# lmb-freiburg/understanding_flow_robustness

Hardware: AMD Instinct MI355X
Metric: attack-iters/s (higher is better)
Workload: dtype f32

## Files before the change

include/ufr_hip.h:

```cpp
#ifndef UFR_HIP_H_
#define UFR_HIP_H_

#include <stdint.h>

#ifdef __cplusplus
extern "C" {
#endif

#define UFR_ABI_VERSION 9

enum { UFR_F32 = 0, UFR_F64 = 1, UFR_F16 = 2 };
enum {
  UFR_OK = 0,
  UFR_EINVAL = -1,
  UFR_EUNSUPPORTED = -2,
  UFR_ELAUNCH = -3
};

typedef void* ufr_stream_t;

int ufr_abi_version(void);
const char* ufr_last_error(void);
int ufr_device_count(void);
const char* ufr_build_manifest(void);
// ... 376 lines not shown
int ufr_normalize_frames(const float* frames_a, const float* frames_b, float* out, int Ba, int Bb, int C, int H, int W,
                         const double* mean, ufr_stream_t stream);

int ufr_corr_forward_planes_window(const void* f1_planes, const void* f2_planes, long in_plane_stride, void* out_planes,
                                   long out_plane_stride, int out_chunk0, int B, int C, int H, int W, int patch,
                                   int dilation_patch, float scale, float slope, const int* win, int level_stride,
                                   int win_cells, ufr_stream_t stream);

int ufr_corr_forward_planes_changed(const void* f1_planes, const void* f2_planes, long in_plane_stride, void* out_planes,
                                    long out_plane_stride, int out_chunk0, int B, int C, int H, int W, int patch,
                                    int dilation_patch, float scale, float slope, const int* win, int level_stride,
                                    int win_cells_h, int win_cells_w, int margin, ufr_stream_t stream);

int ufr_corr_backward_window_fused(const float* f1, const float* f2, const float* G, int g_chunk0, float g_scale,
                                   const float* G_redir, float* grad_window, int B, int C, int H, int W, int patch,
                                   int dilation_patch, const int* win, int level_stride, int wh, int ww, int margin,
                                   ufr_stream_t stream);

int ufr_corr_forward_planes(const void* f1_planes, const void* f2_planes, long in_plane_stride, void* out_planes,
                            long out_plane_stride, int out_chunk0, int B, int C, int H, int W, int patch,
                            int dilation_patch, float scale, float slope, ufr_stream_t stream);
int ufr_flow_head_planes_forward(const void* planes, long plane_stride, int chunk0, int chunks, const float* wpk, int w_chunks,
                                 const float* bias, float* out, int B, int H, int W, ufr_stream_t stream);
int ufr_flow_head_planes_forward_mfma(const void* planes, long plane_stride, int chunk0, int chunks, const void* wmf, int w_chunks,
                                      const float* bias, float* out, int B, int H, int W, ufr_stream_t stream);
int ufr_flow_head_split_plan(int B, int H, int W, int chunks, int* slices, int* starved, long* partial_floats);
int ufr_flow_head_planes_forward_split(const void* planes, long plane_stride, int chunk0, int chunks, const void* wmf, int w_chunks,
                                       float* partials, long partial_floats, int slices, int B, int H, int W, ufr_stream_t stream);
int ufr_flow_head_split_finish(const float* partials, long partial_floats, int slices, const float* bias, float* flow,
                               const float* up_w, const float* up_bias, void* up_planes, long up_plane_stride, int up_chunk, int B,
                               int H, int W, ufr_stream_t stream);
int ufr_deconv_flow_tail_backward_mfma(const void* grad_planes, long plane_stride, int chunk0, int chunks, const void* wmf,
                                       int w_chunks, float* G, int g_chunks, int out_chunk, int B, int H, int W, ufr_stream_t stream);
int ufr_flow_head_planes_backward(const float* grad_y, const float* wpk, int w_chunks, float* G, int g_chunks, int chunk0, int chunks,
                                  int B, int H, int W, int accumulate, ufr_stream_t stream);
int ufr_flow_head_planes_backward_finalize(const float* grad_y, const float* wpk, int w_chunks, float* G, int g_chunks, int chunk0,
                                           int chunks, int B, int H, int W, int accumulate, const void* mask_planes, void* out_planes,
                                           long out_plane_stride, int fin_chunk0, int fin_chunks, float slope, ufr_stream_t stream);
#define UFR_PF_REGION_BAND 1
#define UFR_PF_REGION_WINDOW 2
int ufr_flow_head_planes_backward_regions(const float* grad_y, const float* wpk, int w_chunks, float* G, int g_chunks, int chunk0,
                                          int chunks, int B, int H, int W, int accumulate, int head_chunks, int region,
                                          const int* origin, int origin_stride, int origin_div, int reg_h, int reg_w, int margin,
                                          float* head_out, int head_out_images, const void* mask_planes, void* out_planes,
                                          long out_plane_stride, int fin_chunk0, int fin_chunks, float slope, ufr_stream_t stream);
int ufr_upfeat_planes_forward_mfma(const void* planes, long plane_stride, int chunk0, int chunks, const void* wmf, int w_chunks,
                                   const float* bias, float* out, int B, int H, int W, ufr_stream_t stream);
int ufr_upfeat_planes_backward(const float* grad_y, const float* wpk, int w_chunks, float* G, int g_chunks, int chunk0, int chunks,
                               int B, int H, int W, int accumulate, ufr_stream_t stream);
int ufr_flow_up_planes_forward(const float* x, const float* w, const float* bias, void* planes, long plane_stride,
                               int chunk, int B, int H, int W, ufr_stream_t stream);
int ufr_flow_up_planes_backward(const float* G, int chunk, const float* w, float* grad_x, int B, int H, int W,
                                int accumulate , ufr_stream_t stream);

#define UFR_TRAIN_LOSS_MAX_SCALES 8
typedef struct {
  const float* gt; int B, H, W;
  int nscale;
  const float* pred[UFR_TRAIN_LOSS_MAX_SCALES];
  float* grad[UFR_TRAIN_LOSS_MAX_SCALES];
  int h[UFR_TRAIN_LOSS_MAX_SCALES], w[UFR_TRAIN_LOSS_MAX_SCALES];
  double weight[UFR_TRAIN_LOSS_MAX_SCALES];
  int kind;
  double div_flow;
  double* ws; long ws_elems;
  double* out;
} ufr_train_loss_desc;
long ufr_train_loss_workspace_doubles(int B, int nscale, const int* h, const int* w);
int ufr_train_loss(const ufr_train_loss_desc* d, ufr_stream_t stream);

typedef struct { float* p; const float* g; float* m; float* v; long n; } ufr_adamw_seg;
typedef struct { double lr, beta1, beta2, eps, weight_decay, bias1, bias2; } ufr_adamw_hyper;
long ufr_grad_norm_partials(const ufr_adamw_seg* segs, int nseg);
int ufr_grad_norm(const ufr_adamw_seg* segs, int nseg, float max_norm, double* partials, long partial_elems, float* norm_out,
                  ufr_stream_t stream);
int ufr_adamw_step(const ufr_adamw_seg* segs, int nseg, const ufr_adamw_hyper* h, const float* norm, ufr_stream_t stream);

int ufr_sweep_paste(const float* tgt, const float* ref, const float* patch_p, const float* mask_p, const int* origins,
                    const int* origins_host, float* adv_tgt, float* adv_ref, int K, int H, int W, int ph, int pw, float lo, float hi,
                    const ufr_cone_chain* chain, int win_h, int win_w, int* win, float* xw, ufr_stream_t stream);
long ufr_sweep_metrics_workspace_doubles(int K);
int ufr_sweep_metrics(const float* pred, const float* gt, const float* mask_p, const int* origins, const int* origins_host, int K,
                      int H, int W, int Hg, int Wg, int ph, int pw, int valid_in_patch, double* ws, long ws_elems, float* out,
                      int row0, int rows, ufr_stream_t stream);

#define UFR_FEATURE_STATS_MAX_SEGS 32
typedef struct {
  const void* src; long plane_stride; long pixels; int kind, images, image0, B, chunk0, channels; double unleaky; long out_col;
} ufr_feature_stats_seg;
long ufr_feature_stats_workspace_doubles(const ufr_feature_stats_seg* segs, int nseg);
int ufr_feature_stats(const ufr_feature_stats_seg* segs, int nseg, double* ws, long ws_elems, double* out, int out_rows, long out_cols,
                      long out_stride, ufr_stream_t stream);

#define UFR_DIVERSE_COLS 8
long ufr_abs_sums_workspace_doubles(long n);
int ufr_abs_sums(const float* g0, const float* g1, long n, double* ws, long ws_elems, float* out, ufr_stream_t stream);
int ufr_momentum_update(const float* img0, const float* img1, const float* g0, const float* g1, const float* sums, float* m0,
                        float* m1, float* adv0, float* adv1, float* delta, int B, int CHW, float mu, float one_minus_mu, float lr,
                        float eps, float lo, float hi, int frames, int ascent, ufr_stream_t stream);
int ufr_diverse_table_check(const int* table_host, int rows, int H, int W);
long ufr_diverse_workspace_doubles(int B, int H, int W, int Cg);
int ufr_diverse_forward(const float* adv0, const float* adv1, const float* gt, float* x0, float* x1, float* gt_out, int B, int H,
                        int W, int Cg, const int* table, int rows, const int* step, float* scale_t, double* ws, long ws_elems,
                        ufr_stream_t stream);
int ufr_diverse_backward(const float* gx0, const float* gx1, float* g0, float* g1, int B, int H, int W, const int* table, int rows,
                         const int* step, ufr_stream_t stream);
// ... 7 lines not shown
```

understanding_flow_robustness_amd/_lib.py:

```python
from __future__ import annotations

import ctypes as C
import os

import torch

_HERE = os.path.dirname(os.path.abspath(__file__))
LIB_PATH = os.environ.get("UFR_HIP_LIB") or os.path.join(_HERE, "lib", "libufr_hip.so")
UFR_F32, UFR_F64, UFR_F16 = 0, 1, 2
ABI_VERSION = 9
_lib = None


class CorrParams(C.Structure):
    _fields_ = [(n, C.c_int) for n in (
        "kH", "kW", "patchH", "patchW", "padH", "padW", "dilationH", "dilationW",
        "dilation_patchH", "dilation_patchW", "dH", "dW")]


UFR_MAX_LEVELS = 8


class Pyramid(C.Structure):
    _fields_ = [("num_levels", C.c_int),
# ... 204 lines not shown
    "ufr_cm_norm_stats_apply": [_vp, _vp, _vp, _f, _vp, _l, _i, _vp, _l, _i, _l, _i, _i, _i, _i, _vp],
    "ufr_cm_norm_backward": [_vp, _vp, _vp, _i, _vp, _vp, _vp, _vp, _l, _i, _l, _i, _i, _i, _vp],
    "ufr_cm_masked_copy": [_vp, _vp, _l, _vp, _l, _vp],
    "ufr_raft_flow_patches": [_vp, _vp, _l, _i, _i, _i, _i, _vp],
    "ufr_raft_motion_finish_slabs": [_vp, _i, _i, _i, _vp, _f, _vp, _l, _vp, _l, _i, _vp, _i, _i, _i, _vp],
    "ufr_raft_motion_finish": [_vp, _l, _vp, _l, _i, _vp, _i, _i, _i, _vp],
    "ufr_raft_coords_step": [_vp, _vp, _vp, _vp, _vp, _l, _vp],
    "ufr_grad_finalize_consume": [_vp, _vp, _vp, _l, _l, _i, _f, _vp],
    "ufr_gru_gates_cm_forward": [_vp, _vp, _l, _i, _vp, _l, _i, _l, _i, _vp],
    "ufr_gru_gates_cm_forward_slabs": [_vp, _i, _i, _vp, _vp, _vp, _vp, _l, _i, _vp, _l, _i, _l, _i, _vp],
    "ufr_gru_blend_cm_forward_slabs": [_vp, _i, _i, _vp, _vp, _vp, _vp, _vp, _l, _i, _vp, _l, _i, _l, _i, _vp],
    "ufr_gru_blend_cm_forward": [_vp, _vp, _vp, _l, _i, _vp, _l, _i, _l, _i, _vp],
    "ufr_gru_blend_cm_backward": [_vp, _vp, _vp, _l, _i, _vp, _vp, _l, _i, _vp, _vp, _l, _i, _vp, _vp],
    "ufr_gru_gates_cm_backward": [_vp, _vp, _l, _i, _vp, _vp, _vp, _l, _i, _vp, _l, _i, _i, _vp, _vp],
    "ufr_altcorr_pyramid_forward": [_vp, _vp, _vp, _vp, _i, _i, _i, _i, _i, _f, _vp],
    "ufr_altcorr_pyramid_backward": [_vp, _vp, _vp, _vp, _vp, _vp, _i, _i, _i, _i, _i, _f, _i, _vp],
    "ufr_altcorr_pyramid_backward_cm": [_vp, _vp, _vp, _vp, _vp, _vp, _i, _i, _i, _i, _i, _f, _i, _vp],
    "ufr_upfeat_planes_forward_mfma": [_vp, _l, _i, _i, _vp, _i, _vp, _vp, _i, _i, _i, _vp],
    "ufr_upfeat_planes_backward": [_vp, _vp, _i, _vp, _i, _i, _i, _i, _i, _i, _i, _vp],
    "ufr_flow_up_planes_forward": [_vp, _vp, _vp, _vp, _l, _i, _i, _i, _i, _vp],
    "ufr_flow_head_split_plan": [_i, _i, _i, _i, C.POINTER(C.c_int), C.POINTER(C.c_int), C.POINTER(C.c_long)],
    "ufr_flow_head_planes_forward_split": [_vp, _l, _i, _i, _vp, _i, _vp, _l, _i, _i, _i, _i, _vp],
    "ufr_flow_head_split_finish": [_vp, _l, _i, _vp, _vp, _vp, _vp, _vp, _l, _i, _i, _i, _i, _vp],
    "ufr_flow_up_planes_backward": [_vp, _i, _vp, _vp, _i, _i, _i, _i, _vp],
    "ufr_corr_forward_planes_changed": [_vp, _vp, _l, _vp, _l, _i, _i, _i, _i, _i, _i, _i, _f, _f, _vp, _i, _i, _i, _i, _vp],
    "ufr_corr_forward_planes_window": [_vp, _vp, _l, _vp, _l, _i, _i, _i, _i, _i, _i, _i, _f, _f, _vp, _i, _i, _vp],
    "ufr_corr_forward_planes": [_vp, _vp, _l, _vp, _l, _i, _i, _i, _i, _i, _i, _i, _f, _f, _vp],
    "ufr_convex_upsample_forward": [_vp, _vp, _vp, _i, _i, _i, _vp],
    "ufr_convex_upsample_backward": [_vp, _vp, _vp, _vp, _vp, _vp, _i, _i, _i, _vp],
    "ufr_affine_resample_f64": [_vp, _vp, _i, _i, _i, _i, _i, _d, _d, _d, _d, _d, _d, _i, _vp],
    "ufr_patch_place": [_vp, _vp, _vp, _i, _i, _i, _vp, _vp, _vp, _i, _i, _i, _i, _vp],
    "ufr_patch_crop_f64": [_vp, _vp, _vp, _i, _i, _i, _i, _i, _i, _i, _vp],
    "ufr_resample_u8_horizontal": [_vp, _vp, _i, _i, _i, _i, _i, _vp, _vp, _i, _vp],
    "ufr_resample_u8_vertical": [_vp, _vp, _i, _i, _i, _i, _vp, _vp, _i, _vp],
    "ufr_u8_to_tensor": [_vp, _vp, _i, _i, _i, _i, _i, _i, _i, _f, _vp],
    "ufr_kitti_flow_decode": [_vp, _vp, _i, _i, _vp],
    "ufr_host_png_unfilter": [_vp, _vp, _i, _i, _i],
    "ufr_igemm_clock_probe": [_vp, _i],
    "ufr_altcorr_planes_prepare": [_vp, _vp, _l, _l, _i, _vp],
    "ufr_altcorr_planes_forward": [_vp, _l, C.POINTER(AltCorrPlaneLevels), _vp, _vp, _i, _i, _i, _i, _i, _f, _vp],
    "ufr_conv1_direct": [_vp, _vp, _i, _i, _i, _i, _vp, _vp, _vp, _f, _vp, _l, _i, _vp],
    "ufr_train_loss": [C.POINTER(TrainLossDesc), _vp],
    "ufr_grad_norm": [C.POINTER(AdamwSeg), _i, _f, _vp, _l, _vp, _vp],
    "ufr_adamw_step": [C.POINTER(AdamwSeg), _i, C.POINTER(AdamwHyper), _vp, _vp],
    "ufr_sweep_paste": [_vp, _vp, _vp, _vp, _vp, _vp, _vp, _vp, _i, _i, _i, _i, _i, _f, _f, C.POINTER(ConeChain), _i, _i, _vp, _vp, _vp],
    "ufr_sweep_metrics": [_vp, _vp, _vp, _vp, _vp, _i, _i, _i, _i, _i, _i, _i, _i, _vp, _l, _vp, _i, _i, _vp],
    "ufr_feature_stats": [C.POINTER(FeatureStatsSeg), _i, _vp, _l, _vp, _i, _l, _l, _vp],
    "ufr_abs_sums": [_vp, _vp, _l, _vp, _l, _vp, _vp],
    "ufr_momentum_update": [_vp, _vp, _vp, _vp, _vp, _vp, _vp, _vp, _vp, _vp, _i, _i, _f, _f, _f, _f, _f, _f, _i, _i, _vp],
    "ufr_diverse_table_check": [_vp, _i, _i, _i],
    "ufr_diverse_forward": [_vp, _vp, _vp, _vp, _vp, _vp, _i, _i, _i, _i, _vp, _i, _vp, _vp, _vp, _l, _vp],
    "ufr_diverse_backward": [_vp, _vp, _vp, _vp, _i, _i, _i, _vp, _i, _vp, _vp],
    "ufr_step_advance": [_vp, _vp],
}
DIVERSE_COLS = 8
PLAIN = {"ufr_abi_version": (C.c_int, []), "ufr_last_error": (C.c_char_p, []),
         "ufr_device_count": (C.c_int, []), "ufr_build_manifest": (C.c_char_p, []),
         "ufr_igemm_variant_fallbacks": (C.c_int, []),
         "ufr_conv3x3_c2_workspace_floats": (C.c_long, [_i, _i, _i, _i]),
         "ufr_cm_norm_workspace_doubles": (C.c_long, [_l, _i, _i]),
         "ufr_resample2d_backward_workspace_bytes": (C.c_long, [_i, _i, _i]),
         "ufr_pwc_warp_backward_workspace_bytes": (C.c_long, [_i, _i, _i]),
         "ufr_altcorr_pyramid_workspace_bytes": (C.c_long, [_i, _i, _i, _i, _i, _i]),
         "ufr_train_loss_workspace_doubles": (C.c_long, [_i, _i, C.POINTER(C.c_int), C.POINTER(C.c_int)]),
         "ufr_grad_norm_partials": (C.c_long, [C.POINTER(AdamwSeg), _i]),
         "ufr_sweep_metrics_workspace_doubles": (C.c_long, [_i]),
         "ufr_feature_stats_workspace_doubles": (C.c_long, [C.POINTER(FeatureStatsSeg), _i]),
         "ufr_abs_sums_workspace_doubles": (C.c_long, [_l]),
         "ufr_diverse_workspace_doubles": (C.c_long, [_i, _i, _i, _i])}


def lib():
    global _lib
    if _lib is None:
        if not os.path.exists(LIB_PATH):
            raise RuntimeError(
                f"{LIB_PATH} not found: build it with `python -c 'import __graft_entry__ as g; "
                "g.build()'` or `make -C understanding_flow_robustness_amd/csrc` (hipcc, gfx950). "
                "There is no CPU fallback.")
        handle = C.CDLL(LIB_PATH)
        for name, args in SIGNATURES.items():
            fn = getattr(handle, name)
            fn.argtypes, fn.restype = args, C.c_int
        for name, (res, args) in PLAIN.items():
            fn = getattr(handle, name)
            fn.argtypes, fn.restype = args, res
        if handle.ufr_abi_version() != ABI_VERSION:
            raise RuntimeError(f"{LIB_PATH} has ABI version {handle.ufr_abi_version()}, these bindings are written for "
                               f"{ABI_VERSION}: rebuild it (`make -C understanding_flow_robustness_amd/csrc`)")
        verify_build(handle.ufr_build_manifest().decode("ascii", "replace"))
        _lib = handle
    return _lib


_CSRC = os.path.join(_HERE, "csrc")
_HEADER = os.path.join(os.path.dirname(_HERE), "include", "ufr_hip.h")


def source_checksums(csrc: str = _CSRC, header: str = _HEADER) -> dict:
    import hashlib
    with open(os.path.join(csrc, "ufr_common.h"), "rb") as f:
        shared = f.read()
    with open(header, "rb") as f:
        shared += f.read()
    sums = {}
    for name in sorted(os.listdir(csrc)):
# ... 226 lines not shown
```

understanding_flow_robustness_amd/csrc/attack.hip:

```cpp
#include "ufr_common.h"

namespace {

using ufr::dev::clampf;

__global__ void paste_kernel(const float* __restrict__ tgt, const float* __restrict__ ref,
                             const float* __restrict__ patch, const float* __restrict__ mask,
                             float* __restrict__ adv_tgt, float* __restrict__ adv_ref, long total,
                             long CHW, long pstride, long mstride, int do_clamp, float lo, float hi) {
  for (long i = (long)blockIdx.x * blockDim.x + threadIdx.x; i < total;
       i += (long)gridDim.x * blockDim.x) {
    const long b = i / CHW, e = i - b * CHW;
    const float m = mask[b * mstride + e], pv = patch[b * pstride + e];
    const float mp = m * pv, om = 1.0f - m;
    float a = om * tgt[i] + mp;
    float r = om * ref[i] + mp;
    if (do_clamp) { a = clampf(a, lo, hi); r = clampf(r, lo, hi); }
    adv_tgt[i] = a;
    adv_ref[i] = r;
  }
}

__global__ void update_private_kernel(const float* __restrict__ tgt, const float* __restrict__ ref,
                                      const float* __restrict__ g_tgt, const float* __restrict__ g_ref,
// ... 280 lines not shown
        }
      rows[(long)g * (n + 1) + e] = s;
    }
  }
}

__global__ void patch_apply_paste_rect_kernel(const float* __restrict__ rows, int n_rows, float* __restrict__ patch_p,
                                              float* __restrict__ loss, const float* __restrict__ tgt, const float* __restrict__ ref,
                                              const float* __restrict__ mask_p, const int* __restrict__ origins,
                                              float* __restrict__ adv_tgt, float* __restrict__ adv_ref, int B, int H, int W, int ph,
                                              int pw, float step, float bound, int do_clamp, float lo, float hi,
                                              const float* __restrict__ gate) {
  const bool stopped = gate != nullptr && gate[0] != 0.f;
  const int n = 3 * ph * pw;
  for (int e = blockIdx.x * blockDim.x + threadIdx.x; e <= n; e += gridDim.x * blockDim.x) {
    float s = 0.f;
    for (int r = 0; r < n_rows; ++r) s += rows[(long)r * (n + 1) + e];
    if (e == n) { *loss = s; continue; }
    if (stopped) continue;
    const float pv = patch_p[e] - clampf(step * s, -bound, bound);
    patch_p[e] = pv;
    const int c = e / (ph * pw), q = e - c * ph * pw, i = q / pw, j = q - i * pw;
    const float m = mask_p[e], mp = m * pv, om = 1.0f - m;
    for (int b = 0; b < B; ++b) {
      const int y = origins[2 * b] + i, x = origins[2 * b + 1] + j;
      if ((unsigned)y >= (unsigned)H || (unsigned)x >= (unsigned)W) continue;
      const long o = ((long)b * 3 + c) * H * W + (long)y * W + x;
      float a = om * tgt[o] + mp, d = om * ref[o] + mp;
      if (do_clamp) { a = clampf(a, lo, hi); d = clampf(d, lo, hi); }
      adv_tgt[o] = a;
      adv_ref[o] = d;
    }
  }
}

__global__ void normalize_frames_kernel(const float* __restrict__ a, const float* __restrict__ b, float* __restrict__ out,
                                        long na, long total, int C, long HW, const double* __restrict__ mean) {
  for (long i = (long)blockIdx.x * blockDim.x + threadIdx.x; i < total; i += (long)gridDim.x * blockDim.x) {
    const int c = (int)((i / HW) % C);
    const float v = i < na ? a[i] : b[i - na];
    out[i] = (float)((double)v - mean[c]);
  }
}

__global__ void gate_kernel(const float* __restrict__ loss_cur, float* __restrict__ state, float thr) {
  if (threadIdx.x == 0 && blockIdx.x == 0 && state[0] == 0.f) {
    const float l = *loss_cur;
    state[1] += 1.f;
    state[2] = l;
    if (!(l > thr)) state[0] = 1.f;
  }
}

}

extern "C" int ufr_attack_gate(const float* loss_cur, float* state, float threshold, ufr_stream_t stream) {
  UFR_REQUIRE(loss_cur && state, "attack gate: null pointer argument");
  hipLaunchKernelGGL(gate_kernel, dim3(1), dim3(64), 0, ufr::as_stream(stream), loss_cur, state, threshold);
  return ufr::launched("gate_kernel");
}

extern "C" int ufr_patch_paste(const float* tgt, const float* ref, const float* patch,
                               const float* mask, float* adv_tgt, float* adv_ref, int B, int CHW,
                               long patch_bstride, long mask_bstride, int do_clamp, float lo,
                               float hi, ufr_stream_t stream) {
  UFR_REQUIRE(tgt && ref && patch && mask && adv_tgt && adv_ref, "patch paste: null pointer argument");
  UFR_REQUIRE(B > 0 && CHW > 0, "patch paste: bad shape");
  const long total = (long)B * CHW;
  hipLaunchKernelGGL(paste_kernel, dim3(ufr::stream_grid(total, 256)), dim3(256), 0,
                     ufr::as_stream(stream), tgt, ref, patch, mask, adv_tgt, adv_ref, total,
                     (long)CHW, patch_bstride, mask_bstride, do_clamp, lo, hi);
  return ufr::launched("paste_kernel");
}

extern "C" int ufr_patch_update(const float* tgt, const float* ref, const float* g_tgt,
                                const float* g_ref, float* patch, const float* mask, float* adv_tgt,
                                float* adv_ref, int B, int CHW, long patch_bstride, long mask_bstride,
                                float step, float bound, float lo, float hi, const float* gate_state,
                                ufr_stream_t stream) {
  UFR_REQUIRE(B > 0 && CHW > 0, "patch update: bad shape");
  UFR_REQUIRE(patch_bstride != 0 || B == 1,
              "patch update: one canvas patch behind %d pairs is not defined -- a shared patch lives in patch "
              "coordinates (ufr_patch_grad_crop / ufr_patch_apply / ufr_patch_paste_placed)", B);
  UFR_REQUIRE(tgt && ref && g_tgt && g_ref && patch && mask && adv_tgt && adv_ref,
              "patch update: null pointer argument");
  const long total = (long)B * CHW;
  hipLaunchKernelGGL(update_private_kernel, dim3(ufr::stream_grid(total, 256)), dim3(256), 0, ufr::as_stream(stream),
                     tgt, ref, g_tgt, g_ref, patch, mask, adv_tgt, adv_ref, total, (long)CHW,
                     patch_bstride, mask_bstride, step, bound, lo, hi, gate_state);
  return ufr::launched("update_private_kernel");
}

extern "C" int ufr_flow_loss(const float* flow, const float* target, float* grad_flow, float* loss,
                             int B, int HW, int kind, float weight, float* partials, ufr_stream_t stream) {
  UFR_REQUIRE(flow && target && grad_flow && loss && partials, "flow loss: null pointer argument");
  UFR_REQUIRE(B > 0 && HW > 0 && (kind == 0 || kind == 1), "flow loss: bad argument");
  const long npix = (long)B * HW;
  int grid = ufr::stream_grid(npix, 256);
  if (grid > UFR_LOSS_PARTIALS) grid = UFR_LOSS_PARTIALS;
  hipLaunchKernelGGL(flow_loss_kernel, dim3(grid), dim3(256), 0, ufr::as_stream(stream), flow,
                     target, grad_flow, partials, B, (long)HW, kind, weight);
  hipLaunchKernelGGL(loss_finalize_kernel, dim3(1), dim3(64), 0, ufr::as_stream(stream), partials, grid, loss);
  return ufr::launched("flow_loss_kernel");
}

constexpr int F2_T = 16, F2_R = 4 * F2_T + 8;
// ... 220 lines not shown
    if (cy < h && cx < w) {
      float wxs[8];
      bool vx[8];
#pragma unroll
      for (int t = 0; t < 8; ++t) {
        const int c = 4 * cxl + t, x0 = ti[1][0][c], x1 = ti[1][1][c];
        const float lx = tl[1][c];
        vx[t] = x0 != 255;
        wxs[t] = (x0 == cxl + 1 ? 1.f - lx : 0.f) + (x1 == cxl + 1 ? lx : 0.f);
      }
      float su = 0.f, sv = 0.f;
#pragma unroll
      for (int s = 0; s < 8; ++s) {
        const int r = 4 * cyl + s, y0 = ti[0][0][r], y1 = ti[0][1][r];
        if (y0 == 255) continue;
        const float ly = tl[0][r];
        const float wy = (y0 == cyl + 1 ? 1.f - ly : 0.f) + (y1 == cyl + 1 ? ly : 0.f);
        if (wy == 0.f) continue;
        float ru = 0.f, rv = 0.f;
#pragma unroll
        for (int t = 0; t < 8; ++t)
          if (vx[t]) {
            ru += wxs[t] * g[0][r][4 * cxl + t];
            rv += wxs[t] * g[1][r][4 * cxl + t];
          }
        su += wy * ru;
        sv += wy * rv;
      }
      gflow2[((long)b * 2) * hw + (long)cy * w + cx] = su * flow_scale;
      gflow2[((long)b * 2 + 1) * hw + (long)cy * w + cx] = sv * flow_scale;
    }
  }
  for (int off = 32; off > 0; off >>= 1) part += __shfl_down(part, off, 64);
  if ((tid & 63) == 0) red[tid >> 6] = part;
  __syncthreads();
  if (tid == 0) partials[(blockIdx.z * gridDim.y + blockIdx.y) * gridDim.x + blockIdx.x] = (red[0] + red[1] + red[2] + red[3]) * invn;
}

extern "C" int ufr_flow2_upsampled_loss_fast(const float* flow2, float flow_scale, const float* target, float* grad_flow2, float* loss,
                                             int B, int h, int w, int kind, float weight, float* partials, ufr_stream_t stream) {
  UFR_REQUIRE(flow2 && target && grad_flow2 && loss && partials, "upsampled flow loss (fast): null pointer argument");
  UFR_REQUIRE(B > 0 && h > 0 && w > 0 && (kind == 0 || kind == 1), "upsampled flow loss (fast): bad argument");
  const dim3 grid(ufr::ceil_div(w, F2_T), ufr::ceil_div(h, F2_T), B);
  const long n = (long)grid.x * grid.y * grid.z;
  if (n > UFR_LOSS_PARTIALS || B > 65535)
    return ufr::fail(UFR_EUNSUPPORTED, "upsampled flow loss (fast): %ld tiles exceed the %d partial sums of the fixed-order reduction", n,
                     UFR_LOSS_PARTIALS);
  hipLaunchKernelGGL(flow2_upsampled_loss_fast_kernel, grid, dim3(256), 0, ufr::as_stream(stream), flow2, flow_scale, target,
                     grad_flow2, partials, B, h, w, kind, weight);
  hipLaunchKernelGGL(loss_finalize_kernel, dim3(1), dim3(64), 0, ufr::as_stream(stream), partials, (int)n, loss);
  return ufr::launched("flow2_upsampled_loss_fast_kernel");
}

namespace ufr {
void loss_finalize_launch(const float* partials, int n, float* loss, hipStream_t st) {
  hipLaunchKernelGGL(loss_finalize_kernel, dim3(1), dim3(64), 0, st, partials, n, loss);
}
}

static int check_placed(const int* origins_host, int B, int H, int W, int ph, int pw) {
  if (!origins_host) return 1;
  for (int b = 0; b < B; ++b)
    if (origins_host[2 * b] < 0 || origins_host[2 * b] + ph > H || origins_host[2 * b + 1] < 0 ||
        origins_host[2 * b + 1] + pw > W)
      return 0;
  return 1;
}

extern "C" int ufr_patch_grad_crop(const float* g_tgt, const float* g_ref, const float* mask_p, const int* origins,
                                   const int* origins_host, const float* loss_local, float* rows, int B, int H, int W,
                                   int ph, int pw, int groups, ufr_stream_t stream) {
  UFR_REQUIRE(g_tgt && g_ref && mask_p && origins && loss_local && rows, "patch grad crop: null pointer argument");
  UFR_REQUIRE(B > 0 && H > 0 && W > 0 && ph > 0 && pw > 0 && ph <= H && pw <= W, "patch grad crop: bad shape");
  UFR_REQUIRE(groups > 0 && B % groups == 0, "patch grad crop: the pairs must split evenly into %d groups", groups);
  UFR_REQUIRE(check_placed(origins_host, B, H, W, ph, pw), "patch grad crop: a placement leaves the frame");
  const int n = 3 * ph * pw + 1;
  hipLaunchKernelGGL(patch_grad_crop_kernel, dim3(ufr::ceil_div(n, 256)), dim3(256), 0, ufr::as_stream(stream), g_tgt,
                     g_ref, mask_p, origins, loss_local, rows, B, H, W, ph, pw, groups);
  return ufr::launched("patch_grad_crop_kernel");
}

extern "C" int ufr_patch_grad_crop_window(const float* gxw, const int* win, const float* mask_p, const int* origins,
                                          const float* loss_local, float* rows, int B, int H, int W, int wh, int ww, int ph, int pw,
                                          int groups, ufr_stream_t stream) {
  UFR_REQUIRE(gxw && win && mask_p && origins && loss_local && rows, "patch grad crop (window): null pointer argument");
  UFR_REQUIRE(B > 0 && H > 0 && W > 0 && ph > 0 && pw > 0 && ph <= H && pw <= W && wh > 0 && ww > 0 && wh <= H && ww <= W,
              "patch grad crop (window): bad shape");
  UFR_REQUIRE(groups > 0 && B % groups == 0, "patch grad crop (window): the pairs must split evenly into %d groups", groups);
  const int n = 3 * ph * pw + 1;
  hipLaunchKernelGGL(patch_grad_crop_window_kernel, dim3(ufr::ceil_div(n, 256)), dim3(256), 0, ufr::as_stream(stream), gxw, win,
                     mask_p, origins, loss_local, rows, B, H, W, wh, ww, ph, pw, groups);
  return ufr::launched("patch_grad_crop_window_kernel");
}

extern "C" int ufr_patch_apply(const float* rows, int n_rows, float* patch_p, float* loss, int ph, int pw, float step,
                               float bound, const float* gate_state, ufr_stream_t stream) {
  UFR_REQUIRE(rows && patch_p && loss, "patch apply: null pointer argument");
  UFR_REQUIRE(n_rows > 0 && ph > 0 && pw > 0, "patch apply: bad shape");
  const int n = 3 * ph * pw;
  hipLaunchKernelGGL(patch_apply_kernel, dim3(ufr::ceil_div(n + 1, 256)), dim3(256), 0, ufr::as_stream(stream), rows,
                     n_rows, patch_p, loss, n, step, bound, gate_state);
  return ufr::launched("patch_apply_kernel");
}

extern "C" int ufr_patch_paste_placed(const float* tgt, const float* ref, const float* patch_p, const float* mask_p,
                                      const int* origins, const int* origins_host, float* adv_tgt, float* adv_ref,
// ... 90 lines not shown
```

understanding_flow_robustness_amd/csrc/conv1_direct.hip:

```cpp
#include <atomic>

#include "ufr_common.h"

namespace {

using ufr::dev::bf16x8;
using ufr::dev::f32x4;
using ufr::dev::split3;
typedef __attribute__((ext_vector_type(4))) __bf16 bf16x4;

constexpr int TY = 8, TX = 32;
constexpr int RY = 2 * TY + 5, RX = 2 * TX + 5;
constexpr int LX = 72;
constexpr int PLANE_B = RY * LX * 8;
constexpr int BUF_B = 3 * PLANE_B;
constexpr int PX_PER_THREAD = (RY * RX + 511) / 512;
__device__ constexpr int PROD_W[6] = {2, 0, 1, 1, 0, 0};
__device__ constexpr int PROD_X[6] = {0, 2, 1, 0, 1, 0};

struct Conv1Args {
  const float* fa; const float* fb; int Ba, N, H, W;
  const double* mean;
  const __bf16* wimg;
  const float* bias; float slope;
  __bf16* out; long plane_stride; int out_chunk0;
  int tiles_x, tiles_y, tiles;
};

template <bool BUF_>
__global__ __launch_bounds__(512) __attribute__((amdgpu_waves_per_eu(2, 2))) void conv1_direct_kernel(const Conv1Args a) {
  extern __shared__ __attribute__((aligned(16))) unsigned char lds[];
  const int tid = threadIdx.x, lane = tid & 63, wave = __builtin_amdgcn_readfirstlane(tid >> 6);
  const int q = wave & 3, half = wave >> 2;
  const int li = lane & 15, g = lane >> 4;
  const int Hh = a.H >> 1, Wh = a.W >> 1;
  const long M = (long)a.N * Hh * Wh;

  for (int i = tid; i < 2 * BUF_B / 16; i += 512) reinterpret_cast<uint4*>(lds)[i] = make_uint4(0, 0, 0, 0);
  bf16x8 wf[7][3];
#pragma unroll
  for (int ky = 0; ky < 7; ++ky)
#pragma unroll
    for (int p = 0; p < 3; ++p)
      wf[ky][p] = *reinterpret_cast<const bf16x8*>(a.wimg + (((long)p * 7 + ky) * 64 + q * 16 + li) * 32 + g * 8);
  float bias4[4];
#pragma unroll
  for (int r = 0; r < 4; ++r) bias4[r] = a.bias[q * 16 + g * 4 + r];
  const double m0 = a.mean[0], m1 = a.mean[1], m2 = a.mean[2];
  __amdgpu_buffer_rsrc_t rsrc = __builtin_amdgcn_make_buffer_rsrc(a.out, 0, BUF_ ? (int)(6L * a.plane_stride) : 0, 0x00020000);

  float pre[PX_PER_THREAD][3];
  unsigned pre_ok = 0;
  auto tile_coords = [&](int t, int& n, int& Y0, int& X0) {
    const int tx = t % a.tiles_x, r = t / a.tiles_x;
    n = r / a.tiles_y;
    Y0 = (r - n * a.tiles_y) * TY;
    X0 = tx * TX;
  };
  auto fetch = [&](int t) {
    int n, Y0, X0;
    tile_coords(t, n, Y0, X0);
    const float* img = n < a.Ba ? a.fa + (long)n * 3 * a.H * a.W : a.fb + (long)(n - a.Ba) * 3 * a.H * a.W;
    const long HW = (long)a.H * a.W;
    pre_ok = 0;
#pragma unroll
    for (int i = 0; i < PX_PER_THREAD; ++i) {
      const int idx = tid + 512 * i, ry = idx / RX, rx = idx - ry * RX;
      const int iy = 2 * Y0 - 3 + ry, ix = 2 * X0 - 3 + rx;
      const bool ok = idx < RY * RX && (unsigned)iy < (unsigned)a.H && (unsigned)ix < (unsigned)a.W;
      const long o = (long)iy * a.W + ix;
      pre[i][0] = ok ? img[o] : 0.f;
      pre[i][1] = ok ? img[o + HW] : 0.f;
      pre[i][2] = ok ? img[o + 2 * HW] : 0.f;
      pre_ok |= ok ? 1u << i : 0u;
    }
  };
  auto stage = [&](int buf) {
    unsigned char* base = lds + buf * BUF_B;
#pragma unroll
    for (int i = 0; i < PX_PER_THREAD; ++i) {
      const int idx = tid + 512 * i;
      if (idx >= RY * RX) continue;
      const int ry = idx / RX, rx = idx - ry * RX;
      const bool ok = (pre_ok >> i) & 1u;
      const float v0 = ok ? (float)((double)pre[i][0] - m0) : 0.f;
      const float v1 = ok ? (float)((double)pre[i][1] - m1) : 0.f;
      const float v2 = ok ? (float)((double)pre[i][2] - m2) : 0.f;
      bf16x4 p0, p1, p2;
      __bf16 x, y, z;
      split3(v0, x, y, z); p0[0] = x; p1[0] = y; p2[0] = z;
      split3(v1, x, y, z); p0[1] = x; p1[1] = y; p2[1] = z;
      split3(v2, x, y, z); p0[2] = x; p1[2] = y; p2[2] = z;
      p0[3] = (__bf16)0.f; p1[3] = (__bf16)0.f; p2[3] = (__bf16)0.f;
      unsigned char* d = base + (ry * LX + rx) * 8;
      *reinterpret_cast<bf16x4*>(d) = p0;
      *reinterpret_cast<bf16x4*>(d + PLANE_B) = p1;
      *reinterpret_cast<bf16x4*>(d + 2 * PLANE_B) = p2;
    }
  };

  int t = blockIdx.x;
  if (t >= a.tiles) return;
  fetch(t);
  __syncthreads();
  stage(0);
  int tn = t + gridDim.x;
  if (tn < a.tiles) fetch(tn);
  __syncthreads();

  for (int it = 0; t < a.tiles; ++it, t = tn, tn += gridDim.x) {
    const int buf = it & 1;
    int n, Y0, X0;
    tile_coords(t, n, Y0, X0);
    const unsigned char* src = lds + buf * BUF_B;
    const unsigned char* base = src + ((2 * half * 4) * LX + 2 * (li + g)) * 8;
    bf16x8 xf[3][3];
    auto read_step = [&](int s, bf16x8 (&dst)[3]) {
      const int pt = s / 7, ky = s - 7 * pt;
      const unsigned char* px = base + ((2 * (pt >> 1) + ky) * LX + 2 * ((pt & 1) * 16)) * 8;
#pragma unroll
      for (int p = 0; p < 3; ++p) dst[p] = *reinterpret_cast<const bf16x8*>(px + p * PLANE_B);
    };
    read_step(0, xf[0]);
// ... 32 lines not shown
      const long e = ((long)(a.out_chunk0 + (q >> 1)) * M + m) * 32 + (q & 1) * 16 + (g & 2) * 4;
      const bool live = y < Hh && x < Wh;
      if constexpr (BUF_) {
        const unsigned off = live ? (unsigned)(e * 2) : 0x80000000u;
        typedef __attribute__((ext_vector_type(4))) unsigned u32x4;
        __builtin_amdgcn_raw_buffer_store_b128(__builtin_bit_cast(u32x4, o0), rsrc, off, 0, 0);
        __builtin_amdgcn_raw_buffer_store_b128(__builtin_bit_cast(u32x4, o1), rsrc, off, (unsigned)(a.plane_stride * 2), 0);
        __builtin_amdgcn_raw_buffer_store_b128(__builtin_bit_cast(u32x4, o2), rsrc, off, (unsigned)(a.plane_stride * 4), 0);
      } else if (live) {
        __bf16* o = a.out + e;
        *reinterpret_cast<bf16x8*>(o) = o0;
        *reinterpret_cast<bf16x8*>(o + a.plane_stride) = o1;
        *reinterpret_cast<bf16x8*>(o + 2 * a.plane_stride) = o2;
      }
    };
    f32x4 acc_prev[4];
#pragma unroll
    for (int pt = 0; pt < 8; ++pt) {
      f32x4 acc[4];
#pragma unroll
      for (int c = 0; c < 4; ++c) acc[c] = f32x4{0.f, 0.f, 0.f, 0.f};
      if (pt > 0) epilogue(pt - 1, acc_prev);
#pragma unroll
      for (int ky = 0; ky < 7; ++ky) {
        const int s = pt * 7 + ky;
        if (s + 2 < 56) read_step(s + 2, xf[(s + 2) % 3]);
#pragma unroll
        for (int tp = 0; tp < 6; ++tp) {
          const int c = (ky * 6 + tp) & 3;
          acc[c] = __builtin_amdgcn_mfma_f32_16x16x32_bf16(wf[ky][PROD_W[tp]], xf[s % 3][PROD_X[tp]], acc[c], 0, 0, 0);
        }
      }
#pragma unroll
      for (int i = 0; i < 42; ++i) {
        __builtin_amdgcn_sched_group_barrier(0x008, 1, 0);
        __builtin_amdgcn_sched_group_barrier(0x002, 2, 0);
        if (i & 1) __builtin_amdgcn_sched_group_barrier(0x100, 1, 0);
      }
      __builtin_amdgcn_sched_barrier(0);
#pragma unroll
      for (int c = 0; c < 4; ++c) acc_prev[c] = acc[c];
    }
    epilogue(7, acc_prev);
    if (tn < a.tiles) {
      stage(buf ^ 1);
      if (tn + (int)gridDim.x < a.tiles) fetch(tn + gridDim.x);
    }
    __syncthreads();
  }
}

}

extern "C" int ufr_conv1_direct(const float* frames_a, const float* frames_b, int Ba, int Bb, int H, int W, const double* mean,
                                const void* wimg, const float* bias, float slope, void* out_planes, long plane_stride,
                                int out_chunk0, ufr_stream_t stream) {
  UFR_REQUIRE(frames_a && mean && wimg && bias && out_planes && (frames_b || Bb == 0), "conv1 direct: null pointer");
  UFR_REQUIRE(Ba > 0 && Bb >= 0 && H > 0 && W > 0 && !(H & 1) && !(W & 1) && plane_stride > 0 && out_chunk0 >= 0, "conv1 direct: bad shape");
  Conv1Args a;
  a.fa = frames_a; a.fb = frames_b; a.Ba = Ba; a.N = Ba + Bb; a.H = H; a.W = W; a.mean = mean;
  a.wimg = static_cast<const __bf16*>(wimg); a.bias = bias; a.slope = slope;
  a.out = static_cast<__bf16*>(out_planes); a.plane_stride = plane_stride; a.out_chunk0 = out_chunk0;
  a.tiles_x = ((W >> 1) + TX - 1) / TX; a.tiles_y = ((H >> 1) + TY - 1) / TY;
  const long tiles = (long)a.N * a.tiles_x * a.tiles_y;
  UFR_REQUIRE(tiles < (1L << 30) && (long)a.N * (H >> 1) * (W >> 1) < (1L << 30), "conv1 direct: too many pixels");
  a.tiles = (int)tiles;
  int dev = 0;
  if (hipGetDevice(&dev) != hipSuccess || dev < 0 || dev >= 64) return ufr::fail(UFR_ELAUNCH, "conv1 direct: no current device");
  static std::atomic<bool> raised[64] = {};
  if (!raised[dev].load(std::memory_order_acquire)) {
    hipError_t e = ufr::ensure_dynamic_lds(reinterpret_cast<const void*>(conv1_direct_kernel<true>), 2 * BUF_B);
    if (e == hipSuccess) e = ufr::ensure_dynamic_lds(reinterpret_cast<const void*>(conv1_direct_kernel<false>), 2 * BUF_B);
    if (e != hipSuccess) return ufr::fail(UFR_ELAUNCH, "conv1 direct: %s", hipGetErrorString(e));
    raised[dev].store(true, std::memory_order_release);
  }
  const int grid = (int)(tiles < ufr::kNumCU ? tiles : ufr::kNumCU);
  if (6L * plane_stride < 0x7fffffffL) conv1_direct_kernel<true><<<grid, 512, 2 * BUF_B, ufr::as_stream(stream)>>>(a);
  else conv1_direct_kernel<false><<<grid, 512, 2 * BUF_B, ufr::as_stream(stream)>>>(a);
  return ufr::launched("conv1_direct_kernel");
}
```

understanding_flow_robustness_amd/csrc/correlation_window_mfma.hip:

```cpp
#include "ufr_common.h"

namespace {

using ufr::dev::bf16x8;
using ufr::dev::f32x4;
using ufr::dev::split3;

__device__ constexpr int WPA[6] = {2, 0, 1, 1, 0, 0};
__device__ constexpr int WPB[6] = {0, 2, 1, 0, 1, 0};

constexpr int WP = 21, WR = 10, WC = 256;
constexpr int AST = 72;

template <int NR, int TPW>
__global__ __launch_bounds__(256) void corr_bwd_window_mfma_kernel(
    const float* __restrict__ f1, const float* __restrict__ f2, const float* __restrict__ G, int g_chunk0, float g_scale,
    const float* __restrict__ Gredir, float* __restrict__ gwin, int B, int H, int W, const int* __restrict__ win,
    int level_stride, int wh, int ww, int margin) {
  constexpr int CS = 16 / (4 * TPW);
  __shared__ __attribute__((aligned(16))) __bf16 As[2][NR][3][16 * AST];
  const int tid = threadIdx.x, lane = tid & 63, wave = tid >> 6;
  const int lin = blockIdx.x + gridDim.x * (blockIdx.y + gridDim.y * blockIdx.z);
  const int n = lin % B, rest = lin / B, bx = rest % (int)gridDim.x, by = rest / (int)gridDim.x;
  const int adj = by / CS, cs = by - adj * CS;
  const int pr = bx & 1, ly0 = pr + 2 * (bx >> 1) * NR;
  const int* w = win + n * 8;
  const int y0 = min(max(w[0] / level_stride, 0), H - wh), x0 = min(max(w[1] / level_stride, 0), W - ww);
  const int xb = ((x0 - 2 * WR) >> 2) << 2;
  const long M = (long)B * H * W, plane = (long)H * W;
  const float* src = (adj == 0 ? f2 : f1) + (long)n * WC * plane;
  for (int i = tid; i < 2 * NR * 3 * 16 * AST / 8; i += 256) reinterpret_cast<bf16x8*>(&As[0][0][0][0])[i] = bf16x8{};
  f32x4 acc[NR][TPW];
#pragma unroll
  for (int r = 0; r < NR; ++r)
#pragma unroll
    for (int t = 0; t < TPW; ++t) acc[r][t] = f32x4{0.f, 0.f, 0.f, 0.f};
  __syncthreads();
  const int ybase = y0 + ly0;
  const int ct0 = cs * 4 * TPW + wave * TPW;
  for (int s = 0; s < WP + NR - 1; ++s) {
    const int sy = ybase - 2 * WR + 2 * s;
    if (sy < 0 || sy >= H) continue;
    const int buf = s & 1;
    bf16x8 fb[TPW][2][3];
#pragma unroll
    for (int t = 0; t < TPW; ++t)
#pragma unroll
      for (int ks = 0; ks < 2; ++ks) {
        const int c = (ct0 + t) * 16 + (lane & 15), col = xb + 32 * ks + 8 * (lane >> 4);
        const float* p = src + ((long)c * H + sy) * W + col;
        float4 v0 = make_float4(0.f, 0.f, 0.f, 0.f), v1 = v0;
        if (col >= 0 && col < W) v0 = *reinterpret_cast<const float4*>(p);
        if (col + 4 >= 0 && col + 4 < W) v1 = *reinterpret_cast<const float4*>(p + 4);
        const float v[8] = {v0.x, v0.y, v0.z, v0.w, v1.x, v1.y, v1.z, v1.w};
#pragma unroll
        for (int e = 0; e < 8; ++e) {
          __bf16 a, b2, c2;
          split3(v[e], a, b2, c2);
          fb[t][ks][0][e] = a; fb[t][ks][1][e] = b2; fb[t][ks][2][e] = c2;
        }
      }
    for (int item = tid; item < NR * 16 * WP; item += 256) {
      const int r = item / (16 * WP), rem = item - r * 16 * WP, j = rem >> 4, xl = rem & 15;
      const int i = adj == 0 ? s - r : 2 * WR - s + r;
      const int ly = ly0 + 2 * r;
      if (i < 0 || i >= WP || ly >= wh) continue;
      const int x = x0 + xl, y = y0 + ly;
      const int xs = adj == 0 ? x + 2 * (j - WR) : x - 2 * (j - WR);
      float v = 0.f;
      if (xl < ww && xs >= 0 && xs < W) {
        const int d = i * WP + j;
        const long pix = adj == 0 ? ((long)n * H + y) * W + x : ((long)n * H + sy) * W + xs;
        v = G[((long)(g_chunk0 + (d >> 5)) * M + pix) * 32 + (d & 31)] * g_scale;
      }
      __bf16 a, b2, c2;
      split3(v, a, b2, c2);
      const int o = xl * AST + (xs - xb);
      As[buf][r][0][o] = a; As[buf][r][1][o] = b2; As[buf][r][2][o] = c2;
    }
    __syncthreads();
#pragma unroll
    for (int r = 0; r < NR; ++r) {
      const int i = adj == 0 ? s - r : 2 * WR - s + r;
      if (i < 0 || i >= WP || ly0 + 2 * r >= wh) continue;
#pragma unroll
      for (int ks = 0; ks < 2; ++ks) {
        bf16x8 fa[3];
#pragma unroll
        for (int p = 0; p < 3; ++p)
          fa[p] = *reinterpret_cast<const bf16x8*>(&As[buf][r][p][(lane & 15) * AST + 32 * ks + 8 * (lane >> 4)]);
#pragma unroll
        for (int t = 0; t < TPW; ++t)
#pragma unroll
          for (int q = 0; q < 6; ++q)
            acc[r][t] = __builtin_amdgcn_mfma_f32_16x16x32_bf16(fa[WPA[q]], fb[t][ks][WPB[q]], acc[r][t], 0, 0, 0);
      }
    }
  }
#pragma unroll
  for (int r = 0; r < NR; ++r) {
    const int ly = ly0 + 2 * r;
    if (ly >= wh) continue;
    const int y = y0 + ly;
    const bool rim_y = (ly < margin && y0 > 0) || (ly >= wh - margin && y0 + wh < H);
#pragma unroll
    for (int t = 0; t < TPW; ++t) {
      const int c = (ct0 + t) * 16 + (lane & 15);
#pragma unroll
      for (int e = 0; e < 4; ++e) {
        const int xl = 4 * (lane >> 4) + e;
        if (xl >= ww) continue;
        const bool rim = rim_y || (xl < margin && x0 > 0) || (xl >= ww - margin && x0 + ww < W);
        float v = acc[r][t][e];
        if (adj == 0 && Gredir) v += Gredir[((long)(c >> 5) * M + ((long)n * H + y) * W + x0 + xl) * 32 + (c & 31)];
        gwin[(((long)(adj * B + n) * WC + c) * wh + ly) * ww + xl] = rim ? 0.f : v;
      }
    }
  }
}

}

extern "C" int ufr_corr_backward_window_fused(const float* f1, const float* f2, const float* G, int g_chunk0, float g_scale,
                                              const float* G_redir, float* grad_window, int B, int C, int H, int W, int patch,
                                              int dilation_patch, const int* win, int level_stride, int wh, int ww, int margin,
                                              ufr_stream_t stream) {
  UFR_REQUIRE(f1 && f2 && G && grad_window && win, "corr backward window (fused): null pointer");
  UFR_REQUIRE(B > 0 && H > 0 && W > 0 && g_chunk0 >= 0 && level_stride > 0, "corr backward window (fused): bad shape");
  UFR_REQUIRE(wh > 0 && ww > 0 && wh <= H && ww <= W && margin >= 0 && 2 * margin <= wh && 2 * margin <= ww,
              "corr backward window (fused): window %dx%d (margin %d) in %dx%d", wh, ww, margin, H, W);
  if (C != WC || patch != WP || dilation_patch != 2 || ww > 16 || (W & 3))
    return ufr::fail(UFR_EUNSUPPORTED, "corr backward window (fused): built for 256 channels, patch 21, dilation_patch 2, windows "
                                       "of at most 16 cells across, W a multiple of 4; got C=%d patch=%d dilation=%d ww=%d W=%d",
                     C, patch, dilation_patch, ww, W);
  const int cfg = B <= 2 ? 11 : 21;
#define UFR_CBW_LAUNCH(NR, TPW)                                                                                             \
  corr_bwd_window_mfma_kernel<NR, TPW><<<dim3(2 * ufr::ceil_div(ufr::ceil_div(wh, 2), NR), 2 * (16 / (4 * TPW)), B), 256, 0, \
                                         ufr::as_stream(stream)>>>(f1, f2, G, g_chunk0, g_scale, G_redir, grad_window, B, H, W, \
                                                                   win, level_stride, wh, ww, margin)
  if (cfg == 11) UFR_CBW_LAUNCH(1, 1);
  else UFR_CBW_LAUNCH(2, 1);
#undef UFR_CBW_LAUNCH
  return ufr::launched("corr_bwd_window_mfma_kernel");
}
```

understanding_flow_robustness_amd/csrc/engine_small.hip:

```cpp
#include "ufr_common.h"

namespace {

using ufr::dev::bf16x8;
using ufr::dev::f32x4;
using ufr::dev::split3;

constexpr int PF_TH = 8, PF_TW = 32, PF_HH = PF_TH + 2, PF_HW = PF_TW + 2, PF_CS = 36;
__global__ __launch_bounds__(1024) void flow_head_planes_fwd(const __bf16* __restrict__ x, long plane_stride, int chunk0,
                                                             int chunks, const float* __restrict__ wpk,
                                                             const float* __restrict__ bias, float* __restrict__ out, int B,
                                                             int H, int W, int S) {
  extern __shared__ __attribute__((aligned(16))) float lds_pf[];
  const long M = (long)B * H * W;
  const int tid = threadIdx.x, slice = tid >> 8, t = tid & 255;
  float* tile = lds_pf + (long)slice * (PF_HH * PF_HW * PF_CS);
  float* part = lds_pf + (long)S * (PF_HH * PF_HW * PF_CS + 576);
  const int tiles_x = (W + PF_TW - 1) / PF_TW, tiles_y = (H + PF_TH - 1) / PF_TH;
  const int b = blockIdx.x / (tiles_x * tiles_y), tr = blockIdx.x - b * tiles_x * tiles_y;
  const int y0 = (tr / tiles_x) * PF_TH, x0 = (tr % tiles_x) * PF_TW;
  const int ly = t / PF_TW, lx = t - ly * PF_TW;
  const int per = (chunks + S - 1) / S, c_lo = slice * per, c_hi = min(chunks, c_lo + per);
  float a0 = 0.f, a1 = 0.f;
  for (int ch = c_lo; ch < c_lo + per; ++ch) {
// ... 75 lines not shown
    msk[k] = ok ? 1.f : 0.f;
  }
  float a0 = 0.f, a1 = 0.f;
  const int per = (chunks + S - 1) / S, c_lo = slice * per, c_hi = min(chunks, c_lo + per);
  for (int ch = c_lo; ch < c_hi; ++ch) {
    const __bf16* xc = x + ((long)(chunk0 + ch) * M + pp) * 32 + q * 8;
    const float* wc = lds_w + ch * 576 + q * 8;
#pragma unroll 3
    for (int k = 0; k < 9; ++k) {
      const __bf16* src = xc + off[k];
      const bf16x8 p0 = *reinterpret_cast<const bf16x8*>(src);
      const bf16x8 p1 = *reinterpret_cast<const bf16x8*>(src + plane_stride);
      const bf16x8 p2 = *reinterpret_cast<const bf16x8*>(src + 2 * plane_stride);
      const float4 w0a = *reinterpret_cast<const float4*>(wc + (k * 2 + 0) * 32), w0b = *reinterpret_cast<const float4*>(wc + (k * 2 + 0) * 32 + 4);
      const float4 w1a = *reinterpret_cast<const float4*>(wc + (k * 2 + 1) * 32), w1b = *reinterpret_cast<const float4*>(wc + (k * 2 + 1) * 32 + 4);
      const float w0[8] = {w0a.x, w0a.y, w0a.z, w0a.w, w0b.x, w0b.y, w0b.z, w0b.w};
      const float w1[8] = {w1a.x, w1a.y, w1a.z, w1a.w, w1b.x, w1b.y, w1b.z, w1b.w};
      float s0 = 0.f, s1 = 0.f;
#pragma unroll
      for (int j = 0; j < 8; ++j) {
        const float v = ((float)p0[j] + (float)p1[j]) + (float)p2[j];
        s0 = fmaf(v, w0[j], s0);
        s1 = fmaf(v, w1[j], s1);
      }
      a0 = fmaf(s0, msk[k], a0);
      a1 = fmaf(s1, msk[k], a1);
    }
  }
  a0 += __shfl_xor(a0, 1, 64); a1 += __shfl_xor(a1, 1, 64);
  a0 += __shfl_xor(a0, 2, 64); a1 += __shfl_xor(a1, 2, 64);
  float* part = lds_w + chunks * 576;
  if (q == 0) {
    part[(slice * 64 + (t >> 2)) * 2 + 0] = a0;
    part[(slice * 64 + (t >> 2)) * 2 + 1] = a1;
  }
  __syncthreads();
  if (slice == 0 && q == 0 && live) {
    float r0 = 0.f, r1 = 0.f;
    for (int sl = 0; sl < S; ++sl) {
      r0 += part[(sl * 64 + (t >> 2)) * 2 + 0];
      r1 += part[(sl * 64 + (t >> 2)) * 2 + 1];
    }
    const long HW = (long)H * W, b = pix / HW, p = pix - b * HW;
    out[(b * 2 + 0) * HW + p] = r0 + bias[0];
    out[(b * 2 + 1) * HW + p] = r1 + bias[1];
  }
}

__device__ constexpr int PFM_A[6] = {2, 0, 1, 1, 0, 0};
__device__ constexpr int PFM_B[6] = {0, 2, 1, 0, 1, 0};
__device__ __attribute__((aligned(64))) unsigned pf_zero_page[16];
constexpr int PFM_MAXT = 6;

template <int MODE, int WPS_ = 4, int MAXT_ = PFM_MAXT>
__global__ __launch_bounds__(512) void flow_head_planes_fwd_mfma(const __bf16* __restrict__ x, long plane_stride, int chunk0,
                                                                 int chunks, const __bf16* __restrict__ wmf,
                                                                 const float* __restrict__ bias, float* __restrict__ out,
                                                                 int out_chunk, int B, int H, int W, int TH, int S) {
  constexpr int TW = MODE == 0 ? 32 : 16, TS = MODE == 0 ? 20 : 36;
  constexpr int PFM_HW = MODE == 2 ? 18 : 34;
  extern __shared__ __attribute__((aligned(16))) float pfm_T[];
  const int Hs = MODE == 1 ? 2 * H : H, Ws = MODE == 1 ? 2 * W : W;
  const long M = (long)B * Hs * Ws;
  const int tid = threadIdx.x, lane = tid & 63, wave = tid >> 6, slice = wave / WPS_, tw = wave % WPS_;
  const int tiles_x = (W + TW - 1) / TW, tiles_y = (H + TH - 1) / TH;
  const int b = blockIdx.x / (tiles_x * tiles_y), tr = blockIdx.x - b * tiles_x * tiles_y;
  const int y0 = (tr / tiles_x) * TH, x0 = (tr % tiles_x) * TW;
  const int sy0 = MODE == 1 ? 2 * y0 - 1 : y0 - 1, sx0 = MODE == 1 ? 2 * x0 - 1 : x0 - 1;
  const int nh = (MODE == 1 ? 2 * TH + 2 : TH + 2) * PFM_HW, mt = (nh + 15) >> 4;
  const __bf16* zero = reinterpret_cast<const __bf16*>(pf_zero_page);
  const __bf16* abase[MAXT_];
  unsigned okmask = 0;
#pragma unroll
  for (int s = 0; s < MAXT_; ++s) {
    const int hp = (tw + WPS_ * s) * 16 + (lane & 15);
    const int hy = hp / PFM_HW, hx = hp - hy * PFM_HW;
    const int yy = sy0 + hy, xx = sx0 + hx;
    const bool ok = tw + WPS_ * s < mt && hp < nh && yy >= 0 && yy < Hs && xx >= 0 && xx < Ws;
    abase[s] = ok ? x + ((long)chunk0 * M + ((long)b * Hs + yy) * Ws + xx) * 32 + (lane >> 4) * 8 : zero;
    okmask |= ok ? 1u << s : 0u;
  }
  f32x4 acc[MAXT_][2];
#pragma unroll
  for (int s = 0; s < MAXT_; ++s) acc[s][0] = acc[s][1] = f32x4{0.f, 0.f, 0.f, 0.f};
  const int per = (chunks + S - 1) / S, c_lo = slice * per, c_hi = min(chunks, c_lo + per);
  const __bf16* wl = wmf + (lane & 15) * 32 + (lane >> 4) * 8;
  for (int ch = c_lo; ch < c_hi; ++ch) {
    bf16x8 fb[2][3];
#pragma unroll
    for (int p = 0; p < 3; ++p)
#pragma unroll
      for (int nt = 0; nt < 2; ++nt) fb[nt][p] = *reinterpret_cast<const bf16x8*>(wl + (((long)ch * 3 + p) * 2 + nt) * 512);
#pragma unroll
    for (int h = 0; h < MAXT_; h += 6) {
      bf16x8 fa[6][3];
#pragma unroll
      for (int s = 0; s < 6; ++s)
        if (tw + WPS_ * (h + s) < mt) {
#pragma unroll
          for (int p = 0; p < 3; ++p) {
            const long off = (okmask >> (h + s) & 1u) ? (long)ch * M * 32 + p * plane_stride : 0;
            fa[s][p] = *reinterpret_cast<const bf16x8*>(abase[h + s] + off);
          }
        }
#pragma unroll
      for (int s = 0; s < 6; ++s)
        if (tw + WPS_ * (h + s) < mt) {
#pragma unroll
          for (int nt = 0; nt < 2; ++nt)
#pragma unroll
            for (int q = 0; q < 6; ++q)
              acc[h + s][nt] = __builtin_amdgcn_mfma_f32_16x16x32_bf16(fa[s][PFM_A[q]], fb[nt][PFM_B[q]], acc[h + s][nt], 0, 0, 0);
        }
    }
  }
  float* T = pfm_T + (long)slice * mt * 16 * TS;
#pragma unroll
  for (int s = 0; s < MAXT_; ++s)
    if (tw + WPS_ * s < mt) {
#pragma unroll
      for (int r = 0; r < 4; ++r) {
        float* row = T + ((tw + WPS_ * s) * 16 + (lane >> 4) * 4 + r) * TS;
        row[lane & 15] = acc[s][0][r];
        if (MODE != 0 || (lane & 15) < 2) row[16 + (lane & 15)] = acc[s][1][r];
      }
    }
  __syncthreads();
  if constexpr (MODE == 2) {
    const int Ho = 2 * H, Wo = 2 * W;
    for (int idx = tid; idx < 2 * TH * 32; idx += blockDim.x) {
      const int ly = idx >> 5, lx = idx & 31;
      const int Y = 2 * y0 + ly, X = 2 * x0 + lx;
      if (Y >= Ho || X >= Wo) continue;
      float r0 = 0.f, r1 = 0.f;
      for (int sl = 0; sl < S; ++sl) {
        const float* Ts = pfm_T + (long)sl * mt * 16 * TS;
#pragma unroll
        for (int t = 0; t < 2; ++t) {
          const int ky = ((Y + 1) & 1) + 2 * t, hy = (Y + 1 - ky) / 2 - sy0;
#pragma unroll
          for (int u = 0; u < 2; ++u) {
            const int kx = ((X + 1) & 1) + 2 * u, hx = (X + 1 - kx) / 2 - sx0;
            const float* e = Ts + (hy * PFM_HW + hx) * TS + 2 * (ky * 4 + kx);
            r0 += e[0];
            r1 += e[1];
          }
        }
      }
      const long HWo = (long)Ho * Wo, p = (long)Y * Wo + X;
      out[((long)b * 2 + 0) * HWo + p] = r0 + bias[0];
      out[((long)b * 2 + 1) * HWo + p] = r1 + bias[1];
    }
    return;
  }
  if (tid < TH * TW) {
    const int ly = tid / TW, lx = tid - ly * TW;
    const int yy = y0 + ly, xx = x0 + lx;
    if (yy < H && xx < W) {
      float r0 = 0.f, r1 = 0.f;
      for (int sl = 0; sl < S; ++sl) {
        const float* Ts = pfm_T + (long)sl * mt * 16 * TS;
        if (MODE == 0) {
#pragma unroll
          for (int k = 0; k < 9; ++k) {
            const float* e = Ts + ((ly + k / 3) * PFM_HW + lx + k % 3) * TS + 2 * k;
            r0 += e[0];
            r1 += e[1];
          }
        } else {
#pragma unroll
          for (int k = 0; k < 16; ++k) {
            const float* e = Ts + ((2 * ly + k / 4) * PFM_HW + 2 * lx + k % 4) * TS + 2 * k;
            r0 += e[0];
            r1 += e[1];
          }
        }
      }
      if (MODE == 0) {
        const long HW = (long)H * W, p = (long)yy * W + xx;
        out[((long)b * 2 + 0) * HW + p] = r0 + bias[0];
        out[((long)b * 2 + 1) * HW + p] = r1 + bias[1];
      } else {
        float* o = out + ((long)out_chunk * B * H * W + ((long)b * H + yy) * W + xx) * 32;
        o[0] = r0;
        o[1] = r1;
      }
    }
  }
}

constexpr int PFS_TS = 18;
__global__ __launch_bounds__(256) void flow_head_split_gemm(const __bf16* __restrict__ x, long plane_stride, int chunk0, int chunks,
                                                            const __bf16* __restrict__ wmf, float* __restrict__ Tp, long M, int per) {
  const int lane = threadIdx.x & 63, wave = threadIdx.x >> 6, slice = blockIdx.y;
  const long m0 = ((long)blockIdx.x * 4 + wave) * 16;
  if (m0 >= M) return;
  const long p = m0 + (lane & 15);
  const bool ok = p < M;
  const __bf16* a = ok ? x + ((long)chunk0 * M + p) * 32 + (lane >> 4) * 8 : reinterpret_cast<const __bf16*>(pf_zero_page);
  const long astep = ok ? M * 32 : 0;
  const long pstep = ok ? plane_stride : 0;
  const __bf16* wl = wmf + (lane & 15) * 32 + (lane >> 4) * 8;
  const int c_lo = slice * per, c_hi = min(chunks, c_lo + per);
  f32x4 acc[2] = {f32x4{0.f, 0.f, 0.f, 0.f}, f32x4{0.f, 0.f, 0.f, 0.f}};
// ... 319 lines not shown
      const float w1[8] = {w1a.x, w1a.y, w1a.z, w1a.w, w1b.x, w1b.y, w1b.z, w1b.w};
#pragma unroll
      for (int j = 0; j < 8; ++j) a[j] = fmaf(g1[k], w1[j], fmaf(g0[k], w0[j], a[j]));
    }
    float4* dst = reinterpret_cast<float4*>(G + ((long)(chunk0 + ch) * M + pix) * 32 + q * 8);
    float4 lo = make_float4(a[0], a[1], a[2], a[3]), hi = make_float4(a[4], a[5], a[6], a[7]);
    if (accumulate) {
      const float4 o0 = dst[0], o1 = dst[1];
      lo.x += o0.x; lo.y += o0.y; lo.z += o0.z; lo.w += o0.w;
      hi.x += o1.x; hi.y += o1.y; hi.z += o1.z; hi.w += o1.w;
    }
    dst[0] = lo;
    dst[1] = hi;
  }
}

__global__ void flow_up_planes_fwd(const float* __restrict__ x, const float* __restrict__ w, const float* __restrict__ bias,
                                   __bf16* __restrict__ planes, long plane_stride, int chunk, int B, int H, int W, int has_bias) {
  const int Ho = 2 * H, Wo = 2 * W;
  const long total = (long)B * Ho * Wo;
  for (long i = (long)blockIdx.x * blockDim.x + threadIdx.x; i < total; i += (long)gridDim.x * blockDim.x) {
    const int X = (int)(i % Wo), Y = (int)((i / Wo) % Ho), b = (int)(i / ((long)Wo * Ho));
    float a0 = has_bias ? bias[0] : 0.f, a1 = has_bias ? bias[1] : 0.f;
#pragma unroll
    for (int t = 0; t < 2; ++t) {
      const int ky = ((Y + 1) & 1) + 2 * t, yy = (Y + 1 - ky) / 2;
      if (Y + 1 - ky < 0 || yy >= H) continue;
#pragma unroll
      for (int u = 0; u < 2; ++u) {
        const int kx = ((X + 1) & 1) + 2 * u, xx = (X + 1 - kx) / 2;
        if (X + 1 - kx < 0 || xx >= W) continue;
#pragma unroll
        for (int ic = 0; ic < 2; ++ic) {
          const float v = x[((size_t)b * 2 + ic) * H * W + (size_t)yy * W + xx];
          a0 = fmaf(v, w[((ic * 2 + 0) * 4 + ky) * 4 + kx], a0);
          a1 = fmaf(v, w[((ic * 2 + 1) * 4 + ky) * 4 + kx], a1);
        }
      }
    }
    __bf16 s0[3], s1[3];
    split3(a0, s0[0], s0[1], s0[2]);
    split3(a1, s1[0], s1[1], s1[2]);
    __bf16* dst = planes + ((long)chunk * total + i) * 32;
#pragma unroll
    for (int p = 0; p < 3; ++p) {
      bf16x8 v = {s0[p], s1[p], (__bf16)0.f, (__bf16)0.f, (__bf16)0.f, (__bf16)0.f, (__bf16)0.f, (__bf16)0.f};
      const bf16x8 zero = {(__bf16)0.f, (__bf16)0.f, (__bf16)0.f, (__bf16)0.f, (__bf16)0.f, (__bf16)0.f, (__bf16)0.f, (__bf16)0.f};
      bf16x8* o = reinterpret_cast<bf16x8*>(dst + p * plane_stride);
      o[0] = v; o[1] = zero; o[2] = zero; o[3] = zero;
    }
  }
}

__global__ void flow_up_planes_bwd(const float* __restrict__ G, int chunk, const float* __restrict__ w, float* __restrict__ gx,
                                   int B, int H, int W, int accumulate) {
  const int Ho = 2 * H, Wo = 2 * W;
  const long total = (long)B * H * W, Mf = (long)B * Ho * Wo;
  for (long i = (long)blockIdx.x * blockDim.x + threadIdx.x; i < total; i += (long)gridDim.x * blockDim.x) {
    const int xx = (int)(i % W), yy = (int)((i / W) % H), b = (int)(i / ((long)W * H));
    float a0 = 0.f, a1 = 0.f;
#pragma unroll
    for (int ky = 0; ky < 4; ++ky) {
      const int Y = 2 * yy - 1 + ky;
      if (Y < 0 || Y >= Ho) continue;
#pragma unroll
      for (int kx = 0; kx < 4; ++kx) {
        const int X = 2 * xx - 1 + kx;
        if (X < 0 || X >= Wo) continue;
        const float2 g = *reinterpret_cast<const float2*>(G + ((long)chunk * Mf + ((long)b * Ho + Y) * Wo + X) * 32);
        a0 = fmaf(g.x, w[((0 * 2 + 0) * 4 + ky) * 4 + kx], a0);
        a1 = fmaf(g.x, w[((1 * 2 + 0) * 4 + ky) * 4 + kx], a1);
        a0 = fmaf(g.y, w[((0 * 2 + 1) * 4 + ky) * 4 + kx], a0);
        a1 = fmaf(g.y, w[((1 * 2 + 1) * 4 + ky) * 4 + kx], a1);
      }
    }
    float* o0 = gx + ((size_t)b * 2 + 0) * H * W + (size_t)yy * W + xx;
    float* o1 = gx + ((size_t)b * 2 + 1) * H * W + (size_t)yy * W + xx;
    *o0 = accumulate ? *o0 + a0 : a0;
    *o1 = accumulate ? *o1 + a1 : a1;
  }
}

bool planes_hold(long plane_stride, long pixels, int chunk0, int chunks) {
  return plane_stride > 0 && (long)(chunk0 + chunks) * pixels * 32 <= plane_stride;
}
#define UFR_REQUIRE_RANGE(what, plane_stride, pixels, chunk0, chunks, w_chunks)                                                       \
  do {                                                                                                                                \
    if (!planes_hold(plane_stride, pixels, chunk0, chunks))                                                                           \
      return ufr::fail(UFR_EINVAL, "%s: chunks [%d, %d) leave the planes operand (%ld chunks per plane)", what, chunk0,               \
                       chunk0 + chunks, (long)(plane_stride) / ((long)(pixels) * 32));                                               \
    if ((chunks) > (w_chunks))                                                                                                        \
      return ufr::fail(UFR_EINVAL, "%s: %d chunks asked of packed weights that hold %d", what, chunks, w_chunks);                     \
  } while (0)
#define UFR_REQUIRE_GRANGE(what, chunk0, chunks, w_chunks, g_chunks)                                                                  \
  do {                                                                                                                                \
    if ((chunk0) + (chunks) > (g_chunks))                                                                                             \
      return ufr::fail(UFR_EINVAL, "%s: chunks [%d, %d) leave the gradient sum (%d chunks)", what, chunk0, chunk0 + chunks, g_chunks); \
    if ((chunks) > (w_chunks))                                                                                                        \
      return ufr::fail(UFR_EINVAL, "%s: %d chunks asked of packed weights that hold %d", what, chunks, w_chunks);                     \
  } while (0)

}

extern "C" int ufr_flow_head_planes_forward(const void* planes, long plane_stride, int chunk0, int chunks, const float* wpk, int w_chunks,
                                            const float* bias, float* out, int B, int H, int W, ufr_stream_t stream) {
  UFR_REQUIRE(planes && wpk && bias && out, "flow head (planes) forward: null pointer");
  UFR_REQUIRE(B > 0 && H > 0 && W > 0 && chunks > 0 && chunks <= 48 && chunk0 >= 0 && (long)B * H * W < (1L << 29),
              "flow head (planes) forward: bad shape");
  UFR_REQUIRE_RANGE("flow head (planes) forward", plane_stride, (long)B * H * W, chunk0, chunks, w_chunks);
  const int blocks = B * ufr::ceil_div(H, PF_TH) * ufr::ceil_div(W, PF_TW);
  hipStream_t st = ufr::as_stream(stream);
  (void)ufr::ensure_dynamic_lds(reinterpret_cast<const void*>(flow_head_planes_fwd), (2 * (PF_HH * PF_HW * PF_CS + 576) + 2 * 256 * 2) * 4);
  (void)ufr::ensure_dynamic_lds(reinterpret_cast<const void*>(flow_head_planes_fwd_small), 48 * 576 * 4 + 4 * 64 * 2 * 4);
  if (blocks >= 192) {
    const int S = (blocks < 512 && chunks >= 8) ? 2 : 1;
    const size_t lds = ((size_t)S * (PF_HH * PF_HW * PF_CS + 576) + (size_t)S * 256 * 2) * 4;
    flow_head_planes_fwd<<<blocks, 256 * S, lds, st>>>(static_cast<const __bf16*>(planes), plane_stride, chunk0, chunks, wpk, bias,
                                                       out, B, H, W, S);
    return ufr::launched("flow_head_planes_fwd");
  }
  const long M = (long)B * H * W;
  const int sblocks = ufr::ceil_div(M, 64);
  int S = 1;
  while (S < 4 && (long)sblocks * S * 2 <= 2048 && chunks >= 4 * S) S *= 2;
  const size_t lds = (size_t)chunks * 576 * 4 + (size_t)S * 64 * 2 * 4;
  flow_head_planes_fwd_small<<<sblocks, 256 * S, lds, st>>>(static_cast<const __bf16*>(planes), plane_stride, chunk0, chunks, wpk,
                                                           bias, out, B, H, W, S);
  return ufr::launched("flow_head_planes_fwd_small");
}

namespace {
struct PfMode0Plan { int TH, blocks, S; bool eight, starved; };
PfMode0Plan pf_mode0_plan(int B, int H, int W, int chunks) {
  auto blocks_of = [&](int th) { return (long)B * ufr::ceil_div(H, th) * ufr::ceil_div(W, 32); };
  PfMode0Plan p;
  p.TH = blocks_of(8) >= 512 ? 8 : (blocks_of(4) >= 256 ? 4 : 2);
  p.blocks = (int)blocks_of(p.TH);
  const int S = (p.blocks >= 512 || chunks < 4) ? 1 : 2;
  const int mt = ((p.TH + 2) * 34 + 15) / 16;
  p.eight = mt <= 12 && S == 2 && chunks >= 16 && p.blocks <= 256;
  p.S = p.eight ? 8 : S;
  p.starved = blocks_of(4) < 256;
  return p;
}

template <int MODE>
int launch_pf_mfma(const void* planes, long plane_stride, int chunk0, int chunks, const void* wmf, const float* bias, float* out,
                   int out_chunk, int B, int H, int W, hipStream_t st, const char* what) {
  constexpr int TW = MODE == 0 ? 32 : 16, TS = MODE == 0 ? 20 : 36, HWs = MODE == 2 ? 18 : 34;
  auto blocks_of = [&](int th) { return B * ufr::ceil_div(H, th) * ufr::ceil_div(W, TW); };
  int TH;
  if (MODE == 0) TH = blocks_of(8) >= 512 ? 8 : (blocks_of(4) >= 256 ? 4 : 2);
  else if (MODE == 1) TH = blocks_of(4) >= 256 ? 4 : 2;
  else TH = blocks_of(16) >= 512 ? 16 : (blocks_of(8) >= 256 ? 8 : 4);
  const int blocks = blocks_of(TH);
  const int S = (blocks >= 512 || chunks < 4) ? 1 : 2;
  const int mt = ((MODE == 1 ? 2 * TH + 2 : TH + 2) * HWs + 15) / 16;
  const size_t lds = (size_t)S * mt * 16 * TS * sizeof(float);
  if (lds > 64 * 1024) {
    hipError_t e = ufr::ensure_dynamic_lds(reinterpret_cast<const void*>(flow_head_planes_fwd_mfma<MODE>), lds);
    if (e != hipSuccess) return ufr::fail(UFR_ELAUNCH, "%s: %s", what, hipGetErrorString(e));
  }
  if constexpr (MODE == 0) if (mt <= 12 && S == 2 && chunks >= 16 && blocks <= 256) {
    const size_t lds8 = (size_t)8 * mt * 16 * TS * sizeof(float);
    hipError_t e = ufr::ensure_dynamic_lds(reinterpret_cast<const void*>(flow_head_planes_fwd_mfma<MODE, 1, 12>),
                                           8 * 12 * 16 * TS * sizeof(float));
    if (e != hipSuccess) return ufr::fail(UFR_ELAUNCH, "%s: %s", what, hipGetErrorString(e));
    flow_head_planes_fwd_mfma<MODE, 1, 12><<<blocks, 512, lds8, st>>>(static_cast<const __bf16*>(planes), plane_stride, chunk0, chunks,
                                                                      static_cast<const __bf16*>(wmf), bias, out, out_chunk, B, H, W, TH, 8);
    return ufr::launched(what);
  }
  flow_head_planes_fwd_mfma<MODE><<<blocks, 256 * S, lds, st>>>(static_cast<const __bf16*>(planes), plane_stride, chunk0, chunks,
                                                                static_cast<const __bf16*>(wmf), bias, out, out_chunk, B, H, W, TH, S);
  return ufr::launched(what);
}
}

extern "C" int ufr_flow_head_planes_forward_mfma(const void* planes, long plane_stride, int chunk0, int chunks, const void* wmf,
                                                 int w_chunks, const float* bias, float* out, int B, int H, int W, ufr_stream_t stream) {
  UFR_REQUIRE(planes && wmf && bias && out, "flow head (planes, mfma) forward: null pointer");
  UFR_REQUIRE(B > 0 && H > 0 && W > 0 && chunks > 0 && chunks <= 48 && chunk0 >= 0 && (long)B * H * W < (1L << 29),
              "flow head (planes, mfma) forward: bad shape");
  UFR_REQUIRE_RANGE("flow head (planes, mfma) forward", plane_stride, (long)B * H * W, chunk0, chunks, w_chunks);
  return launch_pf_mfma<0>(planes, plane_stride, chunk0, chunks, wmf, bias, out, 0, B, H, W, ufr::as_stream(stream),
                           "flow_head_planes_fwd_mfma");
}

extern "C" int ufr_flow_head_split_plan(int B, int H, int W, int chunks, int* slices, int* starved, long* partial_floats) {
  UFR_REQUIRE(slices && starved && partial_floats, "flow head split plan: null pointer");
  UFR_REQUIRE(B > 0 && H > 0 && W > 0 && chunks > 0 && chunks <= 48 && (long)B * H * W < (1L << 29), "flow head split plan: bad shape");
  const PfMode0Plan p = pf_mode0_plan(B, H, W, chunks);
  *slices = p.S;
  *starved = p.starved ? 1 : 0;
  *partial_floats = (long)p.S * B * H * W * PFS_TS;
  return UFR_OK;
}

extern "C" int ufr_flow_head_planes_forward_split(const void* planes, long plane_stride, int chunk0, int chunks, const void* wmf,
                                                  int w_chunks, float* partials, long partial_floats, int slices, int B, int H, int W,
                                                  ufr_stream_t stream) {
  UFR_REQUIRE(planes && wmf && partials, "flow head (planes, split) forward: null pointer");
  UFR_REQUIRE(B > 0 && H > 0 && W > 0 && chunks > 0 && chunks <= 48 && chunk0 >= 0 && (long)B * H * W < (1L << 29),
              "flow head (planes, split) forward: bad shape");
  UFR_REQUIRE_RANGE("flow head (planes, split) forward", plane_stride, (long)B * H * W, chunk0, chunks, w_chunks);
  const PfMode0Plan p = pf_mode0_plan(B, H, W, chunks);
  UFR_REQUIRE(slices == p.S, "flow head (planes, split) forward: %d chunk slices asked, the unsplit form of this grid adds %d (the sums "
              "would differ in the last bits)", slices, p.S);
  const long M = (long)B * H * W;
  UFR_REQUIRE(partial_floats >= (long)slices * M * PFS_TS, "flow head (planes, split) forward: the partials buffer holds %ld floats, "
              "%d slices of %ld pixels need %ld", partial_floats, slices, M, (long)slices * M * PFS_TS);
  const int per = ufr::ceil_div(chunks, slices);
  flow_head_split_gemm<<<dim3(ufr::ceil_div(M, 64), slices), 256, 0, ufr::as_stream(stream)>>>(
      static_cast<const __bf16*>(planes), plane_stride, chunk0, chunks, static_cast<const __bf16*>(wmf), partials, M, per);
  return ufr::launched("flow_head_split_gemm");
}

extern "C" int ufr_flow_head_split_finish(const float* partials, long partial_floats, int slices, const float* bias, float* flow,
                                          const float* up_w, const float* up_bias, void* up_planes, long up_plane_stride, int up_chunk,
                                          int B, int H, int W, ufr_stream_t stream) {
  UFR_REQUIRE(partials && bias && flow, "flow head split finish: null pointer");
  UFR_REQUIRE(B > 0 && B <= 65535 && H > 0 && W > 0 && slices > 0 && (long)B * H * W < (1L << 27), "flow head split finish: bad shape");
  UFR_REQUIRE(partial_floats >= (long)slices * B * H * W * PFS_TS, "flow head split finish: the partials buffer holds %ld floats, %d "
              "slices need %ld", partial_floats, slices, (long)slices * B * H * W * PFS_TS);
  if (up_planes) {
    UFR_REQUIRE(up_w && up_chunk >= 0, "flow head split finish: the upsampling needs its weights and a chunk");
    UFR_REQUIRE(planes_hold(up_plane_stride, (long)B * H * W * 4, up_chunk, 1), "flow head split finish: chunk %d leaves the planes "
                "operand", up_chunk);
  }
  flow_head_split_finish<<<dim3(ufr::ceil_div(W, PFF_T), ufr::ceil_div(H, PFF_T), B), 256, 0, ufr::as_stream(stream)>>>(
      partials, slices, bias, flow, up_w, up_bias, static_cast<__bf16*>(up_planes), up_plane_stride, up_chunk, B, H, W);
  return ufr::launched("flow_head_split_finish");
}

extern "C" int ufr_deconv_flow_tail_backward_mfma(const void* grad_planes, long plane_stride, int chunk0, int chunks, const void* wmf,
                                                  int w_chunks, float* G, int g_chunks, int out_chunk, int B, int H, int W,
                                                  ufr_stream_t stream) {
  UFR_REQUIRE(grad_planes && wmf && G, "deconv flow tail backward: null pointer");
  UFR_REQUIRE(B > 0 && H > 0 && W > 0 && chunks > 0 && chunks <= 48 && chunk0 >= 0 && out_chunk >= 0 &&
// ... 74 lines not shown
                       PfFinalize{static_cast<const __bf16*>(mask_planes), static_cast<__bf16*>(out_planes), out_plane_stride, fin_chunk0,
                                  fin_chunks, slope},
                       ufr::as_stream(stream));
}

extern "C" int ufr_flow_head_planes_backward_regions(const float* grad_y, const float* wpk, int w_chunks, float* G, int g_chunks, int chunk0,
                                                     int chunks, int B, int H, int W, int accumulate, int head_chunks, int region,
                                                     const int* origin, int origin_stride, int origin_div, int reg_h, int reg_w,
                                                     int margin, float* head_out, int head_out_images, const void* mask_planes,
                                                     void* out_planes, long out_plane_stride, int fin_chunk0, int fin_chunks, float slope,
                                                     ufr_stream_t stream) {
  const char* what = "flow head (planes) backward, regions";
  UFR_REQUIRE(grad_y && wpk && G && origin, "%s: null pointer", what);
  UFR_REQUIRE(B > 0 && H > 0 && W > 0 && chunks > 0 && chunks <= 48 && chunk0 >= 0 && (long)B * H * W < (1L << 29), "%s: bad shape", what);
  UFR_REQUIRE_GRANGE("flow head (planes) backward, regions", chunk0, chunks, w_chunks, g_chunks);
  UFR_REQUIRE(head_chunks > 0 && head_chunks <= chunks, "%s: the head group is %d of %d chunks", what, head_chunks, chunks);
  UFR_REQUIRE(region == UFR_PF_REGION_BAND || region == UFR_PF_REGION_WINDOW, "%s: region kind %d", what, region);
  UFR_REQUIRE(origin_div > 0 && reg_w > 0 && reg_w <= W && reg_h > 0 && reg_h <= H, "%s: region %d x %d does not fit %d x %d", what,
              reg_h, reg_w, H, W);
  if (region == UFR_PF_REGION_BAND) {
    UFR_REQUIRE(origin_stride >= 1 && reg_h == H && margin == 0 && !head_out, "%s: a band spans every row, has no rim and stays in G", what);
  } else {
    UFR_REQUIRE(origin_stride >= 2 && margin >= 0 && 2 * margin <= reg_h && 2 * margin <= reg_w, "%s: bad window stride / margin", what);
    UFR_REQUIRE(!head_out || head_out_images >= B, "%s: the window tensor holds %d images, the range %d", what, head_out_images, B);
  }
  PfFinalize fin{nullptr, nullptr, 0, 0, 0, 1.f};
  if (out_planes) {
    UFR_REQUIRE(planes_hold(out_plane_stride, (long)B * H * W, chunk0 + fin_chunk0, fin_chunks),
                "%s: the finalised segment leaves the gradient planes", what);
    UFR_REQUIRE(fin_chunk0 >= head_chunks && fin_chunks > 0 && fin_chunk0 + fin_chunks <= chunks && out_plane_stride > 0,
                "%s: the finalised segment leaves the trailing group", what);
    fin = PfFinalize{static_cast<const __bf16*>(mask_planes), static_cast<__bf16*>(out_planes), out_plane_stride, fin_chunk0, fin_chunks, slope};
  }
  auto slice = [](long pixels, int n, int& bx, int& per, int& slices) {
    bx = ufr::ceil_div(pixels * 4, 256);
    slices = 1;
    while ((long)bx * slices < 1024 && slices < n) slices *= 2;
    if (slices > n) slices = n;
    per = ufr::ceil_div(n, slices);
    slices = ufr::ceil_div(n, per);
  };
  PfRegion reg{region, origin, origin_stride, origin_div, reg_h, reg_w, margin, head_out, head_out_images, head_chunks, 0, 0, 0, 1, 1};
  const int tail_chunks = chunks - head_chunks;
  int tail_slices = 0;
  slice((long)B * reg_h * reg_w, head_chunks, reg.head_bx, reg.head_per, reg.head_slices);
  if (tail_chunks > 0) slice((long)B * H * W, tail_chunks, reg.tail_bx, reg.tail_per, tail_slices);
  const int per = reg.head_per > reg.tail_per || tail_chunks == 0 ? reg.head_per : reg.tail_per;
  (void)ufr::ensure_dynamic_lds(reinterpret_cast<const void*>(flow_head_planes_bwd_regions), 48 * 576 * 4);
  flow_head_planes_bwd_regions<<<dim3(reg.head_bx * reg.head_slices + reg.tail_bx * tail_slices), 256, (size_t)per * 576 * 4,
                                 ufr::as_stream(stream)>>>(grad_y, wpk, G, chunk0, chunks, B, H, W, accumulate, reg, fin);
  return ufr::launched("flow_head_planes_bwd_regions");
}

extern "C" int ufr_flow_up_planes_forward(const float* x, const float* w, const float* bias, void* planes, long plane_stride,
                                          int chunk, int B, int H, int W, ufr_stream_t stream) {
  UFR_REQUIRE(x && w && planes, "flow upsample (planes) forward: null pointer");
  UFR_REQUIRE(B > 0 && H > 0 && W > 0 && chunk >= 0, "flow upsample (planes) forward: bad shape");
  flow_up_planes_fwd<<<ufr::stream_grid((long)B * 4 * H * W, 256), 256, 0, ufr::as_stream(stream)>>>(
      x, w, bias, static_cast<__bf16*>(planes), plane_stride, chunk, B, H, W, bias != nullptr);
  return ufr::launched("flow_up_planes_fwd");
}

extern "C" int ufr_flow_up_planes_backward(const float* G, int chunk, const float* w, float* grad_x, int B, int H, int W,
                                           int accumulate, ufr_stream_t stream) {
  UFR_REQUIRE(G && w && grad_x, "flow upsample (planes) backward: null pointer");
  UFR_REQUIRE(B > 0 && H > 0 && W > 0 && chunk >= 0, "flow upsample (planes) backward: bad shape");
  flow_up_planes_bwd<<<ufr::stream_grid((long)B * H * W, 256), 256, 0, ufr::as_stream(stream)>>>(G, chunk, w, grad_x, B, H, W, accumulate);
  return ufr::launched("flow_up_planes_bwd");
}
```

understanding_flow_robustness_amd/flownetc_engine.py:

```python
from __future__ import annotations

import os

import torch
from ._lib import engine_cache as _engine_cache

from . import _lib as L
from . import igemm as ig

_HEADS = ((6, 1024), (5, 1026), (4, 770), (3, 386), (2, 194))


def pf_split_plan(B: int, H: int, W: int, chunks: int):
    import ctypes
    slices, starved, floats = ctypes.c_int(0), ctypes.c_int(0), ctypes.c_long(0)
    L.check(L.lib().ufr_flow_head_split_plan(int(B), int(H), int(W), int(chunks), ctypes.byref(slices), ctypes.byref(starved),
                                             ctypes.byref(floats)), "predict_flow split plan")
    return slices.value, bool(starved.value), floats.value


def _pack_flow_head(weight: torch.Tensor) -> torch.Tensor:
    cin = weight.shape[1]
    chunks = ig.pad32(cin) // 32
    w = torch.zeros(2, chunks * 32, 9, dtype=torch.float32, device=weight.device)
# ... 7 lines not shown
    w = torch.zeros(chunks * 32, 32, dtype=torch.float32, device=weight.device)
    w[:cin, :18] = weight.detach().float().reshape(2, cin, 9).permute(1, 2, 0).reshape(cin, 18)
    wn = w.view(chunks, 32, 32).permute(0, 2, 1).contiguous()
    planes = ig._split3(wn).view(3, chunks, 32, 32).permute(1, 0, 2, 3).contiguous()
    return planes


def _pack_flow_tail_mfma(weight2: torch.Tensor) -> torch.Tensor:
    cout = weight2.shape[1]
    chunks = ig.pad32(cout) // 32
    w = torch.zeros(chunks * 32, 32, dtype=torch.float32, device=weight2.device)
    w[:cout] = weight2.detach().float().reshape(2, cout, 16).permute(1, 2, 0).reshape(cout, 32)
    wn = w.view(chunks, 32, 32).permute(0, 2, 1).contiguous()
    return ig._split3(wn).view(3, chunks, 32, 32).permute(1, 0, 2, 3).contiguous()


_TILE = {7: (128, 768)}
_WINDOW_TILE = {**_TILE, 4: (128, 768)}
_PLAN = dict(min_ktiles=16, tile=_TILE)


class FlowNetCHeadEngine:
    def __init__(self, net, B: int, H: int, W: int, device):
        if H % 64 or W % 64:
            raise ValueError("FlowNetC head engine: frame sides must be multiples of 64")
        L.lib()
        self.net, self.B, self.H, self.W, self.dev = net, int(B), int(H), int(W), torch.device(device)
        g = {s: (H // s, W // s) for s in (4, 8, 16, 32, 64)}
        self.grid = g
        P = lambda s, chunks: ig.Planes(B, g[s][0], g[s][1], chunks, self.dev)
        G = lambda s, chunks: ig.GradSum(B, g[s][0], g[s][1], chunks, self.dev)
        self.siamese = hasattr(net, "conv_redir")
        self.c3a_p, self.c3b_p = (P(8, 8), P(8, 8)) if self.siamese else (None, None)
        self.in31, self.cat3, self.cat2 = P(8, 15 if self.siamese else 8), P(8, 13), P(4, 7)
        self.c4a, self.cat4 = P(16, 16), P(16, 25)
        self.c5a, self.cat5 = P(32, 16), P(32, 33)
        self.c6a, self.c6 = P(64, 32), P(64, 32)
        f32 = dict(dtype=torch.float32, device=self.dev)
        self.flow = {k: torch.zeros(B, 2, *g[2 ** k], **f32) for k in (6, 5, 4, 3, 2)}
        self.G_cat2, self.G_cat3, self.G_cat4, self.G_cat5 = G(4, 7), G(8, 13), G(16, 25), G(32, 33)
        self.G_c6, self.G_in31, self.G_c3a = G(64, 32), G(8, 15 if self.siamese else 8), G(8, 8)
        self.gz_cat2, self.gz_cat3, self.gz_cat4, self.gz_cat5 = P(4, 7), P(8, 13), P(16, 25), P(32, 33)
        self.gz_c6, self.gz_c6a, self.gz_c5a, self.gz_c4a = P(64, 32), P(64, 32), P(32, 16), P(16, 16)
        self.gz_in31 = P(8, 15) if self.siamese else None
        self.g_flow = {k: torch.zeros(B, 2, *g[2 ** k], **f32) for k in (6, 5, 4, 3)}
        self.g_corr = torch.zeros(B, 21, 21, *g[8], **f32)
        self.g_c2a = torch.zeros(B, 128, *g[4], **f32)
        self.g_c3a, self.g_c3a_redir, self.g_c3b = (torch.zeros(B, 256, *g[8], **f32) for _ in range(3))
        self.c3_nchw = torch.zeros(2 * B, 256, *g[8], **f32)
        self._prefix = None
        self.flow_out, self.flow_scale = self.flow[2], float(getattr(net, "div_flow", 20.0))
        self._wprefixes, self._wprefix = {}, None
        self._win_m3 = 0
        self._build_launches()

    def _conv(self, name):
        return getattr(self.net, name)[0]

    def _bias(self, conv):
        if conv.bias is None:
            return torch.zeros(conv.out_channels, dtype=torch.float32, device=self.dev)
        return conv.bias.detach().float().contiguous()

    def _stem_layers(self):
        from .plane_graph import stem_stages
        return [(name, block[0], lvl) for lvl, stage in enumerate(stem_stages(self.net), 1) for name, block in stage]

    def _build_launches(self):
        net, g = self.net, self.grid
        queue = ig.LaunchQueue(self.dev, **_PLAN)

        def plan(wi, x, in_chunk0, rows, out_hw, **kw):
            kw.setdefault("variant", self._variant_for(wi))
            return queue.add(wi, x, in_chunk0, rows, out_hw, **kw)

        self._pipe_variant = {"0": 2, "5": 5}.get(os.environ.get("UFR_IGEMM_PIPE", "6"), 6)

        fwd, bwd = {}, {}
        cw = lambda n, s, p: ig.conv_forward_weights(self._conv(n).weight, s, p)
        cb = lambda n, s, p: ig.conv_backward_weights(self._conv(n).weight, s, p)
        bias = lambda n: self._bias(self._conv(n))
        if self.siamese:
            fwd["conv_redir"] = plan(cw("conv_redir", 1, 0), self.c3a_p, 0, g[8], g[8], out_planes=self.in31, out_chunk0=0,
                                     bias=bias("conv_redir"))
        fwd["conv3_1"] = plan(cw("conv3_1", 1, 1), self.in31, 0, g[8], g[8], out_planes=self.cat3, out_chunk0=0, bias=bias("conv3_1"))
        fwd["conv4"] = plan(cw("conv4", 2, 1), self.cat3, 0, g[16], g[16], out_planes=self.c4a, bias=bias("conv4"))
        fwd["conv4_1"] = plan(cw("conv4_1", 1, 1), self.c4a, 0, g[16], g[16], out_planes=self.cat4, out_chunk0=0, bias=bias("conv4_1"))
        fwd["conv5"] = plan(cw("conv5", 2, 1), self.cat4, 0, g[32], g[32], out_planes=self.c5a, bias=bias("conv5"))
        fwd["conv5_1"] = plan(cw("conv5_1", 1, 1), self.c5a, 0, g[32], g[32], out_planes=self.cat5, out_chunk0=0, bias=bias("conv5_1"))
        fwd["conv6"] = plan(cw("conv6", 2, 1), self.cat5, 0, g[64], g[64], out_planes=self.c6a, bias=bias("conv6"))
        fwd["conv6_1"] = plan(cw("conv6_1", 1, 1), self.c6a, 0, g[64], g[64], out_planes=self.c6, bias=bias("conv6_1"))
        dec = {5: (self.c6, 64, self.cat5, 16), 4: (self.cat5, 32, self.cat4, 16), 3: (self.cat4, 16, self.cat3, 8),
               2: (self.cat3, 8, self.cat2, 4)}
        for k, (src, s_in, dst, chunk0) in dec.items():
            n = f"deconv{k}"
            fwd[n] = plan(ig.deconv_forward_weights(self._conv(n).weight, 1), src, 0, g[s_in], g[s_in // 2], out_planes=dst,
                          out_chunk0=chunk0, bias=bias(n))
        gz = {5: (self.gz_cat5, 16, 16), 4: (self.gz_cat4, 16, 8), 3: (self.gz_cat3, 8, 4), 2: (self.gz_cat2, 4, 2)}
        Gabove = {2: self.G_cat3, 3: self.G_cat4, 4: self.G_cat5}
        self.tail_w, self.tail_args = {}, {}
        for k in (2, 3, 4):
            src, chunk0, _ = gz[k]
            s_in = {2: 8, 3: 16, 4: 32}[k]
            w = self._conv(f"deconv{k}").weight
            main = w.shape[0] - 2
            bwd[f"deconv{k}"] = plan(ig.deconv_backward_weights(w[:main], 1), src, chunk0, g[s_in], g[s_in], out_f32=Gabove[k])
            self.tail_w[k] = _pack_flow_tail_mfma(w[main:])
            self.tail_args[k] = (src, chunk0, ig.pad32(w.shape[1]) // 32, Gabove[k], main // 32, g[s_in])
        bwd["deconv5"] = plan(ig.deconv_backward_weights(self._conv("deconv5").weight, 1), self.gz_cat5, 16, g[64], g[64],
                              add=self.G_c6, mask=self.c6, out_planes=self.gz_c6)
        bwd["conv6_1"] = plan(cb("conv6_1", 1, 1), self.gz_c6, 0, g[64], g[64], mask=self.c6a, out_planes=self.gz_c6a)
        bwd["conv6"] = plan(cb("conv6", 2, 1), self.gz_c6a, 0, g[64], g[32], add=self.G_cat5, mask=self.cat5, out_planes=self.gz_cat5)
        bwd["conv5_1"] = plan(cb("conv5_1", 1, 1), self.gz_cat5, 0, g[32], g[32], mask=self.c5a, out_planes=self.gz_c5a)
        bwd["conv5"] = plan(cb("conv5", 2, 1), self.gz_c5a, 0, g[32], g[16], add=self.G_cat4, mask=self.cat4, out_planes=self.gz_cat4)
        bwd["conv4_1"] = plan(cb("conv4_1", 1, 1), self.gz_cat4, 0, g[16], g[16], mask=self.c4a, out_planes=self.gz_c4a)
        bwd["conv4"] = plan(cb("conv4", 2, 1), self.gz_c4a, 0, g[16], g[8], add=self.G_cat3, mask=self.cat3, out_planes=self.gz_cat3)
        if self.siamese:
            bwd["conv3_1"] = plan(cb("conv3_1", 1, 1), self.gz_cat3, 0, g[8], g[8], mask=self.in31, out_planes=self.gz_in31,
                                  out_f32=self.G_in31, planes_chunks=1, f32_first_chunk=1)
            bwd["conv_redir"] = plan(cb("conv_redir", 1, 0), self.gz_in31, 0, g[8], g[8], out_f32=self.G_c3a)
        else:
            bwd["conv3_1"] = plan(cb("conv3_1", 1, 1), self.gz_cat3, 0, g[8], g[8], out_f32=self.G_in31)
        self.ws = queue.build()
        self.fwd = {k: h.launch for k, h in fwd.items()}
        self.plain = {}
        self.bwd = {k: self._with_tail(("full", k), h.launch, h.args, h.kw, h.S) for k, h in bwd.items()}
        self._plans = {("fwd", k): (*h.args, h.S, h.kw) for k, h in fwd.items()}
        self._plans.update({("bwd", k): (*h.args, h.S, h.kw) for k, h in bwd.items()})
        self._band, self.fwd_band, self.bwd_band = None, {}, {}
        self.bwd_band_wide, self.bwd_rest, self._band_plans, self._pf_band, self._split_w = {}, {}, {}, {}, {}
        self.pf_w = {k: _pack_flow_head(getattr(net, f"predict_flow{k}").weight) for k, _ in _HEADS}
        self.pf_wm = {k: _pack_flow_head_mfma(getattr(net, f"predict_flow{k}").weight) for k, _ in _HEADS}
        self.pf_b = {k: getattr(net, f"predict_flow{k}").bias.detach().float().contiguous() for k, _ in _HEADS}
        self.up = {k: getattr(net, f"upsampled_flow{k}_to_{k - 1}") for k in (6, 5, 4, 3)}
        self.up_w = {k: m.weight.detach().float().contiguous() for k, m in self.up.items()}
        self.up_b = {k: (m.bias.detach().float().contiguous() if m.bias is not None else None) for k, m in self.up.items()}
        self.pf_src = {6: (self.c6, 32), 5: (self.cat5, 33), 4: (self.cat4, 25), 3: (self.cat3, 13), 2: (self.cat2, 7)}
        self.pf_G = {6: self.G_c6, 5: self.G_cat5, 4: self.G_cat4, 3: self.G_cat3, 2: self.G_cat2}
        self.up_dst = {6: (self.cat5, 32), 5: (self.cat4, 24), 4: (self.cat3, 12), 3: (self.cat2, 6)}
        self.up_G = {6: (self.G_cat5, 32), 5: (self.G_cat4, 24), 4: (self.G_cat3, 12), 3: (self.G_cat2, 6)}
        self.pf_split, floats = {}, 0
        for k in (6, 5, 4, 3):
            src, chunks = self.pf_src[k]
            slices, starved, n = pf_split_plan(self.B, src.H, src.W, chunks)
            if starved:
                self.pf_split[k] = (slices, n)
                floats = max(floats, n)
        self.pf_partials = torch.empty(max(floats, 1), dtype=torch.float32, device=self.dev)
        self._pf_pending = None
        self.pf_ran = {}

    def _with_tail(self, key, plain, args, kw, S, resident=None):
        self.plain.pop(key, None)
        if S != 1 and resident is None:
            return plain
        wi, x, c0, rows, out_hw = args
        launch = ig.make_launch(wi, x, c0, rows, out_hw, ws=self.ws, balance=True, resident=resident, **kw)
        if launch.tail_plan is None:
            return plain
        self.plain[key] = plain
        return launch

    def tail_launches(self):
        tables = {"full": self.bwd, "band": self.bwd_band, "rest": self.bwd_rest}
        return [(tag, name, tables[tag][name].tail_plan) for tag, name in sorted(self.plain)]

    def _variant_for(self, wi):
        return self._pipe_variant if wi.Npad % 128 == 0 else 2

    def _build_prefix(self):
        B, dev = self.B, self.dev
        H, W = self.H, self.W
        layers = self._stem_layers()
        wis = [None] + [ig.conv_forward_weights(conv.weight, conv.stride[0], conv.padding[0]) for _, conv, _ in layers[1:]]
        scratch = {}

        def level_buffer(lvl, slot, chunks):
            if (lvl, slot) not in scratch:
                scratch[(lvl, slot)] = ig.Planes(B, H >> lvl, W >> lvl, chunks, dev)
            return scratch[(lvl, slot)]
        halves = {}
        for h, taps in (("a", {2: self.cat2, 3: self.c3a_p}), ("b", {3: self.c3b_p})):
            outs = []
            for i, (_, conv, lvl) in enumerate(layers):
                later = sum(1 for _, _, l in layers[i + 1:] if l == lvl)
                outs.append(taps[lvl] if later == 0 and lvl in taps else level_buffer(lvl, later % 2, ig.pad32(conv.out_channels) // 32))
            chain = []
            for i in range(1, len(layers)):
                name, conv, lvl = layers[i]
                launch = ig.make_launch(wis[i], outs[i - 1], 0, (H >> lvl, W >> lvl), (H >> lvl, W >> lvl), out_planes=outs[i],
                                        out_chunk0=0, bias=self._bias(conv), variant=self._variant_for(wis[i]))
                chain.append((name, launch, wis[i]))
            conv1 = layers[0][1]
            P = dict(c1=outs[0], layers=chain, b1=self._bias(conv1), w1=conv1.weight.detach())
            P.update({name: launch for name, launch, _ in chain})
            P.update({name + "_wi": wi for name, _, wi in chain})
            P.update(self._conv1_launch(B, H, W, outs[0]))
            halves[h] = P
        self._prefix = halves

    def _conv1_launch(self, n: int, H: int, W: int, c1: ig.Planes) -> dict:
        conv1 = self._stem_layers()[0][1]
# ... 64 lines not shown
        B2, dev = 2 * self.B, self.dev
        f32 = dict(dtype=torch.float32, device=dev)
        h2, w2, h4, w4, h8, w8 = wh // 2, ww // 2, wh // 4, ww // 4, wh // 8, ww // 8
        layers = self._stem_layers()
        n = len(layers)
        tap2 = max(i for i, (_, _, lvl) in enumerate(layers) if lvl == 2)
        acts = [ig.Planes(B2, wh >> lvl, ww >> lvl, ig.pad32(conv.out_channels) // 32, dev) for _, conv, lvl in layers]
        gz = [ig.Planes(B2, wh >> lvl, ww >> lvl, ig.pad32(conv.out_channels) // 32, dev) for _, conv, lvl in layers]
        G_p = ig.GradSum(B2, h2 + 3, w2 + 2, 1, dev)
        G_gw2 = ig.GradSum(B2, h4, w4, 4, dev)
        grid = lambda i: (wh >> layers[i][2], ww >> layers[i][2])
        queue, names = ig.LaunchQueue(dev, tune=False, **dict(_PLAN, tile=_WINDOW_TILE)), []
        plan = lambda wi, x, rows, out_hw, **kw: queue.add(wi, x, 0, rows, out_hw, **{"variant": self._variant_for(wi), **kw})
        for i in range(1, n):
            name, conv, _ = layers[i]
            plan(ig.conv_forward_weights(conv.weight, conv.stride[0], conv.padding[0]), acts[i - 1], grid(i), grid(i),
                 out_planes=acts[i], bias=self._bias(conv), variant=4)
            names.append(name)
        for i in range(n - 1, 0, -1):
            name, conv, _ = layers[i]
            kw = dict(add=G_gw2, mask=acts[i - 1], out_planes=gz[i - 1]) if i - 1 == tap2 else dict(out_planes=gz[i - 1], mask=acts[i - 1])
            plan(ig.conv_backward_weights(conv.weight, conv.stride[0], conv.padding[0]), gz[i], grid(i), grid(i - 1), **kw)
            names.append(name + "_bwd")
        plan(ig.conv1_packed_backward_weights(layers[0][1].weight), gz[0], (h2 + 3, w2 + 2), (h2 + 3, w2 + 2), out_f32=G_p)
        names.append(layers[0][0] + "_bwd")
        ws = queue.build()
        chain = [(name, h.launch, h.wi) for name, h in zip(names, queue.handles)]
        P = dict(hw=(wh, ww), c1=acts[0], c2=acts[tap2], c3=acts[-1], gz_c3=gz[-1], gz_c2=gz[tap2], G_gw2=G_gw2, ws=ws,
                 acts=acts, gz=gz, fwd=chain[:n - 1], bwd=chain[n - 1:],
                 G_p=G_p, gxw=torch.zeros(B2, 3, wh, ww, **f32),
                 c2_nchw=torch.zeros(B2, 128, h4, w4, **f32), c3_nchw=torch.zeros(B2, 256, h8, w8, **f32))
        P.update({name: launch for name, launch, _ in chain})
        P.update({name + "_wi": wi for name, _, wi in chain})
        P.update(self._conv1_launch(B2, wh, ww, acts[0]))
        self._wprefixes[(wh, ww)] = P
        self._bound_wprefixes()
        return P

    MAX_WINDOW_PREFIXES = 4

    def _bound_wprefixes(self):
        while len(self._wprefixes) > self.MAX_WINDOW_PREFIXES:
            del self._wprefixes[next(iter(self._wprefixes))]

    def window_prefix(self, wh: int, ww: int) -> dict:
        P = self._wprefixes.pop((int(wh), int(ww)), None)
        if P is None:
            P = self._build_window_prefix(int(wh), int(ww))
        else:
            self._wprefixes[(int(wh), int(ww))] = P
        self._wprefix = P
        return P

    def window_prefix_forward(self, xw: torch.Tensor, win: torch.Tensor, m2: int, m3: int, c2_nchw: bool = True):
        wh, ww = int(xw.shape[2]), int(xw.shape[3])
        P = self.window_prefix(wh, ww)
        self._win_m3 = int(m3)
        self._conv1(P, xw.detach(), None)
        for _, launch, _ in P["fwd"]:
            launch()
        c2, c3, H, W = P["c2"], P["c3"], self.H, self.W
        L.check(L.lib().ufr_window_features_planes(
            L.ptr(c2.t), c2.plane_stride, L.ptr(c3.t), c3.plane_stride, L.ptr(self.cat2.t), self.cat2.plane_stride,
            L.ptr(self.c3a_p.t), self.c3a_p.plane_stride, L.ptr(self.c3b_p.t), self.c3b_p.plane_stride, L.ptr(self.c3_nchw),
            L.ptr(P["c3_nchw"]), L.ptr(win), self.B, H, W, wh, ww, int(m2), int(m3), L.stream()), "window features -> planes")
        if c2_nchw:
            c2.to_nchw(128, 0, out=P["c2_nchw"])

    def window_gather_conv2_gradient(self, win: torch.Tensor, m2: int):
        P = self._wprefix
        wh, ww = P["hw"]
        h4, w4 = self.grid[4]
        L.check(L.lib().ufr_window_gather_chunks(L.ptr(self.G_cat2.t), L.ptr(P["G_gw2"].t), L.ptr(win), self.B, self.B, 2 * self.B, 4,
                                                 h4, w4, wh // 4, ww // 4, 4, int(m2), L.stream()), "window gather (chunks)")

    def window_prefix_backward(self, gw3: torch.Tensor, gw2: torch.Tensor | None = None, unpack: bool = True) -> torch.Tensor:
        P, B = self._wprefix, self.B
        wh, ww = P["hw"]
        if gw2 is not None:
            full = torch.zeros(2 * B, 128, wh // 4, ww // 4, dtype=torch.float32, device=self.dev)
            full[:B] = gw2
            P["G_gw2"].t.copy_(full.view(2 * B, 4, 32, wh // 4, ww // 4).permute(1, 0, 3, 4, 2).reshape(4, -1, 32))
        gz = P["gz_c3"]
        L.check(L.lib().ufr_nchw_grad_to_planes(L.ptr(gw3), L.ptr(P["c3_nchw"]), L.ptr(gz.t), gz.plane_stride, 0, 2 * B, 256, wh // 8,
                                                ww // 8, ig.LEAKY, L.stream()), "window gradient -> planes")
        for _, launch, _ in P["bwd"]:
            launch()
        if not unpack:
            return P["G_p"].t
        L.check(L.lib().ufr_conv1_unpack_grad(L.ptr(P["G_p"].t), L.ptr(P["gxw"]), 2 * B, wh, ww, L.stream()), "conv1 unpack")
        return P["gxw"]

    _FWD_BAND = {"conv_redir": (8, 8), "conv3_1": (8, 8), "conv4": (16, 8), "conv4_1": (16, 16)}
    _BWD_BAND = {"conv5": (32, None), "conv4_1": (16, 16), "conv4": (16, 16), "conv3_1": (8, 8), "conv_redir": (8, 8)}

    def attach_band(self, band):
        if self._band is band:
            return
        self._band, self.fwd_band, self.bwd_band = band, {}, {}
        self.bwd_band_wide, self.bwd_rest, self._band_plans, self._pf_band = {}, {}, {}, {}
        self.plain = {k: v for k, v in self.plain.items() if k[0] == "full"}
        if not band.width:
            return
        W = self.W
        if band.width % 32 or band.width > W:
            raise ValueError("band width must be a multiple of 32 pixels inside the frame")
        origin = band.win[:, 1]
        resident = getattr(band, "tail_resident", None)

        def derive(kind, name, ls_rows, ls_in):
            wi, x, c0, rows, out_hw, S, kw = self._plans[(kind, name)]
            rows_b = (rows[0], band.width // ls_rows)
            extra = dict(row_band=(origin, 8, ls_rows))
            if ls_in is not None:
                extra["in_band"] = (origin, 8, ls_in, band.width // ls_in)
            h = ig.planned_launch(wi, x, c0, rows_b, out_hw, ws=self.ws, options=dict(_PLAN, tune=False), **kw, **extra)
            if kind == "bwd":
                return self._with_tail(("band", name), h.launch, h.args, h.kw, h.S, resident)
            return h.launch

        for name, (ls_rows, _) in self._FWD_BAND.items():
            if ("fwd", name) in self._plans:
                self.fwd_band[name] = derive("fwd", name, ls_rows, None)
        for name, (ls_rows, ls_in) in self._BWD_BAND.items():
            if ("bwd", name) in self._plans:
                self.bwd_band[name] = derive("bwd", name, ls_rows, ls_in)
        if self.siamese:
            self._attach_unread(band, origin)

    _SPLIT_DECONV = {2: ("conv3_1", 8), 3: ("conv4_1", 16)}

    def _attach_unread(self, band, origin):
        def planned(name, wi, x, c0, rows, out_hw, kw):
            kw.setdefault("variant", self._variant_for(wi))
            h = ig.planned_launch(wi, x, c0, rows, out_hw, ws=self.ws, options=_PLAN, **kw)
            self._band_plans[name] = (*h.args, h.kw)
            return self._with_tail(("rest" if name.endswith(" rest") else "band", name), h.launch, h.args, h.kw, h.S,
                                   getattr(band, "tail_resident", None))
# ... 43 lines not shown
        rows = []
        for kind, table, tag in (("fwd", self.fwd, "full"), ("bwd", self.bwd, "full"), ("fwd", self.fwd_band, "band"),
                                 ("bwd", self.bwd_band, "band"), ("bwd", self.bwd_rest, "full")):
            for name, launch in table.items():
                wi = self._band_plans[name][0] if kind == "bwd" and table is not self.bwd and name in self._band_plans else \
                    self._plans[(kind, name)][0]
                d = launch.desc
                rows.append((name, kind, tag, launch, wi.flops(d.B * d.Hr * d.Wr) / 1e9))
        if self._prefix is not None:
            for h, suffix in (("a", ""), ("b", " 2nd frames")):
                F = self._prefix[h]
                packed = [("conv1", F["conv1"], F["conv1_wi"])] if "conv1" in F else []
                for key, launch, wi in packed + F["layers"]:
                    d = launch.desc
                    rows.append((key + suffix, "fwd", "prefix", launch, wi.flops(d.B * d.Hr * d.Wr) / 1e9))
        P = getattr(self, "_wprefix", None)
        if P is not None:
            packed = [("conv1", P["conv1"], P["conv1_wi"])] if "conv1" in P else []
            for kind, chain in (("fwd", packed + P["fwd"]), ("bwd", P["bwd"])):
                for key, launch, wi in chain:
                    d = launch.desc
                    rows.append((key[:-4] if kind == "bwd" else key, kind, "window", launch, wi.flops(d.B * d.Hr * d.Wr) / 1e9))
        return rows

    def conv1_direct_table(self):
        rows = []
        sets = []
        if self._prefix is not None:
            sets += [("conv1 direct" + sfx, "prefix", self._prefix[h]) for h, sfx in (("a", ""), ("b", " 2nd frames"))]
        if getattr(self, "_wprefix", None) is not None:
            sets.append(("conv1 direct", "window", self._wprefix))
        for label, tag, P in sets:
            D = P.get("direct")
            if D is None:
                continue
            n, (H, W) = D["n"], D["hw"]
            frames = torch.rand(n, 3, H, W, device=self.dev)
            nbytes = n * 3 * H * W * 4 + n * (H // 2) * (W // 2) * 64 * 6
            rows.append((label, tag, (lambda P=P, frames=frames: self._conv1(P, frames, None)), float(nbytes), D["gflop"]))
        return rows

    def _pf_forward(self, k, defer=False):
        src, chunks = self.pf_src[k]
        if k in self.pf_split:
            slices, n = self.pf_split[k]
            L.check(L.lib().ufr_flow_head_planes_forward_split(L.ptr(src.t), src.plane_stride, 0, chunks, L.ptr(self.pf_wm[k]),
                                                               self.pf_wm[k].shape[0], L.ptr(self.pf_partials), n, slices, self.B, src.H,
                                                               src.W, L.stream()), "predict_flow forward (split)")
            self.pf_ran[k] = "split"
            self._pf_pending = k
            if not defer:
                self._pf_finish(k, upsample=False)
            return
        self.pf_ran[k] = "mfma"
        L.check(L.lib().ufr_flow_head_planes_forward_mfma(L.ptr(src.t), src.plane_stride, 0, chunks, L.ptr(self.pf_wm[k]),
                                                          self.pf_wm[k].shape[0], L.ptr(self.pf_b[k]), L.ptr(self.flow[k]), self.B, src.H, src.W,
                                                          L.stream()), "predict_flow forward (mfma)")

    def _pf_backward(self, k, gy, accumulate, finalize=None, region=None):
        src, chunks = self.pf_src[k]
        if region is not None:
            head, kind, origin, stride, div, rh, rw, margin, wout = region
            act, out, c0, n = finalize if finalize is not None else (None, None, 0, 0)
            L.check(L.lib().ufr_flow_head_planes_backward_regions(
                L.ptr(gy), L.ptr(self.pf_w[k]), self.pf_w[k].shape[0], L.ptr(self.pf_G[k].t), self.pf_G[k].chunks, 0, chunks, self.B,
                src.H, src.W, int(accumulate), int(head), int(kind), L.ptr(origin), int(stride), int(div), int(rh), int(rw), int(margin),
                L.ptr(wout.t) if wout is not None else None, wout.B if wout is not None else 0,
                L.ptr(act.t) if act is not None else None, L.ptr(out.t) if out is not None else None,
                out.plane_stride if out is not None else 0, int(c0), int(n), float(ig.LEAKY), L.stream()),
                "predict_flow backward (regions)")
            return
        if finalize is not None:
            act, out, c0, n = finalize
            L.check(L.lib().ufr_flow_head_planes_backward_finalize(L.ptr(gy), L.ptr(self.pf_w[k]), self.pf_w[k].shape[0], L.ptr(self.pf_G[k].t),
                                                                   self.pf_G[k].chunks, 0, chunks, self.B,
                                                                   src.H, src.W, int(accumulate), L.ptr(act.t), L.ptr(out.t), out.plane_stride,
                                                                   int(c0), int(n), float(ig.LEAKY), L.stream()),
                    "predict_flow backward + finalize")
            return
        L.check(L.lib().ufr_flow_head_planes_backward(L.ptr(gy), L.ptr(self.pf_w[k]), self.pf_w[k].shape[0], L.ptr(self.pf_G[k].t),
                                                      self.pf_G[k].chunks, 0, chunks, self.B,
                                                      src.H, src.W, int(accumulate), L.stream()), "predict_flow backward")

    def _pf_finish(self, k, upsample):
        slices, n = self.pf_split[k]
        f = self.flow[k]
        dst, chunk = self.up_dst[k] if upsample else (None, 0)
        L.check(L.lib().ufr_flow_head_split_finish(L.ptr(self.pf_partials), n, slices, L.ptr(self.pf_b[k]), L.ptr(f), L.ptr(self.up_w[k]),
                                                   L.ptr(self.up_b[k]) if self.up_b[k] is not None else None,
                                                   L.ptr(dst.t) if upsample else None, dst.plane_stride if upsample else 0, chunk, self.B,
                                                   f.shape[2], f.shape[3], L.stream()), "predict_flow finish (split)")
        self._pf_pending = None

    def _up_forward(self, k):
        if self._pf_pending == k:
            self._pf_finish(k, upsample=True)
            return
        dst, chunk = self.up_dst[k]
        f = self.flow[k]
        L.check(L.lib().ufr_flow_up_planes_forward(L.ptr(f), L.ptr(self.up_w[k]), L.ptr(self.up_b[k]) if self.up_b[k] is not None else None,
                                                   L.ptr(dst.t), dst.plane_stride, chunk, self.B, f.shape[2], f.shape[3],
                                                   L.stream()), "upsampled_flow forward")

    def _deconv_tail(self, k):
        src, chunk0, chunks, Gd, out_chunk, (h, w) = self.tail_args[k]
        L.check(L.lib().ufr_deconv_flow_tail_backward_mfma(L.ptr(src.t), src.plane_stride, chunk0, chunks, L.ptr(self.tail_w[k]),
                                                           self.tail_w[k].shape[0], L.ptr(Gd.t), Gd.chunks, out_chunk, self.B, h, w, L.stream()),
                "deconv data gradient, flow channels")

    def _up_backward(self, k):
        G, chunk = self.up_G[k]
        f = self.g_flow[k]
        L.check(L.lib().ufr_flow_up_planes_backward(L.ptr(G.t), chunk, L.ptr(self.up_w[k]), L.ptr(f), self.B, f.shape[2],
                                                    f.shape[3], 0, L.stream()), "upsampled_flow backward")

    def _finalize(self, Gs, mask, out, chunk0, chunks):
        L.check(L.lib().ufr_grad_finalize(L.ptr(Gs.t), chunk0, L.ptr(mask.t), chunk0, L.ptr(out.t), out.plane_stride, chunk0,
                                          Gs.M, chunks, ig.LEAKY, L.stream()), "gradient finalize")

    def _forward_trunk(self, c2: torch.Tensor, c3: torch.Tensor) -> torch.Tensor:
        L.require_hip(c2, "c2")
        L.require_hip(c3, "c3")
        self.cat2.load_nchw(c2, 0)
        self.in31.load_nchw(c3, 0)
        for name in ("conv3_1", "conv4", "conv4_1", "conv5", "conv5_1", "conv6", "conv6_1"):
            self.fwd[name]()
        self._pf_forward(6, defer=True)
        for k in (5, 4, 3, 2):
            self._up_forward(k + 1)
            self.fwd[f"deconv{k}"]()
            self._pf_forward(k, defer=True)
        return self.flow[2]

    def forward_cached(self, band=None, corr_changed: bool = True) -> torch.Tensor:
        return self.forward(None, self._c3a, self._c3b, band, corr_changed=corr_changed)

    def forward(self, c2a: torch.Tensor | None, c3a: torch.Tensor, c3b: torch.Tensor, band=None,
                corr_changed: bool = True) -> torch.Tensor:
        if not self.siamese:
            return self._forward_trunk(c2a, c3a)
        for t, name in ((c3a, "c3a"), (c3b, "c3b")):
            L.require_hip(t, name)
        self._c3a, self._c3b = c3a, c3b
        inc = False
        if band is not None:
            self.attach_band(band)
            inc = bool(band.width and band.incremental and band.inc_layers)
        if c2a is not None:
            L.require_hip(c2a, "c2a")
            self.cat2.load_nchw(c2a, 0)
            self.c3a_p.load_nchw(c3a, 0)
            self.c3b_p.load_nchw(c3b, 0)
        if inc and band.cone_win is not None and band.cone_hw[1] // 8 <= 23:
            if corr_changed:
                L.check(L.lib().ufr_corr_forward_planes_changed(L.ptr(self.c3a_p.t), L.ptr(self.c3b_p.t), self.c3a_p.plane_stride,
                                                                L.ptr(self.in31.t), self.in31.plane_stride, 1, self.B, 256, *self.grid[8],
                                                                21, 2, 1.0 / 256.0, ig.LEAKY, L.ptr(band.cone_win), 8,
                                                                band.cone_hw[0] // 8, band.cone_hw[1] // 8, self._win_m3, L.stream()),
                        "correlation forward (planes, changed)")
            else:
                L.check(L.lib().ufr_corr_forward_planes_window(L.ptr(self.c3a_p.t), L.ptr(self.c3b_p.t), self.c3a_p.plane_stride,
                                                               L.ptr(self.in31.t), self.in31.plane_stride, 1, self.B, 256, *self.grid[8],
                                                               21, 2, 1.0 / 256.0, ig.LEAKY, L.ptr(band.cone_win), 8,
                                                               band.cone_hw[1] // 8, L.stream()), "correlation forward (planes, window)")
        else:
            L.check(L.lib().ufr_corr_forward_planes(L.ptr(self.c3a_p.t), L.ptr(self.c3b_p.t), self.c3a_p.plane_stride,
                                                    L.ptr(self.in31.t), self.in31.plane_stride, 1, self.B, 256, *self.grid[8], 21, 2,
                                                    1.0 / 256.0, ig.LEAKY, L.stream()), "correlation forward (planes)")
        for name in ("conv_redir", "conv3_1", "conv4", "conv4_1"):
            (self.fwd_band if inc else self.fwd)[name]()
        for name in ("conv5", "conv5_1", "conv6", "conv6_1"):
            self.fwd[name]()
        self._pf_forward(6, defer=True)
        for k in (5, 4, 3, 2):
            self._up_forward(k + 1)
            self.fwd[f"deconv{k}"]()
            self._pf_forward(k, defer=True)
        return self.flow[2]

    def backward(self, g_flow2: torch.Tensor, band=None, fused_window: bool = True, skip_unread: bool = True, tail_split: bool = True):
        L.require_hip(g_flow2, "g_flow2")
        B = self.B
        run = lambda table, tag, name: (table[name] if tail_split else self.plain.get((tag, name), table[name]))()
        banded = band is not None and bool(band.width)
        if band is not None:
            self.attach_band(band)
        gz = {2: (self.G_cat2, self.cat2, self.gz_cat2, 4, 2), 3: (self.G_cat3, self.cat3, self.gz_cat3, 8, 4),
              4: (self.G_cat4, self.cat4, self.gz_cat4, 16, 8), 5: (self.G_cat5, self.cat5, self.gz_cat5, 16, 16)}
        fuse = os.environ.get("UFR_FUSE_FINALIZE", "1") != "0"
        fin = lambda k: (gz[k][1], gz[k][2], gz[k][3], gz[k][4]) if fuse else None
        eng_window = bool(fused_window and band is not None and getattr(band, "eng_window", False)
                          and getattr(self, "_wprefix", None) is not None)
        skip = bool(skip_unread and banded and fused_window and self.siamese)
        if skip and eng_window:
            P = self._wprefix
            wh, ww = P["hw"]
            self._pf_backward(2, g_flow2, accumulate=False, finalize=fin(2),
                              region=(4, L.UFR_PF_REGION_WINDOW, band.cone_win, 8, 4, wh // 4, ww // 4, band.g2_margin, P["G_gw2"]))
        else:
            self._pf_backward(2, g_flow2, accumulate=False, finalize=fin(2))
            if eng_window:
                self.window_gather_conv2_gradient(band.cone_win, band.g2_margin)
            else:
                self.G_cat2.to_nchw(128, 0, out=self.g_c2a)
        for k in (2, 3, 4):
            Gs, act, out, chunk0, chunks = gz[k]
            if not fuse:
                self._finalize(Gs, act, out, chunk0, chunks)
            self._up_backward(k + 1)
            region = None
            if skip and k + 1 in self._pf_band:
                run(self.bwd_band, "band", f"deconv{k}")
                run(self.bwd_rest, "rest", f"deconv{k} rest")
                head, ls = self._pf_band[k + 1]
                region = (head, L.UFR_PF_REGION_BAND, band.win[:, 1], 8, ls, self.grid[ls][0], band.width // ls, 0, None)
            else:
                run(self.bwd, "full", f"deconv{k}")
            self._deconv_tail(k)
            self._pf_backward(k + 1, self.g_flow[k + 1], accumulate=True, finalize=fin(k + 1), region=region)
        Gs, act, out, chunk0, chunks = gz[5]
        if not fuse:
            self._finalize(Gs, act, out, chunk0, chunks)
        self._up_backward(6)
        self._pf_backward(6, self.g_flow[6], accumulate=False)
        for name in ("deconv5", "conv6_1", "conv6", "conv5_1"):
            run(self.bwd, "full", name)
        if not self.siamese:
            for name in ("conv5", "conv4_1", "conv4", "conv3_1"):
                run(self.bwd, "full", name)
            self.G_in31.to_nchw(256, 0, out=self.g_c3a)
            return self.g_c2a, self.g_c3a, None
        for name in ("conv5", "conv4_1", "conv4", "conv3_1", "conv_redir"):
            if banded and not skip and name in self.bwd_band_wide:
                self.bwd_band_wide[name]()
            elif banded:
                run(self.bwd_band, "band", name)
            else:
                run(self.bwd, "full", name)
        gw = getattr(band, "g3_window", None) if (band is not None and fused_window) else None
        h8, w8 = self.grid[8]
        if gw is not None and band.cone_win is not None and band.cone_hw[1] // 8 <= 16 and w8 % 4 == 0:
            L.check(L.lib().ufr_corr_backward_window_fused(L.ptr(self._c3a), L.ptr(self._c3b), L.ptr(self.G_in31.t), 1, 1.0 / 256.0,
                                                           L.ptr(self.G_c3a.t), L.ptr(gw), B, 256, h8, w8, 21, 2,
                                                           L.ptr(band.cone_win), 8, band.cone_hw[0] // 8, band.cone_hw[1] // 8,
                                                           int(band.g3_margin), L.stream()), "correlation backward (window, fused)")
            return (None if eng_window else self.g_c2a), None, None
        self.G_c3a.to_nchw(256, 0, out=self.g_c3a_redir)
        self.G_in31.to_nchw(441, 1, scale=1.0 / 256.0, out=self.g_corr.view(B, 441, *self.grid[8]))
        self._corr_backward(self.g_corr, band)
        return (None if eng_window else self.g_c2a), self.g_c3a, self.g_c3b

    def _corr_backward(self, g_corr, band):
        from . import spatial_correlation_sampler_backend as correlation
        import ctypes as C
        h8, w8 = self.grid[8]
        if band is not None and band.cone_win is not None:
            L.check(L.lib().ufr_corr_backward_window(L.ptr(self._c3a), L.ptr(self._c3b), L.ptr(g_corr), L.ptr(self.g_c3a),
                                                     L.ptr(self.g_c3b), self.B, 256, h8, w8, 21, 2, L.ptr(band.cone_win), 8,
                                                     band.cone_hw[0] // 8, band.cone_hw[1] // 8, L.stream()),
                    "correlation backward (window)")
        else:
            p = correlation._params(1, 1, 21, 21, 0, 0, 1, 1, 2, 2, 1, 1)
            L.check(L.lib().ufr_corr_backward(L.ptr(self._c3a), L.ptr(self._c3b), L.ptr(g_corr), L.ptr(self.g_c3a),
                                              L.ptr(self.g_c3b), L.UFR_F32, self.B, 256, h8, w8, C.byref(p), L.stream()),
                    "correlation backward")
        self.g_c3a.add_(self.g_c3a_redir)

    REPLACEABLE = ("conv3a", "conv3b", "corr", "conv_redir", "conv3_1")
    _HEAD_SEGMENTS = {
        "conv_redir": ("in31", 0, 32), "corr": ("in31", 1, 441), "conv3_1": ("cat3", 0, 256), "deconv3": ("cat3", 8, 128),
        "upsampled_flow4_to_3": ("cat3", 12, 2), "conv4": ("c4a", 0, 512), "conv4_1": ("cat4", 0, 512), "deconv4": ("cat4", 16, 256),
        "upsampled_flow5_to_4": ("cat4", 24, 2), "conv5": ("c5a", 0, 512), "conv5_1": ("cat5", 0, 512), "deconv5": ("cat5", 16, 512),
        "upsampled_flow6_to_5": ("cat5", 32, 2), "conv6": ("c6a", 0, 1024), "conv6_1": ("c6", 0, 1024), "deconv2": ("cat2", 4, 64),
        "upsampled_flow3_to_2": ("cat2", 6, 2)}
    _FLOW_KEYS = {"flow6": 6, "flow5": 5, "flow4": 4, "flow3": 3, "predict": 2}

    def segment_map(self, stem=None) -> dict:
        if not self.siamese:
            raise RuntimeError("feature-map segments: the FlowNetC head (the FlowNetS trunk has no correlation)")
        seg = {}
        if stem is not None:
            for lvl, cn in ((1, 64), (2, 128), (3, 256)):
                p = stem.bufs[f"c{lvl}"].planes
                seg[f"conv{lvl}a"], seg[f"conv{lvl}b"] = (p, 0, cn, 0, None), (p, 0, cn, self.B, None)
        for key, (buf, c0, cn) in self._HEAD_SEGMENTS.items():
            seg[key] = (getattr(self, buf), c0, cn, 0, "unleaky" if key == "corr" else None)
        for key, k in self._FLOW_KEYS.items():
            seg[key] = (self.flow[k], 0, 2, 0, None)
        return seg

    def capture(self, keys=None, stem=None) -> dict:
        seg = self.segment_map(stem)
        out = {}
        for key in (list(seg) if keys is None else keys):
# ... 112 lines not shown
```

understanding_flow_robustness_amd/patch_attack.py:

```python
from __future__ import annotations

import ctypes as C
import os
from argparse import Namespace

import numpy as np
import torch
from ._lib import engine_cache as _engine_cache

from . import _lib as L
from .flownets.utils_model import predict_flow

LOSS_THRESHOLD = 0.1
CLAMP_BOUND = 2.0


def _pixel_range(flownet: str):
    return (0.0, 1.0) if any(k in flownet for k in ("FlowNetC", "FlowNetS", "FlowNet2", "RAFT", "PWC")) else (-1.0, 1.0)


class ShardedExchange:

    def __init__(self, group=None):
        import torch.distributed as dist
        self.dist, self.group = dist, group
        self.world = dist.get_world_size(group) if dist.is_initialized() else 1
        self.rank = dist.get_rank(group) if dist.is_initialized() else 0

    def __call__(self, packed: torch.Tensor) -> torch.Tensor:
        if self.world > 1:
            self.dist.all_reduce(packed, op=self.dist.ReduceOp.SUM, group=self.group)
        return packed

    def gather(self, rows_local: torch.Tensor, rows_all: torch.Tensor) -> torch.Tensor:
        if self.world > 1:
            self.dist.all_gather_into_tensor(rows_all, rows_local, group=self.group)
        return rows_all


class PatchAttackStep:

    def __init__(self, flow_net, args, batch, height, width, device="cuda:0", shared_patch=True,
                 exchange: ShardedExchange | None = None, use_graph=True, warmup=3, use_cone=None, patch_hw=None,
                 sum_groups=1, skip_unread=True, corr_changed=True, tail_split=True, tail_resident=None):
        L.lib()
        self.net, self.args = flow_net, args
        self.skip_unread = bool(skip_unread)
        self.corr_changed = bool(corr_changed)
        self.tail_split, self.tail_resident = bool(tail_split), tail_resident
        self.B, self.H, self.W = batch, height, width
        self.dev = torch.device(device)
        self.shared = shared_patch
        self.exchange = exchange
        self.world = exchange.world if exchange is not None else 1
        if self.world > 1 and not shared_patch:
            raise ValueError("per-sample patches need no exchange; shard them as independent replicas")
        self.placed = patch_hw is not None
        if shared_patch and batch * self.world > 1 and not self.placed:
            raise ValueError("one patch behind several pairs is defined in patch coordinates: pass patch_hw=(ph, pw) "
                             "and load() a [1,3,ph,pw] patch / mask with per-pair origins (SURVEY.md 8e)")
        if self.placed and not shared_patch:
            raise ValueError("patch_hw: per-sample patches stay canvas-sized like the reference's")
        self.groups = int(sum_groups)
        if self.groups < 1 or batch % self.groups or (self.groups > 1 and not self.placed):
            raise ValueError("sum_groups must divide the pairs of a patch-coordinate step")
        self.lo, self.hi = _pixel_range(args.flownet)
        self.kind = 1 if getattr(args, "l2", False) else 0
        self.alpha = float(getattr(args, "alpha", 0.0))
        self.step = 0.5 * float(args.lr)
        self.CHW = 3 * height * width
        f32 = dict(dtype=torch.float32, device=self.dev)
        pb = 1 if shared_patch else batch
        self.tgt = torch.zeros(batch, 3, height, width, **f32)
        self.ref = torch.zeros_like(self.tgt)
        self._mask_canvas = None if self.placed else torch.zeros_like(self.tgt)
        self._mask_stale = self.placed
        if self.placed:
            ph, pw = (int(v) for v in patch_hw)
            if not (0 < ph <= height and 0 < pw <= width):
                raise ValueError("patch_hw does not fit the frame")
            self.ph, self.pw, self.n_p = ph, pw, 3 * ph * pw
            self.patch = torch.zeros(1, 3, ph, pw, **f32)
            self.mask_p = torch.zeros(1, 3, ph, pw, **f32)
            self.origins = torch.zeros(batch, 2, dtype=torch.int32, device=self.dev)
            self.origins_host = None
            self.rows_local = torch.zeros(self.groups, self.n_p + 1, **f32)
            self.rows_all = torch.zeros(self.world * self.groups, self.n_p + 1, **f32) if self.world > 1 else self.rows_local
            self.loss_local = torch.zeros(1, **f32)
            self.loss_cur = torch.zeros(1, **f32)
        else:
            self.patch = torch.zeros(pb, 3, height, width, **f32)
            self.loss_cur = torch.zeros(1, **f32)
            self.loss_local = self.loss_cur
        self.patch_init = torch.zeros_like(self.patch)
        self.target = torch.zeros(batch, 2, height, width, **f32)
        self.adv_tgt = torch.zeros_like(self.tgt).requires_grad_(True)
        self.adv_ref = torch.zeros_like(self.tgt).requires_grad_(True)
        self.g_flow = torch.zeros_like(self.target)
        self.loss_ws = torch.zeros(L.LOSS_PARTIALS, **f32)
        self._fused_loss = (batch * -(-(height // 4) // 16) * -(-(width // 4) // 16) <= L.LOSS_PARTIALS
                            and height % 4 == 0 and width % 4 == 0)
        self.g_flow2 = torch.zeros(batch, 2, height // 4, width // 4, **f32)
        self.state = torch.zeros(4, **f32)
        L.freeze_parameters(self.net)
        self.net.eval()
        self.graph = self.graph_b = self.graph_next = self.graph_b_next = None
        self._first = True
        self._rect_paste = False
        self.use_graph = use_graph
        self._warmup = warmup
        if use_cone is None:
            use_cone = os.environ.get("UFR_CONE", "1") != "0"
        spec = getattr(flow_net, "CONE", None)
        self.cone = spec if (use_cone and spec is not None and height % spec.total_stride == 0
                             and width % spec.total_stride == 0) else None
        self.win_hw = None
        self.win = torch.zeros(batch, 8, dtype=torch.int32, device=self.dev)
        self.patch_loaded = torch.zeros_like(self.patch) if self.cone is not None else None

    @property
    def mask(self):
        if self.placed and self._mask_stale:
            if self._mask_canvas is None:
                self._mask_canvas = torch.zeros_like(self.tgt)
            with torch.cuda.device(self.dev):
                L.check(L.lib().ufr_patch_mask_placed(L.ptr(self.mask_p), L.ptr(self.origins), L.ptr(self._mask_canvas), self.B,
                                                      self.H, self.W, self.ph, self.pw, L.stream()), "placed mask")
            self._mask_stale = False
        return self._mask_canvas

    def _paste(self, do_clamp, gate=False, write_mask=False):
        if self.placed and self._rect_paste and not write_mask:
            L.check(L.lib().ufr_patch_paste_placed_rect(
                L.ptr(self.tgt), L.ptr(self.ref), L.ptr(self.patch), L.ptr(self.mask_p), L.ptr(self.origins),
                L.ptr(self.adv_tgt), L.ptr(self.adv_ref), self.B, self.H, self.W, self.ph, self.pw, int(do_clamp), self.lo,
                self.hi, L.ptr(self.state) if gate else None, L.stream()), "placed rect paste")
            return
        if self.placed:
            L.check(L.lib().ufr_patch_paste_placed(
                L.ptr(self.tgt), L.ptr(self.ref), L.ptr(self.patch), L.ptr(self.mask_p), L.ptr(self.origins), None,
                L.ptr(self.adv_tgt), L.ptr(self.adv_ref), None, self.B, self.H,
                self.W, self.ph, self.pw, int(do_clamp), self.lo, self.hi, L.ptr(self.state) if gate else None,
                L.stream()), "placed paste")
            return
        L.check(L.lib().ufr_patch_paste(L.ptr(self.tgt), L.ptr(self.ref), L.ptr(self.patch), L.ptr(self.mask),
                                        L.ptr(self.adv_tgt), L.ptr(self.adv_ref), self.B, self.CHW,
                                        0 if self.shared else self.CHW, self.CHW, int(do_clamp), self.lo,
                                        self.hi, L.stream()), "patch paste")

    def _update(self, g_tgt, g_ref):
        L.check(L.lib().ufr_patch_update(L.ptr(self.tgt), L.ptr(self.ref), L.ptr(g_tgt), L.ptr(g_ref),
                                         L.ptr(self.patch), L.ptr(self.mask), L.ptr(self.adv_tgt),
                                         L.ptr(self.adv_ref), self.B, self.CHW, 0 if self.shared else self.CHW,
                                         self.CHW, self.step, CLAMP_BOUND, self.lo, self.hi,
                                         L.ptr(self.state), L.stream()), "patch update")

# ... 66 lines not shown
        self.band, reach = None, getattr(self.net, "BAND_REACH", None)
        if reach is not None and os.environ.get("UFR_BAND", "1") != "0":
            from .band_conv import Band, corr_band_width
            bw = -(-(ww + 2 * reach + 31) // 32) * 32
            if W % 32 != 0 or bw * 4 > W * 3:
                bw = 0
            self._band_reach = reach
            self.band = Band(torch.zeros(B, 8, dtype=torch.int32, device=self.dev), bw, cone_win=self.win,
                             cone_hw=(wh, ww))
            if bw and corr_band_width(ww) <= bw:
                self.band.corr_width = corr_band_width(ww)
            if self.tail_resident:
                self.band.tail_resident = int(self.tail_resident)
            if bw and os.environ.get("UFR_INCREMENTAL", "1") != "0":
                self.band.inc_layers = tuple(getattr(self.net, "INCREMENTAL_LAYERS", ()))

    def _win_copy(self, fn, src, dst, n, c, hf, wf, ls, margin):
        wh, ww = self.win_hw
        L.check(fn(L.ptr(src), L.ptr(dst), L.ptr(self.win), self.B, n, c, hf, wf, wh // ls, ww // ls, ls, margin,
                   L.stream()), "window copy")

    def _cone_refresh(self, prefix_features=None):
        lib = L.lib()
        wh, ww = self.win_hw
        L.check(lib.ufr_cone_window(L.ptr(self.mask), self.B, self.CHW, 3, self.H, self.W, C.byref(self._chain),
                                    wh, ww, L.ptr(self.win), L.ptr(self.state[3:]), L.stream()), "cone window")
        if not self.placed:
            self.g_tgt_full.zero_(); self.g_ref_full.zero_()
        if self.band is not None and self.band.width:
            start = torch.div(self.win[:, 1] - self._band_reach, 32, rounding_mode="floor") * 32
            self.band.win[:, 1] = start.clamp(0, self.W - self.band.width)
            if self.band.corr_width:
                from .band_conv import corr_band_origin
                self.band.win[:, 2] = corr_band_origin(self.win[:, 1], self.band.corr_width, self.W)
        self._cone_prefix(prefix_features)

    def _cone_prefix(self, prefix_features=None):
        if self.eng is not None:
            if prefix_features is not None:
                self.eng.load_prefix_features(*prefix_features)
            else:
                self.eng.prefix_full(self.adv_tgt.detach(), self.adv_ref.detach())
            return
        feats = prefix_features if prefix_features is not None else \
            self.net.encode(torch.cat((self.adv_tgt.detach(), self.adv_ref.detach()), 0))
        for (ls, m, n, full, _), f in zip(self.taps, feats):
            if f.shape[0] < n or f.shape[1:] != full.shape[1:]:
                raise ValueError("prefix_features do not match this step's frames")
            full.detach().copy_(f[:n])

    def _forward_cone(self):
        lib, B, H, W = L.lib(), self.B, self.H, self.W
        wh, ww = self.win_hw
        L.check(lib.ufr_window_gather_pair(L.ptr(self.adv_tgt), L.ptr(self.adv_ref), L.ptr(self.xw), L.ptr(self.win),
                                           L.ptr(self.loss_local), B, 3, H, W, wh, ww, L.stream()), "window gather (pair)")
        if self.eng is not None:
            self._feats_w = None
            if self.eng_kind == "pwc":
                self.eng.window_prefix_forward(self.xw, self.win, self.taps[0][1])
                self.eng.forward_cached()
            else:
                (_, m2, _, _, _), (_, m3, _, _, _) = self.taps
                self.eng.window_prefix_forward(self.xw, self.win, m2, m3, c2_nchw=False)
                self.eng.forward_cached(self.band, corr_changed=self.corr_changed)
            if self._fused_loss:
                return None
            return torch.nn.functional.interpolate(self.eng.flow_out * self.eng.flow_scale, scale_factor=4, mode="bilinear",
                                                   align_corners=False)
        self._feats_w = [f[:n] for f, (_, _, n, _, _) in zip(self.net.encode(self.xw), self.taps)]
        for f, (ls, m, n, full, _) in zip(self._feats_w, self.taps):
            self._win_copy(lib.ufr_window_scatter, f, full, n, f.shape[1], H // ls, W // ls, ls, m)
        full = [t[3] for t in self.taps]
        extra = {"band": self.band} if self.band is not None else {}
        return self.net.head(*full[:-1], full[-1][:B], full[-1][B:], **extra)

    def _backward_cone(self, flow):
        lib, B, H, W = L.lib(), self.B, self.H, self.W
        self._packed_grad = False
        if self.eng is not None:
            if flow is None:
                g_flow2 = self.g_flow2
            else:
                (g_flow2,) = torch.autograd.grad(flow, (self.eng.flow_out,), self.g_flow)
            if self.eng_kind == "pwc":
                ls, m, n, _, gw = self.taps[0]
                g_f2 = self.eng.backward(g_flow2.contiguous())
                self._win_copy(lib.ufr_window_gather, g_f2, gw, n, g_f2.shape[1], H // ls, W // ls, ls, m)
                gxw = self.eng.window_prefix_backward(gw)
            else:
                (ls2, m2, _, _, gw2), (ls3, m3, _, _, gw3) = self.taps
                if self.band is not None:
                    self.band.g3_window, self.band.g3_margin = gw3, m3
                    self.band.eng_window, self.band.g2_margin = True, m2
                g2a, g3a, g3b = self.eng.backward(g_flow2.contiguous(), self.band, skip_unread=self.skip_unread,
                                                  tail_split=self.tail_split)
                if g2a is not None:
                    self._win_copy(lib.ufr_window_gather, g2a, gw2, B, 128, H // ls2, W // ls2, ls2, m2)
                if g3a is not None:
                    self._win_copy(lib.ufr_window_gather, g3a, gw3, B, 256, H // ls3, W // ls3, ls3, m3)
                    self._win_copy(lib.ufr_window_gather, g3b, gw3[B:], B, 256, H // ls3, W // ls3, ls3, m3)
                self._packed_grad = self.placed
                gxw = self.eng.window_prefix_backward(self.taps[1][4], None if g2a is None else self.taps[0][4],
                                                      unpack=not self.placed)
        else:
            g_full = torch.autograd.grad(flow, [t[3] for t in self.taps], self.g_flow)
            for g, (ls, m, n, _, gwin) in zip(g_full, self.taps):
                self._win_copy(lib.ufr_window_gather, g.contiguous(), gwin, n, g.shape[1], H // ls, W // ls, ls, m)
            gxw, = torch.autograd.grad(self._feats_w, (self.xw,), [t[4] for t in self.taps])
        self._feats_w = None
        gxw = gxw.contiguous()
        if self.placed:
            return gxw, None
        self._win_copy(lib.ufr_window_scatter, gxw, self.g_tgt_full, B, 3, H, W, 1, 0)
        self._win_copy(lib.ufr_window_scatter, gxw[B:], self.g_ref_full, B, 3, H, W, 1, 0)
        return self.g_tgt_full, self.g_ref_full

    def _part_a(self):
        if self.cone is not None:
            flow = self._forward_cone()
        else:
            self.loss_local.zero_()
            flow = predict_flow(self.net, None, self.adv_tgt, self.adv_ref, self.args)
        weight = (1.0 - self.alpha) * ((1.0 / self.world) if self.shared else float(self.B))
        if flow is None:
            L.check(L.lib().ufr_flow2_upsampled_loss_fast(L.ptr(self.eng.flow_out), float(self.eng.flow_scale), L.ptr(self.target),
                                                          L.ptr(self.g_flow2), L.ptr(self.loss_local), self.B, self.H // 4, self.W // 4,
                                                          self.kind, weight, L.ptr(self.loss_ws), L.stream()), "upsampled flow loss")
        else:
            if not flow.is_contiguous():
                flow = flow.contiguous()
            L.check(L.lib().ufr_flow_loss(L.ptr(flow), L.ptr(self.target), L.ptr(self.g_flow), L.ptr(self.loss_local),
                                          self.B, self.H * self.W, self.kind, weight, L.ptr(self.loss_ws), L.stream()),
                    "flow loss")
        if not self.shared:
            self.loss_local.div_(float(self.B))
        if self.alpha != 0.0:
            if self.placed:
                reg = (self.mask_p * self.patch - self.mask_p * self.patch_init).abs().sum() / float(self.CHW)
            else:
                reg = torch.nn.functional.l1_loss(self.mask * self.patch, self.mask * self.patch_init)
            self.loss_local.add_(self.alpha * reg / self.world)
        if self.cone is not None:
            g_tgt, g_ref = self._backward_cone(flow)
        else:
            g_tgt, g_ref = torch.autograd.grad(flow, (self.adv_tgt, self.adv_ref), self.g_flow)
            g_tgt, g_ref = g_tgt.contiguous(), g_ref.contiguous()
        if not self.placed:
            self._update(g_tgt, g_ref)
            self._gate()
            return
        if g_ref is None:
            wh, ww = self.win_hw
            crop = L.lib().ufr_patch_grad_crop_packed if self._packed_grad else L.lib().ufr_patch_grad_crop_window
            L.check(crop(L.ptr(g_tgt), L.ptr(self.win), L.ptr(self.mask_p), L.ptr(self.origins),
                                                       L.ptr(self.loss_local), L.ptr(self.rows_local), self.B, self.H, self.W, wh, ww,
                                                       self.ph, self.pw, self.groups, L.stream()), "patch grad crop (window)")
        else:
            self._crop(g_tgt, g_ref)
        if self.world == 1:
            self._apply()
            self._gate()

    def _part_b(self):
        self._apply()
        self._gate()

    def _gate(self):
        L.check(L.lib().ufr_attack_gate(L.ptr(self.loss_cur), L.ptr(self.state), LOSS_THRESHOLD, L.stream()),
                "attack gate")

    def _incremental_now(self):
        band = getattr(self, "band", None)
        return bool(self.cone is not None and band is not None and band.inc_layers and not self._first)

    def _set_later(self, later: bool):
        band = getattr(self, "band", None) if self.cone is not None else None
# ... 294 lines not shown
```

Baseline: 1533.

## Fuse attack step passes: windowed conv1, head+upsample, corr-to-planes, single patch tail

Adds a fuse_passes path, on by default, that collapses several separate kernels in each attack iteration. The first conv reads the window directly from the full frames instead of running a gather pass. The flow head and its upsample are fused in both directions, and the correlation backward writes straight into the bf16 gradient planes. A single tail kernel then reduces the loss partials, accumulates the patch gradient from the packed buffer, updates the patch, pastes it into the adversarial frames and updates the stop state, coordinated through a ticket counter. The aim is fewer launches and fewer intermediate global-memory round trips, at the cost of more complex kernels and a grid-wide ticket synchronisation.

Result: no change. 1544, median of 6 (+0.7%).

```diff
diff --git a/include/ufr_hip.h b/include/ufr_hip.h
--- a/include/ufr_hip.h
+++ b/include/ufr_hip.h
@@ -452,6 +452,26 @@
                                int chunk, int B, int H, int W, ufr_stream_t stream);
 int ufr_flow_up_planes_backward(const float* G, int chunk, const float* w, float* grad_x, int B, int H, int W,
                                 int accumulate , ufr_stream_t stream);
+int ufr_flow_head_up_planes_forward_mfma(const void* planes, long plane_stride, int chunk0, int chunks, const void* wmf, int w_chunks,
+                                         const float* bias, float* out, const float* up_w, const float* up_bias, void* up_planes,
+                                         long up_plane_stride, int up_chunk, int B, int H, int W, ufr_stream_t stream);
+int ufr_flow_head_up_planes_backward(const float* fine_G, int fine_g_chunks, int fine_chunk, const float* up_w, float* grad_flow,
+                                     const float* wpk, int w_chunks, float* G, int g_chunks, int chunk0, int chunks, int B, int H, int W,
+                                     int accumulate, ufr_stream_t stream);
+int ufr_corr_backward_window_planes(const float* f1, const float* f2, const float* G, int g_chunk0, float g_scale,
+                                    const float* G_redir, float* grad_window, const float* act, float slope, void* out_planes,
+                                    long out_plane_stride, int out_chunk0, int B, int C, int H, int W, int patch, int dilation_patch,
+                                    const int* win, int level_stride, int wh, int ww, int margin, ufr_stream_t stream);
+int ufr_conv1_direct_window(const float* frames_a, const float* frames_b, int B, int Hf, int Wf, const int* win, int wh, int ww,
+                            float* zero, const double* mean, const void* wimg, const float* bias, float slope, void* out_planes,
+                            long plane_stride, int out_chunk0, ufr_stream_t stream);
+int ufr_flow2_upsampled_loss_fast_partials(const float* flow2, float flow_scale, const float* target, float* grad_flow2, int B, int h,
+                                           int w, int kind, float weight, float* partials, int* n_partials, ufr_stream_t stream);
+int ufr_patch_tail_packed(const float* partials, int n_partials, float* loss_local, const float* G, const int* win,
+                          const float* mask_p, const int* origins, float* rows, float* patch_p, float* loss, const float* tgt,
+                          const float* ref, float* adv_tgt, float* adv_ref, int B, int H, int W, int wh, int ww, int ph, int pw,
+                          int groups, float step, float bound, int do_clamp, float lo, float hi, float* state, float threshold,
+                          void* ticket, ufr_stream_t stream);
 
 #define UFR_TRAIN_LOSS_MAX_SCALES 8
 typedef struct {
diff --git a/understanding_flow_robustness_amd/_lib.py b/understanding_flow_robustness_amd/_lib.py
--- a/understanding_flow_robustness_amd/_lib.py
+++ b/understanding_flow_robustness_amd/_lib.py
@@ -280,6 +280,14 @@
     "ufr_diverse_forward": [_vp, _vp, _vp, _vp, _vp, _vp, _i, _i, _i, _i, _vp, _i, _vp, _vp, _vp, _l, _vp],
     "ufr_diverse_backward": [_vp, _vp, _vp, _vp, _i, _i, _i, _vp, _i, _vp, _vp],
     "ufr_step_advance": [_vp, _vp],
+    "ufr_flow_head_up_planes_forward_mfma": [_vp, _l, _i, _i, _vp, _i, _vp, _vp, _vp, _vp, _vp, _l, _i, _i, _i, _i, _vp],
+    "ufr_flow_head_up_planes_backward": [_vp, _i, _i, _vp, _vp, _vp, _i, _vp, _i, _i, _i, _i, _i, _i, _i, _vp],
+    "ufr_corr_backward_window_planes": [_vp, _vp, _vp, _i, _f, _vp, _vp, _vp, _f, _vp, _l, _i, _i, _i, _i, _i, _i, _i, _vp, _i, _i, _i, _i,
+                                        _vp],
+    "ufr_conv1_direct_window": [_vp, _vp, _i, _i, _i, _vp, _i, _i, _vp, _vp, _vp, _vp, _f, _vp, _l, _i, _vp],
+    "ufr_flow2_upsampled_loss_fast_partials": [_vp, _f, _vp, _vp, _i, _i, _i, _i, _f, _vp, C.POINTER(C.c_int), _vp],
+    "ufr_patch_tail_packed": [_vp, _i, _vp, _vp, _vp, _vp, _vp, _vp, _vp, _vp, _vp, _vp, _vp, _vp, _i, _i, _i, _i, _i, _i, _i, _i, _f, _f, _i,
+                              _f, _f, _vp, _f, _vp, _vp],
 }
 DIVERSE_COLS = 8
 PLAIN = {"ufr_abi_version": (C.c_int, []), "ufr_last_error": (C.c_char_p, []),
diff --git a/understanding_flow_robustness_amd/csrc/attack.hip b/understanding_flow_robustness_amd/csrc/attack.hip
--- a/understanding_flow_robustness_amd/csrc/attack.hip
+++ b/understanding_flow_robustness_amd/csrc/attack.hip
@@ -356,6 +356,114 @@
   }
 }
 
+__global__ __launch_bounds__(256) void patch_tail_packed_kernel(
+    const float* __restrict__ partials, int n_partials, float* __restrict__ loss_local, const float* __restrict__ G,
+    const int* __restrict__ win, const float* __restrict__ mask_p, const int* __restrict__ origins, float* __restrict__ rows,
+    float* __restrict__ patch_p, float* __restrict__ loss, const float* __restrict__ tgt, const float* __restrict__ ref,
+    float* __restrict__ adv_tgt, float* __restrict__ adv_ref, int B, int H, int W, int wh, int ww, int ph, int pw, int groups,
+    float step, float bound, int do_clamp, float lo, float hi, float* __restrict__ state, float thr, unsigned* __restrict__ ticket) {
+  __shared__ float loss_sh;
+  const bool stopped = state[0] != 0.f;
+  const int n = 3 * ph * pw, per = B / groups;
+  const int Hp = (wh >> 1) + 3, Wp = (ww >> 1) + 2;
+  const bool owns_loss = (int)blockIdx.x == n / 256;
+  if (owns_loss) {
+    if (threadIdx.x < 64) {
+      float s = 0.f;
+      for (int i = threadIdx.x; i < n_partials; i += 64) s += partials[i];
+      for (int off = 32; off > 0; off >>= 1) s += __shfl_down(s, off, 64);
+      if (threadIdx.x == 0) {
+        const float l = *loss_local + s;
+        *loss_local = l;
+        loss_sh = l;
+      }
+    }
+    __syncthreads();
+  }
+  const int e = blockIdx.x * 256 + threadIdx.x;
+  if (e == n) {
+    float s = 0.f;
+    for (int g = 0; g < groups; ++g) {
+      const float v = (g == 0) ? loss_sh : 0.f;
+      rows[(long)g * (n + 1) + n] = v;
+      s += v;
+    }
+    *loss = s;
+  } else if (e < n) {
+    const int c = e / (ph * pw), r = e - c * ph * pw, i = r / pw, j = r - i * pw;
+    const float m = mask_p[e];
+    const bool shown = m != 0.f;
+    float sum = 0.f;
+    for (int g = 0; g < groups; ++g) {
+      float s = 0.f;
+      if (shown)
+        for (int b = g * per; b < (g + 1) * per; ++b) {
+          const int y = origins[2 * b] + i, x = origins[2 * b + 1] + j;
+          if ((unsigned)y >= (unsigned)H || (unsigned)x >= (unsigned)W) continue;
+          const int y0 = min(max(win[b * 8], 0), H - wh), x0 = min(max(win[b * 8 + 1], 0), W - ww);
+          const int wy = y - y0, wx = x - x0;
+          if ((unsigned)wy >= (unsigned)wh || (unsigned)wx >= (unsigned)ww) continue;
+          const int k = (c * 2 + (wy & 1)) * 2 + (wx & 1);
+          const long ra = ((long)b * Hp + (wy >> 1) + 2) * Wp + (wx >> 1), rb = ra + (long)B * Hp * Wp;
+          const float ga = G[(ra + 2) * 32 + k] + G[(ra + 1) * 32 + 12 + k];
+          const float gb = G[(rb + 2) * 32 + k] + G[(rb + 1) * 32 + 12 + k];
+          s += ga + gb;
+        }
+      rows[(long)g * (n + 1) + e] = s;
+      sum += s;
+    }
+    if (!stopped) {
+      const float pv = patch_p[e] - clampf(step * sum, -bound, bound);
+      patch_p[e] = pv;
+      const float mp = m * pv, om = 1.0f - m;
+      for (int b = 0; b < B; ++b) {
+        const int y = origins[2 * b] + i, x = origins[2 * b + 1] + j;
+        if ((unsigned)y >= (unsigned)H || (unsigned)x >= (unsigned)W) continue;
+        const long o = ((long)b * 3 + c) * H * W + (long)y * W + x;
+        float a = om * tgt[o] + mp, d = om * ref[o] + mp;
+        if (do_clamp) { a = clampf(a, lo, hi); d = clampf(d, lo, hi); }
+        adv_tgt[o] = a;
+        adv_ref[o] = d;
+      }
+    }
+  }
+  __threadfence();
+  __syncthreads();
+  if (threadIdx.x == 0) {
+    const unsigned done = atomicAdd(ticket, 1u);
+    if (done == gridDim.x - 1) {
+      *ticket = 0u;
+      __threadfence();
+      if (!stopped) {
+        const float l = __hip_atomic_load(loss, __ATOMIC_RELAXED, __HIP_MEMORY_SCOPE_AGENT);
+        state[1] += 1.f;
+        state[2] = l;
+        if (!(l > thr)) state[0] = 1.f;
+      }
+    }
+  }
+}
+
+}
+
+extern "C" int ufr_patch_tail_packed(const float* partials, int n_partials, float* loss_local, const float* G, const int* win,
+                                     const float* mask_p, const int* origins, float* rows, float* patch_p, float* loss,
+                                     const float* tgt, const float* ref, float* adv_tgt, float* adv_ref, int B, int H, int W, int wh,
+                                     int ww, int ph, int pw, int groups, float step, float bound, int do_clamp, float lo, float hi,
+                                     float* state, float threshold, void* ticket, ufr_stream_t stream) {
+  UFR_REQUIRE(partials && loss_local && G && win && mask_p && origins && rows && patch_p && loss && tgt && ref && adv_tgt && adv_ref &&
+                  state && ticket, "patch tail (packed): null pointer argument");
+  UFR_REQUIRE(B > 0 && H > 0 && W > 0 && ph > 0 && pw > 0 && ph <= H && pw <= W && wh > 0 && ww > 0 && wh <= H && ww <= W &&
+                  !(wh & 1) && !(ww & 1), "patch tail (packed): bad shape");
+  UFR_REQUIRE(n_partials >= 0 && n_partials <= UFR_LOSS_PARTIALS, "patch tail (packed): %d partial sums, at most %d", n_partials,
+              UFR_LOSS_PARTIALS);
+  UFR_REQUIRE(groups > 0 && B % groups == 0, "patch tail (packed): the pairs must split evenly into %d groups", groups);
+  UFR_REQUIRE((long)B * 3 * ph * pw < (1L << 30), "patch tail (packed): too many patch pixels");
+  const int n = 3 * ph * pw;
+  hipLaunchKernelGGL(patch_tail_packed_kernel, dim3(n / 256 + 1), dim3(256), 0, ufr::as_stream(stream), partials, n_partials, loss_local,
+                     G, win, mask_p, origins, rows, patch_p, loss, tgt, ref, adv_tgt, adv_ref, B, H, W, wh, ww, ph, pw, groups, step, bound,
+                     do_clamp, lo, hi, state, threshold, static_cast<unsigned*>(ticket));
+  return ufr::launched("patch_tail_packed_kernel");
 }
 
 extern "C" int ufr_attack_gate(const float* loss_cur, float* state, float threshold, ufr_stream_t stream) {
@@ -682,6 +790,22 @@
   return ufr::launched("flow2_upsampled_loss_fast_kernel");
 }
 
+extern "C" int ufr_flow2_upsampled_loss_fast_partials(const float* flow2, float flow_scale, const float* target, float* grad_flow2, int B,
+                                                      int h, int w, int kind, float weight, float* partials, int* n_partials,
+                                                      ufr_stream_t stream) {
+  UFR_REQUIRE(flow2 && target && grad_flow2 && partials && n_partials, "upsampled flow loss (fast, partials): null pointer argument");
+  UFR_REQUIRE(B > 0 && h > 0 && w > 0 && (kind == 0 || kind == 1), "upsampled flow loss (fast, partials): bad argument");
+  const dim3 grid(ufr::ceil_div(w, F2_T), ufr::ceil_div(h, F2_T), B);
+  const long n = (long)grid.x * grid.y * grid.z;
+  if (n > UFR_LOSS_PARTIALS || B > 65535)
+    return ufr::fail(UFR_EUNSUPPORTED, "upsampled flow loss (fast, partials): %ld tiles exceed the %d partial sums of the fixed-order "
+                                       "reduction", n, UFR_LOSS_PARTIALS);
+  hipLaunchKernelGGL(flow2_upsampled_loss_fast_kernel, grid, dim3(256), 0, ufr::as_stream(stream), flow2, flow_scale, target,
+                     grad_flow2, partials, B, h, w, kind, weight);
+  *n_partials = (int)n;
+  return ufr::launched("flow2_upsampled_loss_fast_kernel");
+}
+
 namespace ufr {
 void loss_finalize_launch(const float* partials, int n, float* loss, hipStream_t st) {
   hipLaunchKernelGGL(loss_finalize_kernel, dim3(1), dim3(64), 0, st, partials, n, loss);
diff --git a/understanding_flow_robustness_amd/csrc/conv1_direct.hip b/understanding_flow_robustness_amd/csrc/conv1_direct.hip
--- a/understanding_flow_robustness_amd/csrc/conv1_direct.hip
+++ b/understanding_flow_robustness_amd/csrc/conv1_direct.hip
@@ -25,6 +25,8 @@
   const float* bias; float slope;
   __bf16* out; long plane_stride; int out_chunk0;
   int tiles_x, tiles_y, tiles;
+  const int* win; int Hf, Wf;
+  float* zero;
 };
 
 template <bool BUF_>
@@ -35,6 +37,7 @@
   const int li = lane & 15, g = lane >> 4;
   const int Hh = a.H >> 1, Wh = a.W >> 1;
   const long M = (long)a.N * Hh * Wh;
+  if (a.zero != nullptr && blockIdx.x == 0 && tid == 0) *a.zero = 0.f;
 
   for (int i = tid; i < 2 * BUF_B / 16; i += 512) reinterpret_cast<uint4*>(lds)[i] = make_uint4(0, 0, 0, 0);
   bf16x8 wf[7][3];
@@ -60,15 +63,20 @@
   auto fetch = [&](int t) {
     int n, Y0, X0;
     tile_coords(t, n, Y0, X0);
-    const float* img = n < a.Ba ? a.fa + (long)n * 3 * a.H * a.W : a.fb + (long)(n - a.Ba) * 3 * a.H * a.W;
-    const long HW = (long)a.H * a.W;
+    const long HW = (long)a.Hf * a.Wf;
+    const int nf = n < a.Ba ? n : n - a.Ba;
+    const float* img = (n < a.Ba ? a.fa : a.fb) + (long)nf * 3 * HW;
+    if (a.win != nullptr) {
+      const int* w = a.win + nf * 8;
+      img += (long)min(max(w[0], 0), a.Hf - a.H) * a.Wf + min(max(w[1], 0), a.Wf - a.W);
+    }
     pre_ok = 0;
 #pragma unroll
     for (int i = 0; i < PX_PER_THREAD; ++i) {
       const int idx = tid + 512 * i, ry = idx / RX, rx = idx - ry * RX;
       const int iy = 2 * Y0 - 3 + ry, ix = 2 * X0 - 3 + rx;
       const bool ok = idx < RY * RX && (unsigned)iy < (unsigned)a.H && (unsigned)ix < (unsigned)a.W;
-      const long o = (long)iy * a.W + ix;
+      const long o = (long)iy * a.Wf + ix;
       pre[i][0] = ok ? img[o] : 0.f;
       pre[i][1] = ok ? img[o + HW] : 0.f;
       pre[i][2] = ok ? img[o + 2 * HW] : 0.f;
@@ -207,12 +215,14 @@
 
 }
 
-extern "C" int ufr_conv1_direct(const float* frames_a, const float* frames_b, int Ba, int Bb, int H, int W, const double* mean,
-                                const void* wimg, const float* bias, float slope, void* out_planes, long plane_stride,
-                                int out_chunk0, ufr_stream_t stream) {
+namespace {
+int launch_conv1_direct(const float* frames_a, const float* frames_b, int Ba, int Bb, int H, int W, const int* win, int Hf, int Wf,
+                        float* zero, const double* mean, const void* wimg, const float* bias, float slope, void* out_planes,
+                        long plane_stride, int out_chunk0, ufr_stream_t stream) {
   UFR_REQUIRE(frames_a && mean && wimg && bias && out_planes && (frames_b || Bb == 0), "conv1 direct: null pointer");
   UFR_REQUIRE(Ba > 0 && Bb >= 0 && H > 0 && W > 0 && !(H & 1) && !(W & 1) && plane_stride > 0 && out_chunk0 >= 0, "conv1 direct: bad shape");
   Conv1Args a;
+  a.win = win; a.Hf = Hf; a.Wf = Wf; a.zero = zero;
   a.fa = frames_a; a.fb = frames_b; a.Ba = Ba; a.N = Ba + Bb; a.H = H; a.W = W; a.mean = mean;
   a.wimg = static_cast<const __bf16*>(wimg); a.bias = bias; a.slope = slope;
   a.out = static_cast<__bf16*>(out_planes); a.plane_stride = plane_stride; a.out_chunk0 = out_chunk0;
@@ -234,3 +244,20 @@
   else conv1_direct_kernel<false><<<grid, 512, 2 * BUF_B, ufr::as_stream(stream)>>>(a);
   return ufr::launched("conv1_direct_kernel");
 }
+}
+
+extern "C" int ufr_conv1_direct(const float* frames_a, const float* frames_b, int Ba, int Bb, int H, int W, const double* mean,
+                                const void* wimg, const float* bias, float slope, void* out_planes, long plane_stride,
+                                int out_chunk0, ufr_stream_t stream) {
+  return launch_conv1_direct(frames_a, frames_b, Ba, Bb, H, W, nullptr, H, W, nullptr, mean, wimg, bias, slope, out_planes, plane_stride,
+                             out_chunk0, stream);
+}
+
+extern "C" int ufr_conv1_direct_window(const float* frames_a, const float* frames_b, int B, int Hf, int Wf, const int* win, int wh,
+                                       int ww, float* zero, const double* mean, const void* wimg, const float* bias, float slope,
+                                       void* out_planes, long plane_stride, int out_chunk0, ufr_stream_t stream) {
+  UFR_REQUIRE(frames_b && win, "conv1 direct (window): null pointer");
+  UFR_REQUIRE(Hf > 0 && Wf > 0 && wh > 0 && ww > 0 && wh <= Hf && ww <= Wf, "conv1 direct (window): window %dx%d in %dx%d", wh, ww, Hf, Wf);
+  return launch_conv1_direct(frames_a, frames_b, B, B, wh, ww, win, Hf, Wf, zero, mean, wimg, bias, slope, out_planes, plane_stride,
+                             out_chunk0, stream);
+}
diff --git a/understanding_flow_robustness_amd/csrc/correlation_window_mfma.hip b/understanding_flow_robustness_amd/csrc/correlation_window_mfma.hip
--- a/understanding_flow_robustness_amd/csrc/correlation_window_mfma.hip
+++ b/understanding_flow_robustness_amd/csrc/correlation_window_mfma.hip
@@ -12,11 +12,15 @@
 constexpr int WP = 21, WR = 10, WC = 256;
 constexpr int AST = 72;
 
+struct WinPlanes {
+  const float* act; float slope; __bf16* out; long plane_stride; int chunk0;
+};
+
 template <int NR, int TPW>
 __global__ __launch_bounds__(256) void corr_bwd_window_mfma_kernel(
     const float* __restrict__ f1, const float* __restrict__ f2, const float* __restrict__ G, int g_chunk0, float g_scale,
     const float* __restrict__ Gredir, float* __restrict__ gwin, int B, int H, int W, const int* __restrict__ win,
-    int level_stride, int wh, int ww, int margin) {
+    int level_stride, int wh, int ww, int margin, const WinPlanes wp) {
   constexpr int CS = 16 / (4 * TPW);
   __shared__ __attribute__((aligned(16))) __bf16 As[2][NR][3][16 * AST];
   const int tid = threadIdx.x, lane = tid & 63, wave = tid >> 6;
@@ -113,19 +117,26 @@
         const bool rim = rim_y || (xl < margin && x0 > 0) || (xl >= ww - margin && x0 + ww < W);
         float v = acc[r][t][e];
         if (adj == 0 && Gredir) v += Gredir[((long)(c >> 5) * M + ((long)n * H + y) * W + x0 + xl) * 32 + (c & 31)];
-        gwin[(((long)(adj * B + n) * WC + c) * wh + ly) * ww + xl] = rim ? 0.f : v;
+        v = rim ? 0.f : v;
+        const long at = (((long)(adj * B + n) * WC + c) * wh + ly) * ww + xl;
+        if (gwin) gwin[at] = v;
+        if (wp.out) {
+          if (wp.act) v = wp.act[at] > 0.f ? v : v * wp.slope;
+          __bf16 s0, s1, s2;
+          split3(v, s0, s1, s2);
+          const long rows = 2L * B * wh * ww;
+          __bf16* dst = wp.out + ((long)(wp.chunk0 + (c >> 5)) * rows + ((long)(adj * B + n) * wh + ly) * ww + xl) * 32 + (c & 31);
+          dst[0] = s0; dst[wp.plane_stride] = s1; dst[2 * wp.plane_stride] = s2;
+        }
       }
     }
   }
 }
 
-}
-
-extern "C" int ufr_corr_backward_window_fused(const float* f1, const float* f2, const float* G, int g_chunk0, float g_scale,
-                                              const float* G_redir, float* grad_window, int B, int C, int H, int W, int patch,
-                                              int dilation_patch, const int* win, int level_stride, int wh, int ww, int margin,
-                                              ufr_stream_t stream) {
-  UFR_REQUIRE(f1 && f2 && G && grad_window && win, "corr backward window (fused): null pointer");
+int launch_corr_bwd_window(const float* f1, const float* f2, const float* G, int g_chunk0, float g_scale, const float* G_redir,
+                           float* grad_window, int B, int C, int H, int W, int patch, int dilation_patch, const int* win,
+                           int level_stride, int wh, int ww, int margin, const WinPlanes wp, ufr_stream_t stream) {
+  UFR_REQUIRE(f1 && f2 && G && (grad_window || wp.out) && win, "corr backward window (fused): null pointer");
   UFR_REQUIRE(B > 0 && H > 0 && W > 0 && g_chunk0 >= 0 && level_stride > 0, "corr backward window (fused): bad shape");
   UFR_REQUIRE(wh > 0 && ww > 0 && wh <= H && ww <= W && margin >= 0 && 2 * margin <= wh && 2 * margin <= ww,
               "corr backward window (fused): window %dx%d (margin %d) in %dx%d", wh, ww, margin, H, W);
@@ -137,9 +148,32 @@
 #define UFR_CBW_LAUNCH(NR, TPW)                                                                                             \
   corr_bwd_window_mfma_kernel<NR, TPW><<<dim3(2 * ufr::ceil_div(ufr::ceil_div(wh, 2), NR), 2 * (16 / (4 * TPW)), B), 256, 0, \
                                          ufr::as_stream(stream)>>>(f1, f2, G, g_chunk0, g_scale, G_redir, grad_window, B, H, W, \
-                                                                   win, level_stride, wh, ww, margin)
+                                                                   win, level_stride, wh, ww, margin, wp)
   if (cfg == 11) UFR_CBW_LAUNCH(1, 1);
   else UFR_CBW_LAUNCH(2, 1);
 #undef UFR_CBW_LAUNCH
   return ufr::launched("corr_bwd_window_mfma_kernel");
 }
+}
+
+extern "C" int ufr_corr_backward_window_fused(const float* f1, const float* f2, const float* G, int g_chunk0, float g_scale,
+                                              const float* G_redir, float* grad_window, int B, int C, int H, int W, int patch,
+                                              int dilation_patch, const int* win, int level_stride, int wh, int ww, int margin,
+                                              ufr_stream_t stream) {
+  UFR_REQUIRE(grad_window, "corr backward window (fused): null pointer");
+  return launch_corr_bwd_window(f1, f2, G, g_chunk0, g_scale, G_redir, grad_window, B, C, H, W, patch, dilation_patch, win, level_stride,
+                                wh, ww, margin, WinPlanes{nullptr, 1.f, nullptr, 0, 0}, stream);
+}
+
+extern "C" int ufr_corr_backward_window_planes(const float* f1, const float* f2, const float* G, int g_chunk0, float g_scale,
+                                               const float* G_redir, float* grad_window, const float* act, float slope,
+                                               void* out_planes, long out_plane_stride, int out_chunk0, int B, int C, int H, int W,
+                                               int patch, int dilation_patch, const int* win, int level_stride, int wh, int ww,
+                                               int margin, ufr_stream_t stream) {
+  UFR_REQUIRE(out_planes && out_chunk0 >= 0 && B > 0 && wh > 0 && ww > 0 && C > 0, "corr backward window (planes): null pointer / bad shape");
+  UFR_REQUIRE(out_plane_stride > 0 && ((long)out_chunk0 + (C + 31) / 32) * 2L * B * wh * ww * 32 <= out_plane_stride,
+              "corr backward window (planes): chunks [%d, %d) leave the planes operand", out_chunk0, out_chunk0 + (C + 31) / 32);
+  return launch_corr_bwd_window(f1, f2, G, g_chunk0, g_scale, G_redir, grad_window, B, C, H, W, patch, dilation_patch, win, level_stride,
+                                wh, ww, margin, WinPlanes{act, slope, static_cast<__bf16*>(out_planes), out_plane_stride, out_chunk0},
+                                stream);
+}
diff --git a/understanding_flow_robustness_amd/csrc/engine_small.hip b/understanding_flow_robustness_amd/csrc/engine_small.hip
--- a/understanding_flow_robustness_amd/csrc/engine_small.hip
+++ b/understanding_flow_robustness_amd/csrc/engine_small.hip
@@ -151,13 +151,18 @@
 __device__ __attribute__((aligned(64))) unsigned pf_zero_page[16];
 constexpr int PFM_MAXT = 6;
 
+struct PfUpFwd {
+  const float* w; const float* bias; __bf16* planes; long plane_stride; int chunk;
+};
 template <int MODE, int WPS_ = 4, int MAXT_ = PFM_MAXT>
 __global__ __launch_bounds__(512) void flow_head_planes_fwd_mfma(const __bf16* __restrict__ x, long plane_stride, int chunk0,
                                                                  int chunks, const __bf16* __restrict__ wmf,
                                                                  const float* __restrict__ bias, float* __restrict__ out,
-                                                                 int out_chunk, int B, int H, int W, int TH, int S) {
-  constexpr int TW = MODE == 0 ? 32 : 16, TS = MODE == 0 ? 20 : 36;
-  constexpr int PFM_HW = MODE == 2 ? 18 : 34;
+                                                                 int out_chunk, int B, int H, int W, int TH, int S, const PfUpFwd up) {
+  constexpr bool PF = MODE == 0 || MODE == 3;
+  constexpr int TW = PF ? 32 : 16, TS = PF ? 20 : 36;
+  constexpr int PFM_HW = MODE == 3 ? 36 : (MODE == 2 ? 18 : 34);
+  constexpr int HALO = MODE == 3 ? 2 : 1;
   extern __shared__ __attribute__((aligned(16))) float pfm_T[];
   const int Hs = MODE == 1 ? 2 * H : H, Ws = MODE == 1 ? 2 * W : W;
   const long M = (long)B * Hs * Ws;
@@ -165,8 +170,8 @@
   const int tiles_x = (W + TW - 1) / TW, tiles_y = (H + TH - 1) / TH;
   const int b = blockIdx.x / (tiles_x * tiles_y), tr = blockIdx.x - b * tiles_x * tiles_y;
   const int y0 = (tr / tiles_x) * TH, x0 = (tr % tiles_x) * TW;
-  const int sy0 = MODE == 1 ? 2 * y0 - 1 : y0 - 1, sx0 = MODE == 1 ? 2 * x0 - 1 : x0 - 1;
-  const int nh = (MODE == 1 ? 2 * TH + 2 : TH + 2) * PFM_HW, mt = (nh + 15) >> 4;
+  const int sy0 = MODE == 1 ? 2 * y0 - 1 : y0 - HALO, sx0 = MODE == 1 ? 2 * x0 - 1 : x0 - HALO;
+  const int nh = (MODE == 1 ? 2 * TH + 2 : TH + 2 * HALO) * PFM_HW, mt = (nh + 15) >> 4;
   const __bf16* zero = reinterpret_cast<const __bf16*>(pf_zero_page);
   const __bf16* abase[MAXT_];
   unsigned okmask = 0;
@@ -221,7 +226,7 @@
       for (int r = 0; r < 4; ++r) {
         float* row = T + ((tw + WPS_ * s) * 16 + (lane >> 4) * 4 + r) * TS;
         row[lane & 15] = acc[s][0][r];
-        if (MODE != 0 || (lane & 15) < 2) row[16 + (lane & 15)] = acc[s][1][r];
+        if (!PF || (lane & 15) < 2) row[16 + (lane & 15)] = acc[s][1][r];
       }
     }
   __syncthreads();
@@ -249,6 +254,71 @@
       const long HWo = (long)Ho * Wo, p = (long)Y * Wo + X;
       out[((long)b * 2 + 0) * HWo + p] = r0 + bias[0];
       out[((long)b * 2 + 1) * HWo + p] = r1 + bias[1];
+    }
+    return;
+  }
+  if constexpr (MODE == 3) {
+    float* f = pfm_T + (long)S * mt * 16 * TS;
+    const int nf = (TH + 2) * 34;
+    for (int idx = tid; idx < nf; idx += blockDim.x) {
+      const int hy = idx / 34, hx = idx - hy * 34;
+      const int yy = y0 - 1 + hy, xx = x0 - 1 + hx;
+      float r0 = 0.f, r1 = 0.f;
+      if (yy >= 0 && yy < H && xx >= 0 && xx < W) {
+        for (int sl = 0; sl < S; ++sl) {
+          const float* Ts = pfm_T + (long)sl * mt * 16 * TS;
+#pragma unroll
+          for (int k = 0; k < 9; ++k) {
+            const float* e = Ts + ((hy + k / 3) * PFM_HW + hx + k % 3) * TS + 2 * k;
+            r0 += e[0];
+            r1 += e[1];
+          }
+        }
+        r0 = r0 + bias[0];
+        r1 = r1 + bias[1];
+        if (hy >= 1 && hy <= TH && hx >= 1 && hx <= 32) {
+          const long HW = (long)H * W, p = (long)yy * W + xx;
+          out[((long)b * 2 + 0) * HW + p] = r0;
+          out[((long)b * 2 + 1) * HW + p] = r1;
+        }
+      }
+      f[idx] = r0;
+      f[nf + idx] = r1;
+    }
+    __syncthreads();
+    const int Ho = 2 * H, Wo = 2 * W;
+    const long total = (long)B * Ho * Wo;
+    for (int idx = tid; idx < 2 * TH * 64; idx += blockDim.x) {
+      const int Y = 2 * y0 + (idx >> 6), X = 2 * x0 + (idx & 63);
+      if (Y >= Ho || X >= Wo) continue;
+      float a0 = up.bias ? up.bias[0] : 0.f, a1 = up.bias ? up.bias[1] : 0.f;
+#pragma unroll
+      for (int t = 0; t < 2; ++t) {
+        const int ky = ((Y + 1) & 1) + 2 * t, yy = (Y + 1 - ky) / 2;
+        if (Y + 1 - ky < 0 || yy >= H) continue;
+#pragma unroll
+        for (int u = 0; u < 2; ++u) {
+          const int kx = ((X + 1) & 1) + 2 * u, xx = (X + 1 - kx) / 2;
+          if (X + 1 - kx < 0 || xx >= W) continue;
+#pragma unroll
+          for (int ic = 0; ic < 2; ++ic) {
+            const float v = f[ic * nf + (yy - y0 + 1) * 34 + xx - x0 + 1];
+            a0 = fmaf(v, up.w[((ic * 2 + 0) * 4 + ky) * 4 + kx], a0);
+            a1 = fmaf(v, up.w[((ic * 2 + 1) * 4 + ky) * 4 + kx], a1);
+          }
+        }
+      }
+      __bf16 s0[3], s1[3];
+      split3(a0, s0[0], s0[1], s0[2]);
+      split3(a1, s1[0], s1[1], s1[2]);
+      __bf16* dst = up.planes + ((long)up.chunk * total + ((long)b * Ho + Y) * Wo + X) * 32;
+#pragma unroll
+      for (int p = 0; p < 3; ++p) {
+        bf16x8 v = {s0[p], s1[p], (__bf16)0.f, (__bf16)0.f, (__bf16)0.f, (__bf16)0.f, (__bf16)0.f, (__bf16)0.f};
+        const bf16x8 zero = {(__bf16)0.f, (__bf16)0.f, (__bf16)0.f, (__bf16)0.f, (__bf16)0.f, (__bf16)0.f, (__bf16)0.f, (__bf16)0.f};
+        bf16x8* o = reinterpret_cast<bf16x8*>(dst + p * up.plane_stride);
+        o[0] = v; o[1] = zero; o[2] = zero; o[3] = zero;
+      }
     }
     return;
   }
@@ -674,32 +744,92 @@
   }
 }
 
+__device__ __forceinline__ void flow_up_bwd_pixel(const float* __restrict__ G, int chunk, const float* __restrict__ w, int b, int yy,
+                                                  int xx, int H, int W, long Mf, float& a0, float& a1) {
+  const int Ho = 2 * H, Wo = 2 * W;
+  a0 = 0.f; a1 = 0.f;
+#pragma unroll
+  for (int ky = 0; ky < 4; ++ky) {
+    const int Y = 2 * yy - 1 + ky;
+    if (Y < 0 || Y >= Ho) continue;
+#pragma unroll
+    for (int kx = 0; kx < 4; ++kx) {
+      const int X = 2 * xx - 1 + kx;
+      if (X < 0 || X >= Wo) continue;
+      const float2 g = *reinterpret_cast<const float2*>(G + ((long)chunk * Mf + ((long)b * Ho + Y) * Wo + X) * 32);
+      a0 = fmaf(g.x, w[((0 * 2 + 0) * 4 + ky) * 4 + kx], a0);
+      a1 = fmaf(g.x, w[((1 * 2 + 0) * 4 + ky) * 4 + kx], a1);
+      a0 = fmaf(g.y, w[((0 * 2 + 1) * 4 + ky) * 4 + kx], a0);
+      a1 = fmaf(g.y, w[((1 * 2 + 1) * 4 + ky) * 4 + kx], a1);
+    }
+  }
+}
+
 __global__ void flow_up_planes_bwd(const float* __restrict__ G, int chunk, const float* __restrict__ w, float* __restrict__ gx,
                                    int B, int H, int W, int accumulate) {
-  const int Ho = 2 * H, Wo = 2 * W;
-  const long total = (long)B * H * W, Mf = (long)B * Ho * Wo;
+  const long total = (long)B * H * W, Mf = total * 4;
   for (long i = (long)blockIdx.x * blockDim.x + threadIdx.x; i < total; i += (long)gridDim.x * blockDim.x) {
     const int xx = (int)(i % W), yy = (int)((i / W) % H), b = (int)(i / ((long)W * H));
-    float a0 = 0.f, a1 = 0.f;
-#pragma unroll
-    for (int ky = 0; ky < 4; ++ky) {
-      const int Y = 2 * yy - 1 + ky;
-      if (Y < 0 || Y >= Ho) continue;
-#pragma unroll
-      for (int kx = 0; kx < 4; ++kx) {
-        const int X = 2 * xx - 1 + kx;
-        if (X < 0 || X >= Wo) continue;
-        const float2 g = *reinterpret_cast<const float2*>(G + ((long)chunk * Mf + ((long)b * Ho + Y) * Wo + X) * 32);
-        a0 = fmaf(g.x, w[((0 * 2 + 0) * 4 + ky) * 4 + kx], a0);
-        a1 = fmaf(g.x, w[((1 * 2 + 0) * 4 + ky) * 4 + kx], a1);
-        a0 = fmaf(g.y, w[((0 * 2 + 1) * 4 + ky) * 4 + kx], a0);
-        a1 = fmaf(g.y, w[((1 * 2 + 1) * 4 + ky) * 4 + kx], a1);
-      }
-    }
+    float a0, a1;
+    flow_up_bwd_pixel(G, chunk, w, b, yy, xx, H, W, Mf, a0, a1);
     float* o0 = gx + ((size_t)b * 2 + 0) * H * W + (size_t)yy * W + xx;
     float* o1 = gx + ((size_t)b * 2 + 1) * H * W + (size_t)yy * W + xx;
     *o0 = accumulate ? *o0 + a0 : a0;
     *o1 = accumulate ? *o1 + a1 : a1;
+  }
+}
+
+constexpr int PBU_TH = 4, PBU_TW = 32, PBU_HALO = (PBU_TH + 2) * (PBU_TW + 2), PBU_GF = 2 * PBU_HALO + 8;
+struct PfUp {
+  const float* Gf; int chunk; const float* w; float* gflow;
+};
+
+__global__ __launch_bounds__(512) void flow_head_planes_bwd_up(const PfUp up, const float* __restrict__ wpk, float* __restrict__ G,
+                                                               int chunk0, int chunks, int B, int H, int W, int accumulate, int per,
+                                                               int slices) {
+  extern __shared__ __attribute__((aligned(16))) float lds_up[];
+  float* gf = lds_up;
+  float* lds_w = lds_up + PBU_GF;
+  const long M = (long)B * H * W;
+  const int tid = threadIdx.x;
+  const int tile = blockIdx.x / slices, slice = blockIdx.x - tile * slices;
+  const int c_lo = slice * per, c_hi = min(chunks, c_lo + per);
+  const int tiles_x = (W + PBU_TW - 1) / PBU_TW, tiles_y = (H + PBU_TH - 1) / PBU_TH;
+  const int b = tile / (tiles_x * tiles_y), tr = tile - b * tiles_x * tiles_y;
+  const int y0 = (tr / tiles_x) * PBU_TH, x0 = (tr % tiles_x) * PBU_TW;
+  for (int i = tid; i < (c_hi - c_lo) * 576 / 4; i += blockDim.x)
+    reinterpret_cast<float4*>(lds_w)[i] = reinterpret_cast<const float4*>(wpk + (long)c_lo * 576)[i];
+  if (tid < PBU_HALO) {
+    const int hy = tid / (PBU_TW + 2), hx = tid - hy * (PBU_TW + 2);
+    const int yy = y0 + hy - 1, xx = x0 + hx - 1;
+    float a0 = 0.f, a1 = 0.f;
+    if (yy >= 0 && yy < H && xx >= 0 && xx < W) {
+      flow_up_bwd_pixel(up.Gf, up.chunk, up.w, b, yy, xx, H, W, M * 4, a0, a1);
+      if (slice == 0 && hy >= 1 && hy <= PBU_TH && hx >= 1 && hx <= PBU_TW) {
+        const long HW = (long)H * W, p = (long)yy * W + xx;
+        up.gflow[((long)b * 2 + 0) * HW + p] = a0;
+        up.gflow[((long)b * 2 + 1) * HW + p] = a1;
+      }
+    }
+    gf[tid] = a0;
+    gf[PBU_HALO + tid] = a1;
+  }
+  __syncthreads();
+  const int t = tid >> 2, q = tid & 3, ly = t / PBU_TW, lx = t - ly * PBU_TW;
+  const int yy = y0 + ly, xx = x0 + lx;
+  if (yy >= H || xx >= W) return;
+  float g0[9], g1[9];
+#pragma unroll
+  for (int k = 0; k < 9; ++k) {
+    const int o = (ly + 1 - (k / 3 - 1)) * (PBU_TW + 2) + lx + 1 - (k % 3 - 1);
+    g0[k] = gf[o];
+    g1[k] = gf[PBU_HALO + o];
+  }
+  const long pix = ((long)b * H + yy) * W + xx;
+  for (int ch = c_lo; ch < c_hi; ++ch) {
+    float4 lo, hi;
+    pf_bwd_chunk(lds_w + (ch - c_lo) * 576 + q * 8, g0, g1, lo, hi);
+    pf_bwd_store(G + ((long)(chunk0 + ch) * M + pix) * 32 + q * 8, accumulate, lo, hi);
   }
 }
 
@@ -789,12 +919,35 @@
                                            8 * 12 * 16 * TS * sizeof(float));
     if (e != hipSuccess) return ufr::fail(UFR_ELAUNCH, "%s: %s", what, hipGetErrorString(e));
     flow_head_planes_fwd_mfma<MODE, 1, 12><<<blocks, 512, lds8, st>>>(static_cast<const __bf16*>(planes), plane_stride, chunk0, chunks,
-                                                                      static_cast<const __bf16*>(wmf), bias, out, out_chunk, B, H, W, TH, 8);
+                                                                      static_cast<const __bf16*>(wmf), bias, out, out_chunk, B, H, W, TH, 8,
+                                                                      PfUpFwd{nullptr, nullptr, nullptr, 0, 0});
     return ufr::launched(what);
   }
   flow_head_planes_fwd_mfma<MODE><<<blocks, 256 * S, lds, st>>>(static_cast<const __bf16*>(planes), plane_stride, chunk0, chunks,
-                                                                static_cast<const __bf16*>(wmf), bias, out, out_chunk, B, H, W, TH, S);
+                                                                static_cast<const __bf16*>(wmf), bias, out, out_chunk, B, H, W, TH, S,
+                                                                PfUpFwd{nullptr, nullptr, nullptr, 0, 0});
   return ufr::launched(what);
+}
+
+int launch_pf_up_mfma(const void* planes, long plane_stride, int chunk0, int chunks, const void* wmf, const float* bias, float* out,
+                      const PfUpFwd& up, int B, int H, int W, hipStream_t st, const char* what) {
+  const PfMode0Plan p = pf_mode0_plan(B, H, W, chunks);
+  if (p.eight)
+    return ufr::fail(UFR_EUNSUPPORTED, "%s: this grid runs the eight-slice form of the small grids (use the split form: "
+                                       "ufr_flow_head_planes_forward_split + ufr_flow_head_split_finish)", what);
+  const int TH = p.TH == 4 ? 8 : p.TH;
+  const int blocks = B * ufr::ceil_div(H, TH) * ufr::ceil_div(W, 32);
+  const int mt = ((TH + 4) * 36 + 15) / 16;
+  const size_t lds = ((size_t)p.S * mt * 16 * 20 + 2 * (size_t)(TH + 2) * 34) * sizeof(float);
+  auto go = [&](auto kernel) {
+    hipError_t e = ufr::ensure_dynamic_lds(reinterpret_cast<const void*>(kernel), lds);
+    if (e != hipSuccess) return ufr::fail(UFR_ELAUNCH, "%s: %s", what, hipGetErrorString(e));
+    kernel<<<blocks, 256 * p.S, lds, st>>>(static_cast<const __bf16*>(planes), plane_stride, chunk0, chunks,
+                                           static_cast<const __bf16*>(wmf), bias, out, 0, B, H, W, TH, p.S, up);
+    return ufr::launched(what);
+  };
+  if (mt > 4 * PFM_MAXT) return go(flow_head_planes_fwd_mfma<3, 4, 12>);
+  return go(flow_head_planes_fwd_mfma<3>);
 }
 }
 
@@ -806,6 +959,22 @@
   UFR_REQUIRE_RANGE("flow head (planes, mfma) forward", plane_stride, (long)B * H * W, chunk0, chunks, w_chunks);
   return launch_pf_mfma<0>(planes, plane_stride, chunk0, chunks, wmf, bias, out, 0, B, H, W, ufr::as_stream(stream),
                            "flow_head_planes_fwd_mfma");
+}
+
+extern "C" int ufr_flow_head_up_planes_forward_mfma(const void* planes, long plane_stride, int chunk0, int chunks, const void* wmf,
+                                                    int w_chunks, const float* bias, float* out, const float* up_w, const float* up_bias,
+                                                    void* up_planes, long up_plane_stride, int up_chunk, int B, int H, int W,
+                                                    ufr_stream_t stream) {
+  const char* what = "flow head + upsample (planes, mfma) forward";
+  UFR_REQUIRE(planes && wmf && bias && out && up_w && up_planes, "%s: null pointer", what);
+  UFR_REQUIRE(B > 0 && H > 0 && W > 0 && chunks > 0 && chunks <= 48 && chunk0 >= 0 && up_chunk >= 0 && (long)B * H * W < (1L << 27),
+              "%s: bad shape", what);
+  UFR_REQUIRE_RANGE("flow head + upsample (planes, mfma) forward", plane_stride, (long)B * H * W, chunk0, chunks, w_chunks);
+  UFR_REQUIRE(planes_hold(up_plane_stride, (long)B * H * W * 4, up_chunk, 1), "%s: chunk %d leaves the upsampled planes operand", what,
+              up_chunk);
+  return launch_pf_up_mfma(planes, plane_stride, chunk0, chunks, wmf, bias, out,
+                           PfUpFwd{up_w, up_bias, static_cast<__bf16*>(up_planes), up_plane_stride, up_chunk}, B, H, W,
+                           ufr::as_stream(stream), what);
 }
 
 extern "C" int ufr_flow_head_split_plan(int B, int H, int W, int chunks, int* slices, int* starved, long* partial_floats) {
@@ -986,6 +1155,28 @@
   return ufr::launched("flow_head_planes_bwd_regions");
 }
 
+extern "C" int ufr_flow_head_up_planes_backward(const float* fine_G, int fine_g_chunks, int fine_chunk, const float* up_w,
+                                                float* grad_flow, const float* wpk, int w_chunks, float* G, int g_chunks, int chunk0,
+                                                int chunks, int B, int H, int W, int accumulate, ufr_stream_t stream) {
+  const char* what = "flow head + upsample (planes) backward";
+  UFR_REQUIRE(fine_G && up_w && grad_flow && wpk && G, "%s: null pointer", what);
+  UFR_REQUIRE(B > 0 && H > 0 && W > 0 && chunks > 0 && chunks <= 48 && chunk0 >= 0 && (long)B * H * W < (1L << 27), "%s: bad shape", what);
+  UFR_REQUIRE_GRANGE("flow head + upsample (planes) backward", chunk0, chunks, w_chunks, g_chunks);
+  UFR_REQUIRE(fine_chunk >= 0 && fine_chunk < fine_g_chunks, "%s: chunk %d is not in the fine grid's gradient sum (%d chunks)", what,
+              fine_chunk, fine_g_chunks);
+  const long tiles = (long)B * ufr::ceil_div(H, PBU_TH) * ufr::ceil_div(W, PBU_TW);
+  int slices = 1;
+  while (tiles * slices < 256 && slices < chunks) slices *= 2;
+  if (slices > chunks) slices = chunks;
+  const int per = ufr::ceil_div(chunks, slices);
+  slices = ufr::ceil_div(chunks, per);
+  hipError_t e = ufr::ensure_dynamic_lds(reinterpret_cast<const void*>(flow_head_planes_bwd_up), ((size_t)PBU_GF + 48 * 576) * 4);
+  if (e != hipSuccess) return ufr::fail(UFR_ELAUNCH, "%s: %s", what, hipGetErrorString(e));
+  flow_head_planes_bwd_up<<<dim3((unsigned)(tiles * slices)), 512, ((size_t)PBU_GF + (size_t)per * 576) * 4, ufr::as_stream(stream)>>>(
+      PfUp{fine_G, fine_chunk, up_w, grad_flow}, wpk, G, chunk0, chunks, B, H, W, accumulate, per, slices);
+  return ufr::launched("flow_head_planes_bwd_up");
+}
+
 extern "C" int ufr_flow_up_planes_forward(const float* x, const float* w, const float* bias, void* planes, long plane_stride,
                                           int chunk, int B, int H, int W, ufr_stream_t stream) {
   UFR_REQUIRE(x && w && planes, "flow upsample (planes) forward: null pointer");
diff --git a/understanding_flow_robustness_amd/flownetc_engine.py b/understanding_flow_robustness_amd/flownetc_engine.py
--- a/understanding_flow_robustness_amd/flownetc_engine.py
+++ b/understanding_flow_robustness_amd/flownetc_engine.py
@@ -83,6 +83,7 @@
         self.flow_out, self.flow_scale = self.flow[2], float(getattr(net, "div_flow", 20.0))
         self._wprefixes, self._wprefix = {}, None
         self._win_m3 = 0
+        self.fuse_passes = True
         self._build_launches()
 
     def _conv(self, name):
@@ -170,15 +171,18 @@
         self.pf_G = {6: self.G_c6, 5: self.G_cat5, 4: self.G_cat4, 3: self.G_cat3, 2: self.G_cat2}
         self.up_dst = {6: (self.cat5, 32), 5: (self.cat4, 24), 4: (self.cat3, 12), 3: (self.cat2, 6)}
         self.up_G = {6: (self.G_cat5, 32), 5: (self.G_cat4, 24), 4: (self.G_cat3, 12), 3: (self.G_cat2, 6)}
-        self.pf_split, floats = {}, 0
+        self.pf_split, self.pf_up_fused, floats = {}, set(), 0
         for k in (6, 5, 4, 3):
             src, chunks = self.pf_src[k]
             slices, starved, n = pf_split_plan(self.B, src.H, src.W, chunks)
+            if not starved and slices != 8:
+                self.pf_up_fused.add(k)
             if starved:
                 self.pf_split[k] = (slices, n)
                 floats = max(floats, n)
         self.pf_partials = torch.empty(max(floats, 1), dtype=torch.float32, device=self.dev)
         self._pf_pending = None
+        self._pf_up_done = None
         self.pf_ran = {}
 
     def _with_tail(self, key, plain, args, kw, S, resident=None):
@@ -349,11 +353,24 @@
         self._wprefix = P
         return P
 
-    def window_prefix_forward(self, xw: torch.Tensor, win: torch.Tensor, m2: int, m3: int, c2_nchw: bool = True):
-        wh, ww = int(xw.shape[2]), int(xw.shape[3])
+    def window_direct(self, wh: int, ww: int) -> bool:
+        return self.window_prefix(wh, ww).get("direct") is not None
+
+    def window_prefix_forward(self, xw: torch.Tensor | None, win: torch.Tensor, m2: int, m3: int, c2_nchw: bool = True,
+                              frames=None, hw=None, zero: torch.Tensor | None = None):
+        wh, ww = (int(xw.shape[2]), int(xw.shape[3])) if frames is None else (int(hw[0]), int(hw[1]))
         P = self.window_prefix(wh, ww)
         self._win_m3 = int(m3)
-        self._conv1(P, xw.detach(), None)
+        if frames is not None:
+            D, c1 = P["direct"], P["direct"]["c1"]
+            fa, fb = (t.detach().contiguous() for t in frames)
+            L.require_hip(fa, "frames")
+            L.check(L.lib().ufr_conv1_direct_window(L.ptr(fa), L.ptr(fb), self.B, self.H, self.W, L.ptr(win), wh, ww,
+                                                    L.ptr(zero) if zero is not None else None,
+                                                    L.ptr(self.net._mean64.reshape(-1).contiguous()), L.ptr(D["wimg"]), L.ptr(D["bias"]),
+                                                    float(ig.LEAKY), L.ptr(c1.t), c1.plane_stride, 0, L.stream()), "conv1 direct (window)")
+        else:
+            self._conv1(P, xw.detach(), None)
         for _, launch, _ in P["fwd"]:
             launch()
         c2, c3, H, W = P["c2"], P["c3"], self.H, self.W
@@ -371,7 +388,7 @@
         L.check(L.lib().ufr_window_gather_chunks(L.ptr(self.G_cat2.t), L.ptr(P["G_gw2"].t), L.ptr(win), self.B, self.B, 2 * self.B, 4,
                                                  h4, w4, wh // 4, ww // 4, 4, int(m2), L.stream()), "window gather (chunks)")
 
-    def window_prefix_backward(self, gw3: torch.Tensor, gw2: torch.Tensor | None = None, unpack: bool = True) -> torch.Tensor:
+    def window_prefix_backward(self, gw3: torch.Tensor | None, gw2: torch.Tensor | None = None, unpack: bool = True) -> torch.Tensor:
         P, B = self._wprefix, self.B
         wh, ww = P["hw"]
         if gw2 is not None:
@@ -379,8 +396,9 @@
             full[:B] = gw2
             P["G_gw2"].t.copy_(full.view(2 * B, 4, 32, wh // 4, ww // 4).permute(1, 0, 3, 4, 2).reshape(4, -1, 32))
         gz = P["gz_c3"]
-        L.check(L.lib().ufr_nchw_grad_to_planes(L.ptr(gw3), L.ptr(P["c3_nchw"]), L.ptr(gz.t), gz.plane_stride, 0, 2 * B, 256, wh // 8,
-                                                ww // 8, ig.LEAKY, L.stream()), "window gradient -> planes")
+        if gw3 is not None:
+            L.check(L.lib().ufr_nchw_grad_to_planes(L.ptr(gw3), L.ptr(P["c3_nchw"]), L.ptr(gz.t), gz.plane_stride, 0, 2 * B, 256,
+                                                    wh // 8, ww // 8, ig.LEAKY, L.stream()), "window gradient -> planes")
         for _, launch, _ in P["bwd"]:
             launch()
         if not unpack:
@@ -530,13 +548,31 @@
             if not defer:
                 self._pf_finish(k, upsample=False)
             return
+        if defer and self.fuse_passes and k in self.pf_up_fused:
+            dst, chunk = self.up_dst[k]
+            self.pf_ran[k] = "mfma+up"
+            L.check(L.lib().ufr_flow_head_up_planes_forward_mfma(
+                L.ptr(src.t), src.plane_stride, 0, chunks, L.ptr(self.pf_wm[k]), self.pf_wm[k].shape[0], L.ptr(self.pf_b[k]),
+                L.ptr(self.flow[k]), L.ptr(self.up_w[k]), L.ptr(self.up_b[k]) if self.up_b[k] is not None else None, L.ptr(dst.t),
+                dst.plane_stride, chunk, self.B, src.H, src.W, L.stream()), "predict_flow + upsampled_flow forward (mfma)")
+            self._pf_up_done = k
+            return
         self.pf_ran[k] = "mfma"
         L.check(L.lib().ufr_flow_head_planes_forward_mfma(L.ptr(src.t), src.plane_stride, 0, chunks, L.ptr(self.pf_wm[k]),
                                                           self.pf_wm[k].shape[0], L.ptr(self.pf_b[k]), L.ptr(self.flow[k]), self.B, src.H, src.W,
                                                           L.stream()), "predict_flow forward (mfma)")
 
-    def _pf_backward(self, k, gy, accumulate, finalize=None, region=None):
+    def _pf_backward(self, k, gy, accumulate, finalize=None, region=None, up=False):
         src, chunks = self.pf_src[k]
+        if up:
+            if finalize is not None or region is not None:
+                raise ValueError("predict_flow backward: the form with upsampled_flow's adjoint has no regions and no finalisation")
+            Gf, fchunk = self.up_G[k]
+            w, G = self.pf_w[k], self.pf_G[k]
+            L.check(L.lib().ufr_flow_head_up_planes_backward(L.ptr(Gf.t), Gf.chunks, fchunk, L.ptr(self.up_w[k]), L.ptr(gy), L.ptr(w),
+                                                             w.shape[0], L.ptr(G.t), G.chunks, 0, chunks, self.B, src.H, src.W,
+                                                             int(accumulate), L.stream()), "upsampled_flow + predict_flow backward")
+            return
         if region is not None:
             head, kind, origin, stride, div, rh, rw, margin, wout = region
             act, out, c0, n = finalize if finalize is not None else (None, None, 0, 0)
@@ -571,6 +607,9 @@
         self._pf_pending = None
 
     def _up_forward(self, k):
+        if self._pf_up_done == k:
+            self._pf_up_done = None
+            return
         if self._pf_pending == k:
             self._pf_finish(k, upsample=True)
             return
@@ -663,6 +702,7 @@
         banded = band is not None and bool(band.width)
         if band is not None:
             self.attach_band(band)
+            band.g3_planes_done = False
         gz = {2: (self.G_cat2, self.cat2, self.gz_cat2, 4, 2), 3: (self.G_cat3, self.cat3, self.gz_cat3, 8, 4),
               4: (self.G_cat4, self.cat4, self.gz_cat4, 16, 8), 5: (self.G_cat5, self.cat5, self.gz_cat5, 16, 16)}
         fuse = os.environ.get("UFR_FUSE_FINALIZE", "1") != "0"
@@ -699,8 +739,9 @@
         Gs, act, out, chunk0, chunks = gz[5]
         if not fuse:
             self._finalize(Gs, act, out, chunk0, chunks)
-        self._up_backward(6)
-        self._pf_backward(6, self.g_flow[6], accumulate=False)
+        if not self.fuse_passes:
+            self._up_backward(6)
+        self._pf_backward(6, self.g_flow[6], accumulate=False, up=self.fuse_passes)
         for name in ("deconv5", "conv6_1", "conv6", "conv5_1"):
             run(self.bwd, "full", name)
         if not self.siamese:
@@ -718,6 +759,15 @@
         gw = getattr(band, "g3_window", None) if (band is not None and fused_window) else None
         h8, w8 = self.grid[8]
         if gw is not None and band.cone_win is not None and band.cone_hw[1] // 8 <= 16 and w8 % 4 == 0:
+            P = self._wprefix
+            band.g3_planes_done = bool(getattr(band, "g3_planes", False) and eng_window and P["hw"] == tuple(band.cone_hw))
+            if band.g3_planes_done:
+                gz = P["gz_c3"]
+                L.check(L.lib().ufr_corr_backward_window_planes(
+                    L.ptr(self._c3a), L.ptr(self._c3b), L.ptr(self.G_in31.t), 1, 1.0 / 256.0, L.ptr(self.G_c3a.t), None,
+                    L.ptr(P["c3_nchw"]), float(ig.LEAKY), L.ptr(gz.t), gz.plane_stride, 0, B, 256, h8, w8, 21, 2, L.ptr(band.cone_win), 8,
+                    band.cone_hw[0] // 8, band.cone_hw[1] // 8, int(band.g3_margin), L.stream()), "correlation backward (window, planes)")
+                return None, None, None
             L.check(L.lib().ufr_corr_backward_window_fused(L.ptr(self._c3a), L.ptr(self._c3b), L.ptr(self.G_in31.t), 1, 1.0 / 256.0,
                                                            L.ptr(self.G_c3a.t), L.ptr(gw), B, 256, h8, w8, 21, 2,
                                                            L.ptr(band.cone_win), 8, band.cone_hw[0] // 8, band.cone_hw[1] // 8,
diff --git a/understanding_flow_robustness_amd/patch_attack.py b/understanding_flow_robustness_amd/patch_attack.py
--- a/understanding_flow_robustness_amd/patch_attack.py
+++ b/understanding_flow_robustness_amd/patch_attack.py
@@ -42,12 +42,13 @@
 
     def __init__(self, flow_net, args, batch, height, width, device="cuda:0", shared_patch=True,
                  exchange: ShardedExchange | None = None, use_graph=True, warmup=3, use_cone=None, patch_hw=None,
-                 sum_groups=1, skip_unread=True, corr_changed=True, tail_split=True, tail_resident=None):
+                 sum_groups=1, skip_unread=True, corr_changed=True, tail_split=True, tail_resident=None, fuse_passes=True):
         L.lib()
         self.net, self.args = flow_net, args
         self.skip_unread = bool(skip_unread)
         self.corr_changed = bool(corr_changed)
         self.tail_split, self.tail_resident = bool(tail_split), tail_resident
+        self.fuse_passes = bool(fuse_passes)
         self.B, self.H, self.W = batch, height, width
         self.dev = torch.device(device)
         self.shared = shared_patch
@@ -102,6 +103,7 @@
                             and height % 4 == 0 and width % 4 == 0)
         self.g_flow2 = torch.zeros(batch, 2, height // 4, width // 4, **f32)
         self.state = torch.zeros(4, **f32)
+        self.ticket = torch.zeros(1, dtype=torch.int32, device=self.dev)
         L.freeze_parameters(self.net)
         self.net.eval()
         self.graph = self.graph_b = self.graph_next = self.graph_b_next = None
@@ -274,8 +276,10 @@
     def _forward_cone(self):
         lib, B, H, W = L.lib(), self.B, self.H, self.W
         wh, ww = self.win_hw
-        L.check(lib.ufr_window_gather_pair(L.ptr(self.adv_tgt), L.ptr(self.adv_ref), L.ptr(self.xw), L.ptr(self.win),
-                                           L.ptr(self.loss_local), B, 3, H, W, wh, ww, L.stream()), "window gather (pair)")
+        direct = bool(self.fuse_passes and self.eng is not None and self.eng_kind != "pwc" and self.eng.window_direct(wh, ww))
+        if not direct:
+            L.check(lib.ufr_window_gather_pair(L.ptr(self.adv_tgt), L.ptr(self.adv_ref), L.ptr(self.xw), L.ptr(self.win),
+                                               L.ptr(self.loss_local), B, 3, H, W, wh, ww, L.stream()), "window gather (pair)")
         if self.eng is not None:
             self._feats_w = None
             if self.eng_kind == "pwc":
@@ -283,7 +287,12 @@
                 self.eng.forward_cached()
             else:
                 (_, m2, _, _, _), (_, m3, _, _, _) = self.taps
-                self.eng.window_prefix_forward(self.xw, self.win, m2, m3, c2_nchw=False)
+                self.eng.fuse_passes = self.fuse_passes
+                if direct:
+                    self.eng.window_prefix_forward(None, self.win, m2, m3, c2_nchw=False, frames=(self.adv_tgt, self.adv_ref),
+                                                   hw=(wh, ww), zero=self.loss_local)
+                else:
+                    self.eng.window_prefix_forward(self.xw, self.win, m2, m3, c2_nchw=False)
                 self.eng.forward_cached(self.band, corr_changed=self.corr_changed)
             if self._fused_loss:
                 return None
@@ -314,6 +323,8 @@
                 if self.band is not None:
                     self.band.g3_window, self.band.g3_margin = gw3, m3
                     self.band.eng_window, self.band.g2_margin = True, m2
+                    self.band.g3_planes = self.fuse_passes
+                self.eng.fuse_passes = self.fuse_passes
                 g2a, g3a, g3b = self.eng.backward(g_flow2.contiguous(), self.band, skip_unread=self.skip_unread,
                                                   tail_split=self.tail_split)
                 if g2a is not None:
@@ -322,8 +333,9 @@
                     self._win_copy(lib.ufr_window_gather, g3a, gw3, B, 256, H // ls3, W // ls3, ls3, m3)
                     self._win_copy(lib.ufr_window_gather, g3b, gw3[B:], B, 256, H // ls3, W // ls3, ls3, m3)
                 self._packed_grad = self.placed
-                gxw = self.eng.window_prefix_backward(self.taps[1][4], None if g2a is None else self.taps[0][4],
-                                                      unpack=not self.placed)
+                planes_done = self.band is not None and getattr(self.band, "g3_planes_done", False)
+                gxw = self.eng.window_prefix_backward(None if planes_done else self.taps[1][4],
+                                                      None if g2a is None else self.taps[0][4], unpack=not self.placed)
         else:
             g_full = torch.autograd.grad(flow, [t[3] for t in self.taps], self.g_flow)
             for g, (ls, m, n, _, gwin) in zip(g_full, self.taps):
@@ -344,6 +356,21 @@
             self.loss_local.zero_()
             flow = predict_flow(self.net, None, self.adv_tgt, self.adv_ref, self.args)
         weight = (1.0 - self.alpha) * ((1.0 / self.world) if self.shared else float(self.B))
+        one_tail = bool(self.fuse_passes and flow is None and self.placed and self.world == 1 and self._rect_paste
+                        and self.alpha == 0.0 and self.eng_kind != "pwc")
+        if one_tail:
+            n_part = C.c_int(0)
+            L.check(L.lib().ufr_flow2_upsampled_loss_fast_partials(
+                L.ptr(self.eng.flow_out), float(self.eng.flow_scale), L.ptr(self.target), L.ptr(self.g_flow2), self.B, self.H // 4,
+                self.W // 4, self.kind, weight, L.ptr(self.loss_ws), C.byref(n_part), L.stream()), "upsampled flow loss (partials)")
+            g_packed, _ = self._backward_cone(flow)
+            wh, ww = self.win_hw
+            L.check(L.lib().ufr_patch_tail_packed(
+                L.ptr(self.loss_ws), n_part.value, L.ptr(self.loss_local), L.ptr(g_packed), L.ptr(self.win), L.ptr(self.mask_p),
+                L.ptr(self.origins), L.ptr(self.rows_local), L.ptr(self.patch), L.ptr(self.loss_cur), L.ptr(self.tgt), L.ptr(self.ref),
+                L.ptr(self.adv_tgt), L.ptr(self.adv_ref), self.B, self.H, self.W, wh, ww, self.ph, self.pw, self.groups, self.step,
+                CLAMP_BOUND, 1, self.lo, self.hi, L.ptr(self.state), LOSS_THRESHOLD, L.ptr(self.ticket), L.stream()), "patch tail")
+            return
         if flow is None:
             L.check(L.lib().ufr_flow2_upsampled_loss_fast(L.ptr(self.eng.flow_out), float(self.eng.flow_scale), L.ptr(self.target),
                                                           L.ptr(self.g_flow2), L.ptr(self.loss_local), self.B, self.H // 4, self.W // 4,
```
